# kronbichler/multigrid

Measured on AMD Instinct MI355X. Metric: DoFs/s for Laplace matvec + V-cycle, poisson_cube p=4 fp64, higher is better.
Workload: dtype f64; 1 GPU; poisson_cube FE_Q(4) 128^3 cells, 135005697 DoFs per GPU, 8 levels, step = 1 fp64 vmult + 1 V-cycle (Chebyshev degree 3, first kind); cells_per_dim=128, degree=4, n_dofs_per_gpu=135005697, global_dofs=135005697, parallelism=1 GPU

## Files before the change

### multigrid_amd/csrc/mgx_api.cpp

```cpp
#include "../../include/mgx.h"
#include "mgx_bricks.hpp"
#include "mgx_device_memory.hpp"
#include "mgx_internal.hpp"
#include "mgx_krylov.hpp"

#include <hip/hip_runtime.h>
#include <rccl/rccl.h>

#include <dlfcn.h>

#include <algorithm>
#include <chrono>
#include <cmath>
#include <cstdio>
#include <cstdlib>
#include <cstring>
#include <memory>
#include <string>
#include <type_traits>
#include <utility>
#include <vector>

using namespace mgx;

namespace
{
  thread_local std::string g_last_error;

  int fail(int code, const std::string &msg)
  {
    g_last_error = msg;
    return code;
  }

  inline size_t number_size(int number) { return number == MGX_F64 ? 8 : 4; }

  bool g_trace = false;
  bool trace_on() { return g_trace; }
#define MGX_TRACE(...)                  \
  do                                    \
    {                                   \
      if (trace_on())                   \
        {                               \
          std::fprintf(stderr, "[mgx] " __VA_ARGS__); \
          std::fputc('\n', stderr);     \
          std::fflush(stderr);          \
        }                               \
    }                                   \
  while (0)
}

int mgx::report_error(int code, const char *message) { return fail(code, message ? message : ""); }

#ifndef MGX_CELLS_FORM
#define MGX_CELLS_FORM 0
#endif
extern "C" int mgx_has_cells_form(void) { return MGX_CELLS_FORM; }
extern "C" int64_t mgx_live_device_allocations(void) { return mgx::live_device_allocations().load(); }

mgx::Tunables mgx::Tunables::from_environment()
{
  Tunables t;
  auto     num = [](const char *name, uint32_t dflt) {
    const char *e = std::getenv(name);
    return e ? (uint32_t)std::strtoul(e, nullptr, 10) : dflt;
  };
  t.trace               = std::getenv("MGX_TRACE") != nullptr;
  t.brick_min           = num("MGX_BRICK_MIN", t.brick_min);
  t.brick_min_from_env  = std::getenv("MGX_BRICK_MIN") != nullptr;
  t.overlap_min         = num("MGX_OVERLAP_MIN_BRICKS", t.overlap_min);
  t.restrict_colour_min = num("MGX_RESTRICT_COLOUR_MIN", t.restrict_colour_min);
  t.cell_colour_min     = num("MGX_CELL_COLOUR_MIN", t.cell_colour_min);
  t.free_max_bricks     = num("MGX_FREE_MAX_BRICKS", t.free_max_bricks);
  t.free_one_max        = num("MGX_FREE_ONE_MAX", t.free_one_max);
  t.graph_max_dofs      = num("MGX_GRAPH_MAX_DOFS", t.graph_max_dofs);
  return t;
}

bool mgx::Tunables::set(const std::string &name, double value)
{
  const bool     on = value != 0.;
  const uint32_t u  = value <= 0. ? 0u : (value >= 4294967295. ? 0xFFFFFFFFu : (uint32_t)value);
  struct Entry
  {
    const char *name;
    bool       *flag;
    uint32_t   *number;
  };
  const Entry table[] = {
    {"trace", &trace, nullptr},
    {"brick_min", nullptr, &brick_min},
    {"overlap_min_bricks", nullptr, &overlap_min},
    {"restrict_colour_min", nullptr, &restrict_colour_min},
    {"cell_colour_min", nullptr, &cell_colour_min},
    {"free_max_bricks", nullptr, &free_max_bricks},
    {"free_one_max", nullptr, &free_one_max},
    {"graph_max_dofs", nullptr, &graph_max_dofs},
    {"general_kernel", &general_kernel, nullptr},
    {"no_bricks", &no_bricks, nullptr},
#if MGX_CELLS_FORM
    {"cells_form", &cells_form, nullptr},
    {"brick_wide_max", nullptr, &wide_max},
#endif
    {"macro_wg_per_cu_x16", nullptr, &macro_wg_x16},
    {"no_diag_table", &no_diag_table, nullptr},
    {"no_macro_v2", &no_macro_v2, nullptr},
    {"no_general_bricks", &no_general_bricks, nullptr},
    {"general_brick_min", nullptr, &general_brick_min},
    {"fused_prolong_min_bricks", nullptr, &fused_prolong_min_bricks},
    {"roctx", &roctx, nullptr},
    {"no_fused_init", &no_fused_init, nullptr},
    {"no_fused_restrict", &no_fused_restrict, nullptr},
    {"no_fused_prolong", &no_fused_prolong, nullptr},
    {"force_fused_transfers", &force_fused_transfers, nullptr},
    {"transfer_v1", &transfer_v1, nullptr},
    {"restrict_atomic", &restrict_atomic, nullptr},
    {"exchange_unfused", &exchange_unfused, nullptr},
    {"no_graph", &no_graph, nullptr},
    {"dg_no_overlap", &dg_no_overlap, nullptr},
    {"dg_unmerged_restrict", &dg_unmerged_restrict, nullptr},
    {"no_fused_decomposed", &no_fused_decomposed, nullptr},
    {"no_fused_assembly", &no_fused_assembly, nullptr},
    {"no_fused_residual", &no_fused_residual, nullptr},
    {"no_restrict_scratch", &no_restrict_scratch, nullptr},
    {"rccl_selftest", &rccl_selftest, nullptr},
  };
  for (const Entry &e : table)
    if (name == e.name)
      {
        if (e.flag)
          *e.flag = on;
        else
          *e.number = u;
        if (name == "brick_min")
          brick_min_from_env = true;
        return true;
      }
  return false;
}

struct ExchangePlan
{
  std::vector<uint32_t> not_owned_host;
  int                    plan_id = 0, number = MGX_F64, self_pos = 0;
  std::vector<int>       rank;
  std::vector<uint32_t>  count;
  std::vector<uint32_t *> index_dev;
  std::vector<void *>    send, recv;
  uint32_t              *shared_dev = nullptr, *not_owned_dev = nullptr;
  uint32_t               n_shared = 0, n_not_owned = 0;
  void                  *own_buf = nullptr;
  std::vector<uint32_t>  start;
  uint32_t              *all_index_dev = nullptr, *csr_start_dev = nullptr, *csr_pos_dev = nullptr;
  uint8_t               *all_seg_dev = nullptr, *csr_k_dev = nullptr;
  bool                   fused = false;
};

struct RcclApi
{
  void *lib = nullptr;
  decltype(&ncclGetUniqueId)    GetUniqueId    = nullptr;
  decltype(&ncclCommInitRank)   CommInitRank   = nullptr;
  decltype(&ncclCommDestroy)    CommDestroy    = nullptr;
  decltype(&ncclGroupStart)     GroupStart     = nullptr;
  decltype(&ncclGroupEnd)       GroupEnd       = nullptr;
  decltype(&ncclSend)           Send           = nullptr;
  decltype(&ncclRecv)           Recv           = nullptr;
  decltype(&ncclAllReduce)      AllReduce      = nullptr;
  decltype(&ncclGetErrorString) GetErrorString = nullptr;
  bool load()
  {
    if (lib)
      return true;
    const char *names[] = {"librccl.so", "librccl.so.1", "/opt/rocm/lib/librccl.so.1"};
    for (const char *n : names)
      if ((lib = dlopen(n, RTLD_NOW | RTLD_NOLOAD)))
        break;
    if (!lib)
      for (const char *n : names)
        if ((lib = dlopen(n, RTLD_NOW | RTLD_GLOBAL)))
          break;
    if (!lib)
      return false;
#define MGX_RCCL_SYM(name)                                        \
  name = reinterpret_cast<decltype(name)>(dlsym(lib, "nccl" #name)); \
  if (!name)                                                      \
    {                                                             \
      lib = nullptr;                                              \
      return false;                                               \
    }
    MGX_RCCL_SYM(GetUniqueId)
    MGX_RCCL_SYM(CommInitRank)
    MGX_RCCL_SYM(CommDestroy)
    MGX_RCCL_SYM(GroupStart)
    MGX_RCCL_SYM(GroupEnd)
    MGX_RCCL_SYM(Send)
    MGX_RCCL_SYM(Recv)
    MGX_RCCL_SYM(AllReduce)
    MGX_RCCL_SYM(GetErrorString)
#undef MGX_RCCL_SYM
    return true;
  }
};
static RcclApi &rccl_api()
{
  static RcclApi api;
  return api;
}

struct mgx_context_s
{
  int         device = 0;
  Tunables    tun;
  DeviceArena mem{"mgx_context"};
  hipStream_t stream = nullptr;
  bool        borrowed_stream = false;
  hipStream_t side     = nullptr;
  hipEvent_t  ev_iface = nullptr, ev_side = nullptr;
  double     *partial_dev = nullptr;
  double     *result_dev  = nullptr;
  double     *result_host = nullptr;
  bool                                        profile = false;
  struct Bracket
  {
    hipEvent_t start, stop;
    int        form, launches;
  };
  std::vector<Bracket> ev_pool, ev_used;
  bool                                      has_comm = false;
  mgx_comm_desc                             comm{};
  ncclComm_t                                nccl = nullptr;
  bool                                      use_rccl = false;
  int                                       rccl_rank = 0, rccl_size = 1;
  double                                   *ar_dev = nullptr;
  std::vector<std::pair<size_t, struct ExchangePlan *>> plans;
};

struct mgx_operator_s
{
  mgx_context_t ctx = nullptr;
  DeviceArena   mem{"mgx_operator"};
  OperatorData  d;
  double        S[kMaxN * kMaxN], D[kMaxN * kMaxN], w[kMaxN];
  bool          has_diag = false;
  bool          profiled = false;
  uint32_t     *global_index_dev = nullptr;
  double        start_sum = 0, start_count = 0;
  std::unique_ptr<ExchangePlan> plan;
  double  *cg_partials = nullptr, *cg_result = nullptr;
  void    *cg_carrier  = nullptr;
  bool     constrained_last = false;
  bool     coef_update  = false;
  double   metric[6]    = {0, 0, 0, 0, 0, 0};
  double   det_jacobian = 0;
  void    *unit_q = nullptr, *jxw_q = nullptr;
};

struct mgx_smoother_s
{
  mgx_operator_t    op = nullptr;
  DeviceArena       mem{"mgx_smoother"};
  mgx_smoother_info info{};
  void             *x_old = nullptr, *tmp = nullptr;
  void             *x_old2 = nullptr;
  bool              fourth_kind = false;
  double            range_a     = 0;
  double            req_range  = 0;
  int               req_degree = 0, req_eig_its = 0;
  krylov::ChebyshevFactors factors() const { return krylov::ChebyshevFactors(info, fourth_kind); }
};

struct mgx_transfer_s
{
  mgx_operator_t coarse = nullptr, fine = nullptr;
  DeviceArena    mem{"mgx_transfer"};
  TransferData   d;
  void          *scratch = nullptr;
  void          *interp_1d  = nullptr;
  uint32_t      *own_coarse = nullptr;
};

struct mgx_solver_s
{
  mgx_context_t               ctx = nullptr;
  DeviceArena                 mem{"mgx_solver"};
  int                         n_levels = 0, degree = 0, n_cycles = 1, vnumber = MGX_F64;
  std::vector<mgx_operator_t> matrix, matrix_dp;
  std::vector<mgx_transfer_t> transfer, transfer_dp;
  std::vector<mgx_smoother_t> smooth;
  std::vector<double *>       solution, rhs, residual;
  std::vector<void *>         defect, t, solution_update;
  std::vector<uint32_t *>     bc_index_dev;
  std::vector<double *>       bc_value_dev, bc_zero_dev;
  std::vector<uint32_t>       bc_count;
  double                     *cg_r = nullptr, *cg_z = nullptr, *cg_d = nullptr, *cg_h = nullptr;
  bool                        timing = false;
  std::vector<double>         timings;
  int             graph_level = -1, graph_calls = 0;
  bool            graph_failed = false;
  hipGraph_t      graph = nullptr;
  hipGraphExec_t  graph_exec = nullptr;
  mgx_solver_t    agg_solver = nullptr;
  int             agg_level  = -1;
  int             agg_offset = 0;
  uint32_t       *agg_map    = nullptr;
  uint8_t        *agg_owned  = nullptr;
  hipEvent_t      agg_in = nullptr, agg_out = nullptr;
  std::vector<double> agg_host;
  std::vector<double> cg_history;
  std::vector<double *> nl_state;
};

namespace
{
  int read_result(mgx_context_t ctx, double *out)
  {
    MGX_HIP(hipMemcpyAsync(ctx->result_host, ctx->result_dev, sizeof(double), hipMemcpyDeviceToHost, ctx->stream));
    MGX_HIP(hipStreamSynchronize(ctx->stream));
    *out = ctx->result_host[0];
    return MGX_OK;
  }

  int comm_allreduce(mgx_context_t ctx, double *values, int count)
  {
    if (!ctx->has_comm)
      return MGX_OK;
    if (ctx->use_rccl)
      {
        if (count > 8)
          return fail(MGX_ERR_INVALID_ARGUMENT, "comm_allreduce: more than 8 values");
        RcclApi &R = rccl_api();
        MGX_HIP(hipMemcpyAsync(ctx->ar_dev, values, sizeof(double) * count, hipMemcpyHostToDevice, ctx->stream));
        if (R.AllReduce(ctx->ar_dev, ctx->ar_dev, (size_t)count, ncclDouble, ncclSum, ctx->nccl, ctx->stream) != ncclSuccess)
          return fail(MGX_ERR_HIP, "ncclAllReduce failed");
        MGX_HIP(hipMemcpyAsync(values, ctx->ar_dev, sizeof(double) * count, hipMemcpyDeviceToHost, ctx->stream));
        MGX_HIP(hipStreamSynchronize(ctx->stream));
        return MGX_OK;
      }
    if (!ctx->comm.allreduce_sum || ctx->comm.allreduce_sum(ctx->comm.user, values, count) != 0)
      return fail(MGX_ERR_HIP, "allreduce_sum callback failed");
    return MGX_OK;
  }

  int dot(mgx_context_t ctx, int number, const void *x, const void *y, size_t n, double *out,
          const ExchangePlan *plan = nullptr)
  {
    launch_dot(ctx->stream, number, x, y, n, ctx->partial_dev, ctx->result_dev);
    MGX_TRY(read_result(ctx, out));
    if (!ctx->has_comm)
      return MGX_OK;
    if (!plan)
      {
        for (auto &pr : ctx->plans)
          if (pr.first == n)
            {
              if (plan && (plan->n_not_owned != pr.second->n_not_owned || plan->n_shared != pr.second->n_shared))
                return fail(MGX_ERR_INVALID_ARGUMENT, "dot: two operators of this context have vectors of this length but "
                                                      "different ownership; reductions need the operator");
              plan = pr.second;
            }
        if (!plan)
          return fail(MGX_ERR_INVALID_ARGUMENT, "dot: no operator with vectors of this length is registered on this "
                                                "decomposed context (duplicated interface DoFs could not be discounted)");
      }
    if (plan->n_not_owned > 0)
      {
        double dup = 0;
        launch_dot_list(ctx->stream, number, x, y, plan->not_owned_dev, plan->n_not_owned, ctx->partial_dev,
                        ctx->result_dev);
        MGX_TRY(read_result(ctx, &dup));
        *out -= dup;
      }
    return comm_allreduce(ctx, out, 1);
  }

  int exchange_add(mgx_operator_t op, void *vec, hipStream_t on = nullptr, const BrickLaunch *post = nullptr,
                   bool *post_done = nullptr)
  {
    ExchangePlan *P = op->plan.get();
    if (!P)
      return MGX_OK;
    mgx_context_t ctx = op->ctx;
    hipStream_t   s   = on ? on : ctx->stream;
    const int     num = op->d.number;
    if (P->fused)
      launch_pack_all(s, num, P->send.data(), P->start.data(), (int)P->rank.size(), vec, P->all_index_dev,
                      P->all_seg_dev, P->start.back());
    else
      {
        for (size_t k = 0; k < P->rank.size(); ++k)
          launch_pack(s, num, P->send[k], vec, P->index_dev[k], P->count[k]);
        launch_pack(s, num, P->own_buf, vec, P->shared_dev, P->n_shared);
        launch_constrained_set(s, num, vec, 0.0, P->shared_dev, P->n_shared);
      }
    if (ctx->use_rccl)
      {
        RcclApi             &R  = rccl_api();
        const ncclDataType_t dt = num == MGX_F64 ? ncclDouble : ncclFloat;
        bool                 ok = R.GroupStart() == ncclSuccess;
        const bool to_self = ctx->tun.rccl_selftest && ctx->rccl_size == 1;
        for (size_t k = 0; ok && k < P->rank.size(); ++k)
          {
            const int peer = to_self ? 0 : P->rank[k];
            ok = ok && R.Send(P->send[k], P->count[k], dt, peer, ctx->nccl, s) == ncclSuccess;
            ok = ok && R.Recv(P->recv[k], P->count[k], dt, peer, ctx->nccl, s) == ncclSuccess;
          }
        ok = (R.GroupEnd() == ncclSuccess) && ok;
        if (!ok)
          return fail(MGX_ERR_HIP, "RCCL exchange failed");
// ... 1416 lines not shown
                                        op->cg_partials + 4 * (size_t)used);
          launch_reduce4(s, op->cg_partials, used, nullptr, op->cg_result);
          MGX_HIP(hipMemcpyAsync(sums, op->cg_result, 4 * sizeof(double), hipMemcpyDeviceToHost, s));
          MGX_HIP(hipStreamSynchronize(s));
          MGX_HIP(hipGetLastError());
          return MGX_OK;
        }
    }
  launch_cg_pre(s, num, x, p, q, alpha, beta, n);
  MGX_TRY(apply_plain(op, q, p));
  if (!ctx->has_comm)
    {
      const uint32_t used = launch_dot4(s, num, q, p, r, n, op->cg_partials);
      launch_reduce4(s, op->cg_partials, used, nullptr, op->cg_result);
      MGX_HIP(hipMemcpyAsync(sums, op->cg_result, 4 * sizeof(double), hipMemcpyDeviceToHost, s));
      MGX_HIP(hipStreamSynchronize(s));
    }
  else
    {
      MGX_TRY(dot(ctx, num, q, p, n, &sums[0], op->plan.get()));
      MGX_TRY(dot(ctx, num, r, r, n, &sums[1], op->plan.get()));
      MGX_TRY(dot(ctx, num, q, r, n, &sums[2], op->plan.get()));
      MGX_TRY(dot(ctx, num, q, q, n, &sums[3], op->plan.get()));
    }
  MGX_HIP(hipGetLastError());
  return MGX_OK;
}

static int brick_cell_lists(mgx_operator_t op, DeviceArena &mem, std::vector<uint32_t> &list_start, CellLists &out)
{
  const BrickData      &bd = op->d.bricks;
  const uint32_t        cb = op->d.n_cells / bd.n_bricks;
  std::vector<uint32_t> lists;
  list_start.assign(1, 0);
  lists.reserve(op->d.n_cells);
  for (int g = 0; g < bd.n_colours; ++g)
    for (uint32_t q = 0; q < 8; ++q)
      {
        for (uint32_t pos = bd.colour_start[g]; pos < bd.colour_start[g + 1]; ++pos)
          for (uint32_t m = q; m < cb; m += 8)
            lists.push_back(bd.order[pos] * cb + m);
        list_start.push_back((uint32_t)lists.size());
      }
  hipStream_t s         = op->ctx->stream;
  uint32_t   *lists_dev = nullptr;
  MGX_TRY(mem.alloc(&lists_dev, lists.size() + 1));
  MGX_HIP(hipMemcpyAsync(lists_dev, lists.data(), sizeof(uint32_t) * lists.size(), hipMemcpyHostToDevice, s));
  MGX_HIP(hipStreamSynchronize(s));
  out = CellLists(lists_dev, list_start.data(), (int)list_start.size() - 1);
  return MGX_OK;
}

int mgx_compute_residual(mgx_operator_t op, void *dst, const void *src, const void *rhs_q)
{
  MGX_REQUIRE(op && dst, "mgx_compute_residual: null argument");
  MGX_REQUIRE(dst != src, "mgx_compute_residual: dst and src must not alias");
  MGX_TRY(refuse_2d(op->d, "mgx_compute_residual", "right-hand sides of a two-dimensional problem are assembled on the host"));
  MGX_REQUIRE(op->d.idx27_plain, "mgx_compute_residual: the operator was created without idx27_plain");
  hipStream_t  s     = op->ctx->stream;
  const size_t bytes = number_size(op->d.number) * op->d.n_dofs;
  DeviceArena tmp("mgx_compute_residual");
  tmp.drain_before_release(s);
  if (!src)
    {
      void *zero = nullptr;
      MGX_TRY(tmp.zeros(&zero, bytes, s));
      src = zero;
    }
  MGX_HIP(hipMemsetAsync(dst, 0, bytes, s));
  std::vector<uint32_t> list_start;
  CellLists             lists;
  if (op->d.bricks.available())
    MGX_TRY(brick_cell_lists(op, tmp, list_start, lists));
  else if (op->d.cell_order && !op->d.asm_start)
    lists = CellLists(op->d);
  launch_cell_residual(s, op->d, dst, src, rhs_q, lists);
  MGX_HIP(hipGetLastError());
  return exchange_add(op, dst);
}

static int require_coef_q(mgx_operator_t op, const char *who)
{
  if (op->d.coef_q)
    return MGX_OK;
  return fail(MGX_ERR_UNSUPPORTED, std::string(who) + ": the operator has no per-point coefficient (separable or "
                                     "one-tensor-per-mesh branch); create it with mgx_operator_desc::coef_q set, e.g. to the "
                                     "unit-law tensor JxW_q J^-1 J^-T");
}

static int release_point_geometry(mgx_operator_t op)
{
  if (op->unit_q)
    {
      MGX_HIP(hipStreamSynchronize(op->ctx->stream));
      op->mem.release(op->unit_q);
      op->mem.release(op->jxw_q);
      op->unit_q = op->jxw_q = nullptr;
    }
  return MGX_OK;
}

static int set_point_geometry(mgx_operator_t op, const double *unit_q, const double *jxw_q, const char *who)
{
  const size_t nq = n_local_values(op->d.dim, op->d.p), nc = op->d.n_cells, nt = (size_t)n_tensor_entries(op->d.dim);
  const size_t nd = (size_t)op->d.dim;
  bool         ok = true;
  for (size_t c = 0; c < nc && ok; ++c)
    for (size_t q = 0; q < nq && ok; ++q)
      {
        ok = jxw_q[c * nq + q] > 0.;
        for (size_t k = 0; k < nd && ok; ++k)
          ok = unit_q[(c * nt + k) * nq + q] > 0.;
      }
  MGX_REQUIRE(ok, std::string(who) + ": JxW_q and the diagonal of JxW_q J^-1 J^-T must be positive at every quadrature point");
  void *u_dev = nullptr, *w_dev = nullptr;
  MGX_TRY(op->mem.upload_as(op->d.number, &u_dev, unit_q, nc * nt * nq));
  MGX_TRY(op->mem.upload_as(op->d.number, &w_dev, jxw_q, nc * nq));
  MGX_HIP(hipStreamSynchronize(op->ctx->stream));
  op->mem.release(op->unit_q);
  op->mem.release(op->jxw_q);
  op->unit_q      = u_dev;
  op->jxw_q       = w_dev;
  op->coef_update = true;
  return MGX_OK;
}

int mgx_operator_enable_coefficient_update_2d(mgx_operator_t op, const double metric[3], double det_jacobian)
{
  MGX_REQUIRE(op && metric, "mgx_operator_enable_coefficient_update_2d: null argument");
  if (op->d.dim != 2)
    return fail(MGX_ERR_UNSUPPORTED, "mgx_operator_enable_coefficient_update_2d: not on a three-dimensional operator (call "
                                     "mgx_operator_enable_coefficient_update)");
  MGX_TRY(require_coef_q(op, "mgx_operator_enable_coefficient_update_2d"));
  MGX_REQUIRE(det_jacobian > 0. && metric[0] > 0. && metric[0] * metric[1] - metric[2] * metric[2] > 0.,
              "mgx_operator_enable_coefficient_update_2d: the metric must be positive definite and det J > 0");
  MGX_TRY(release_point_geometry(op));
  std::fill(op->metric, op->metric + 6, 0.);
  std::copy(metric, metric + 3, op->metric);
  op->det_jacobian = det_jacobian;
  op->coef_update  = true;
  return MGX_OK;
}

int mgx_operator_enable_coefficient_update_q_2d(mgx_operator_t op, const double *unit_q, const double *jxw_q)
{
  MGX_REQUIRE(op && unit_q && jxw_q, "mgx_operator_enable_coefficient_update_q_2d: null argument");
  if (op->d.dim != 2)
    return fail(MGX_ERR_UNSUPPORTED, "mgx_operator_enable_coefficient_update_q_2d: not on a three-dimensional operator (call "
                                     "mgx_operator_enable_coefficient_update_q)");
  MGX_TRY(require_coef_q(op, "mgx_operator_enable_coefficient_update_q_2d"));
  return set_point_geometry(op, unit_q, jxw_q, "mgx_operator_enable_coefficient_update_q_2d");
}

int mgx_operator_enable_coefficient_update(mgx_operator_t op, const double metric[6], double det_jacobian)
{
  MGX_REQUIRE(op && metric, "mgx_operator_enable_coefficient_update: null argument");
  MGX_TRY(refuse_2d(op->d, "mgx_operator_enable_coefficient_update",
                    "the arrays of this call are three-dimensional: call mgx_operator_enable_coefficient_update_2d"));
  MGX_TRY(require_coef_q(op, "mgx_operator_enable_coefficient_update"));
  const double m0 = metric[0], m1 = metric[1], m2 = metric[2], m3 = metric[3], m4 = metric[4], m5 = metric[5];
  const double det_m = m0 * (m1 * m2 - m5 * m5) - m3 * (m3 * m2 - m5 * m4) + m4 * (m3 * m5 - m1 * m4);
  MGX_REQUIRE(det_jacobian > 0. && m0 > 0. && m0 * m1 - m3 * m3 > 0. && det_m > 0.,
              "mgx_operator_enable_coefficient_update: the metric must be positive definite and det J > 0");
  MGX_TRY(release_point_geometry(op));
  std::copy(metric, metric + 6, op->metric);
  op->det_jacobian = det_jacobian;
  op->coef_update  = true;
  return MGX_OK;
}

int mgx_operator_enable_coefficient_update_q(mgx_operator_t op, const double *unit_q, const double *jxw_q)
{
  MGX_REQUIRE(op && unit_q && jxw_q, "mgx_operator_enable_coefficient_update_q: null argument");
  MGX_TRY(refuse_2d(op->d, "mgx_operator_enable_coefficient_update_q",
                    "the arrays of this call are three-dimensional: call mgx_operator_enable_coefficient_update_q_2d"));
  MGX_TRY(require_coef_q(op, "mgx_operator_enable_coefficient_update_q"));
  return set_point_geometry(op, unit_q, jxw_q, "mgx_operator_enable_coefficient_update_q");
}

static int require_coefficient_update(mgx_operator_t op, int law, const char *who)
{
  const std::string w(who);
  MGX_REQUIRE(law == MGX_LAW_UNIT || law == MGX_LAW_MINIMAL_SURFACE, w + ": unknown law");
  if (op->ctx->has_comm || op->plan)
    return fail(MGX_ERR_UNSUPPORTED, w + ": not on a decomposed mesh (single rank only)");
  if (op->d.dim == 2 && !op->coef_update)
    return fail(MGX_ERR_UNSUPPORTED, w + ": not on a two-dimensional operator without a geometry: call "
                                         "mgx_operator_enable_coefficient_update_2d (affine cells) or "
                                         "mgx_operator_enable_coefficient_update_q_2d (curved cells) first");
  MGX_REQUIRE(op->coef_update, w + ": call mgx_operator_enable_coefficient_update (affine geometry of the level) or "
                                   "mgx_operator_enable_coefficient_update_q (curved cells) first");
  MGX_REQUIRE(op->d.idx27_plain, w + ": the operator was created without idx27_plain (the state is read with its boundary values)");
  return MGX_OK;
}

int mgx_evaluate_coefficient(mgx_operator_t op, int law, const void *state)
{
  MGX_REQUIRE(op && state, "mgx_evaluate_coefficient: null argument");
  MGX_TRY(require_coefficient_update(op, law, "mgx_evaluate_coefficient"));
  (op->d.dim == 2 ? launch_evaluate_coefficient_2d : launch_evaluate_coefficient)(
    op->ctx->stream, op->d, op->d.coef_q, op->d.number, law == MGX_LAW_MINIMAL_SURFACE, op->metric, op->det_jacobian, op->unit_q,
    op->jxw_q, state);
  MGX_HIP(hipGetLastError());
  op->has_diag = false;
  return MGX_OK;
}

int mgx_operator_get_coefficient(mgx_operator_t op, const void **dptr, size_t *n)
{
  MGX_REQUIRE(op && dptr && n, "mgx_operator_get_coefficient: null argument");
  if (!op->d.coef_q)
    return fail(MGX_ERR_UNSUPPORTED, "mgx_operator_get_coefficient: the operator has no per-point coefficient");
  *dptr = op->d.coef_q;
  *n    = (size_t)op->d.n_cells * n_tensor_entries(op->d.dim) * n_local_values(op->d.dim, op->d.p);
  return MGX_OK;
}

int mgx_compute_nonlinear_residual(mgx_operator_t op, int law, void *dst, const void *state)
{
  MGX_REQUIRE(op && dst && state, "mgx_compute_nonlinear_residual: null argument");
  MGX_REQUIRE(dst != state, "mgx_compute_nonlinear_residual: dst and state must not alias");
  MGX_TRY(require_coefficient_update(op, law, "mgx_compute_nonlinear_residual"));
  hipStream_t s  = op->ctx->stream;
  const bool  ms = law == MGX_LAW_MINIMAL_SURFACE;
  if (!op->d.asm_start && !op->d.cell_order)
    return fail(MGX_ERR_UNSUPPORTED, "mgx_compute_nonlinear_residual: the level has neither cell colours nor the ordered-assembly "
                                     "tables (more than 32 colours): no reproducible assembly");
  CellLists lists;
  if (!op->d.asm_start)
    {
      MGX_HIP(hipMemsetAsync(dst, 0, number_size(op->d.number) * op->d.n_dofs, s));
      lists = CellLists(op->d);
    }
  if (op->d.dim == 2)
    launch_cell_nl_residual_2d(s, op->d, ms, op->metric, op->det_jacobian, op->unit_q, op->jxw_q, dst, state);
  else
    launch_cell_nl_residual(s, op->d, ms, op->metric, op->det_jacobian, op->unit_q, op->jxw_q, dst, state, lists);
  MGX_HIP(hipGetLastError());
  return MGX_OK;
}

int mgx_compute_diagonal(mgx_operator_t op)
{
  MGX_REQUIRE(op, "mgx_compute_diagonal: null argument");
  hipStream_t s = op->ctx->stream;
  const int   n = op->d.p + 1;
  double a1d[kMaxN], m1d[kMaxN];
  double G[kMaxN * kMaxN];
  nodal_gradient(*op, G);
  for (int i = 0; i < n; ++i)
    {
      double a = 0, m = 0;
      for (int q = 0; q < n; ++q)
        {
          const double g = G[q * n + i];
          a += op->w[q] * g * g;
          m += op->w[q] * op->S[q * n + i] * op->S[q * n + i];
        }
      a1d[i] = a;
      m1d[i] = m;
    }
  MGX_HIP(hipMemsetAsync(op->d.inv_diag, 0, number_size(op->d.number) * op->d.n_dofs, s));
  DeviceArena lists_mem("mgx_compute_diagonal");
  lists_mem.drain_before_release(s);
  std::vector<uint32_t> list_start;
  CellLists             lists;
  if (op->d.bricks.available())
    MGX_TRY(brick_cell_lists(op, lists_mem, list_start, lists));
  else if (op->d.cell_order)
    lists = CellLists(op->d);
  launch_cell_diagonal(s, op->d, op->d.inv_diag, a1d, m1d, lists);
  MGX_TRY(exchange_add(op, op->d.inv_diag));
  launch_constrained_set(s, op->d.number, op->d.inv_diag, 1.0, op->d.constrained, op->d.n_constrained);
  launch_invert(s, op->d.number, op->d.inv_diag, op->d.n_dofs);
  MGX_HIP(hipGetLastError());
  op->has_diag = true;
  for (int which = 0; which < 2; ++which)
    {
      void          *&slot = which == 0 ? op->d.diag_items : op->d.diag_items2;
      const uint32_t *map  = which == 0 ? op->d.bricks.item_map : op->d.bricks.item_map2;
      op->mem.release(slot);
      slot = nullptr;
      if (!map || !op->d.separable || op->ctx->tun.no_diag_table)
        continue;
      const uint32_t nb = op->d.p <= 4 ? 4 : 2, g = nb * op->d.p + 1, npts = g * g * g;
      DeviceArena    tmp("mgx_compute_diagonal");
      void          *table = nullptr;
      uint32_t      *flag  = nullptr, mismatch = 1;
      MGX_TRY(op->mem.zeros(&table, number_size(op->d.number) * npts, s));
      MGX_TRY(tmp.zeros(&flag, 1, s));
      if (op->d.number == MGX_F64)
        macro_diag_table_f64(s, op->d, map, table, flag);
      else
        macro_diag_table_f32(s, op->d, map, table, flag);
      MGX_HIP(hipMemcpyAsync(&mismatch, flag, sizeof(uint32_t), hipMemcpyDeviceToHost, s));
      MGX_HIP(hipStreamSynchronize(s));
      if (mismatch == 0)
        slot = table;
      else
        op->mem.release(table);
      if (which == 0)
        MGX_TRACE("compute_diagonal: diagonal %s per brick item", mismatch == 0 ? "uniform" : "not uniform");
    }
  return MGX_OK;
}

int mgx_get_inverse_diagonal(mgx_operator_t op, const void **dptr)
{
  MGX_REQUIRE(op && dptr, "mgx_get_inverse_diagonal: null argument");
  MGX_REQUIRE(op->has_diag, "mgx_get_inverse_diagonal: call mgx_compute_diagonal first");
  *dptr = op->d.inv_diag;
  return MGX_OK;
}

int mgx_smoother_create(mgx_operator_t op, double smoothing_range, int degree, int eig_cg_n_iterations,
                        mgx_smoother_t *out)
{
  MGX_REQUIRE(op && out, "mgx_smoother_create: null argument");
  MGX_REQUIRE(eig_cg_n_iterations > 2, "mgx_smoother_create: eig_cg_n_iterations must be > 2");
  if (!op->has_diag)
    MGX_TRY(mgx_compute_diagonal(op));
  mgx_context_t ctx = op->ctx;
  hipStream_t   s   = ctx->stream;
  const int     num = op->d.number;
  const size_t  n   = op->d.n_dofs, bytes = number_size(num) * n;
  std::unique_ptr<mgx_smoother_s, int (*)(mgx_smoother_t)> sm(new mgx_smoother_s, mgx_smoother_destroy);
  sm->op            = op;
  sm->req_range     = smoothing_range;
  sm->req_degree    = degree;
  sm->req_eig_its   = eig_cg_n_iterations;
  MGX_TRY(sm->mem.alloc(&sm->x_old, bytes));
  MGX_TRY(sm->mem.alloc(&sm->tmp, bytes));
  void       *r = nullptr, *z = nullptr, *d = nullptr, *h = sm->tmp, *x = sm->x_old;
  DeviceArena scratch("mgx_smoother_create");
  for (void **v : {&r, &z, &d})
    MGX_TRY(scratch.alloc(v, bytes));
  {
    double sc[2] = {op->start_sum, op->start_count};
    MGX_TRY(comm_allreduce(ctx, sc, 2));
    launch_index_mod11(s, num, r, op->global_index_dev, sc[0] / sc[1], n);
  }
  MGX_HIP(hipMemsetAsync(x, 0, bytes, s));
  double res = 0;
  MGX_TRY(mgx_operator_l2_norm(op, r, &res));
  MGX_TRACE("smoother_create: n=%zu eig_its=%d res0=%g", n, eig_cg_n_iterations, res);
  const auto jacobi = [&](double *rz) {
    launch_jacobi_dot(s, num, z, op->d.inv_diag, r, n, ctx->partial_dev, ctx->result_dev);
    return fused_sum(op, r, z, rz);
  };
  CGOps<decltype(jacobi)> ops{op, x, r, z, d, h, jacobi};
  mgx_smoother_info      &info = sm->info;
  MGX_TRY(krylov::lanczos_estimate(ops, res, eig_cg_n_iterations, krylov::RitzRule{}, info));
  MGX_HIP(hipStreamSynchronize(s));
  const double a = krylov::chebyshev_interval(smoothing_range, degree, info);
  MGX_TRACE("smoother_create: its=%d lambda=[%g,%g] degree=%d", info.cg_iterations, info.lambda_min, info.lambda_max, info.degree);
  sm->range_a = a;
  *out        = sm.release();
  return MGX_OK;
}

int mgx_smoother_destroy(mgx_smoother_t sm)
{
  if (!sm)
    return MGX_OK;
  (void)hipStreamSynchronize(sm->op->ctx->stream);
  delete sm;
  return MGX_OK;
}

int mgx_smoother_get_info(mgx_smoother_t sm, mgx_smoother_info *info)
{
  MGX_REQUIRE(sm && info, "mgx_smoother_get_info: null argument");
  *info = sm->info;
  return MGX_OK;
}

int mgx_smoother_set_polynomial_type(mgx_smoother_t sm, int polynomial_type)
{
  MGX_REQUIRE(sm, "mgx_smoother_set_polynomial_type: null smoother");
  MGX_REQUIRE(polynomial_type == MGX_CHEBYSHEV_FIRST_KIND || polynomial_type == MGX_CHEBYSHEV_FOURTH_KIND,
              "mgx_smoother_set_polynomial_type: unknown polynomial type");
  sm->fourth_kind = polynomial_type == MGX_CHEBYSHEV_FOURTH_KIND;
  sm->info.delta  = sm->fourth_kind ? sm->info.lambda_max : (sm->info.lambda_max - sm->range_a) * 0.5;
  return MGX_OK;
}

static bool cheb_in_assembly(mgx_operator_t op)
{
  return op->d.asm_start && !op->plan && op->constrained_last && !op->ctx->tun.no_fused_assembly;
}

static void cheb_assembly_iteration(mgx_smoother_t sm, void *x, const void *b, double f1, double f2, bool three_term)
{
  mgx_operator_t op = sm->op;
  ProfileBracket pb(op, three_term ? kCheb : kChebFirst);
  const ChebPost post{sm->x_old, b, op->d.inv_diag, f1, f2, three_term};
  launch_cell_loop(op->ctx->stream, op->d, x, x, nullptr, op->d.n_dofs - op->d.n_constrained, &post);
}

static int cheb_loop(mgx_smoother_t sm, void *x, const void *b)
{
  const mgx_smoother_info &I = sm->info;
  mgx_operator_t           op = sm->op;
  hipStream_t              s  = op->ctx->stream;
  if (I.degree < 2 || std::fabs(I.delta) < 1e-40)
    return MGX_OK;
  krylov::ChebyshevFactors F = sm->factors();
  for (int k = 0; k < I.degree - 1; ++k)
    {
      double f1, f2;
      F.next(k, f1, f2);
      if (cheb_in_assembly(op))
        {
          cheb_assembly_iteration(sm, x, b, f1, f2, true);
          continue;
        }
      MGX_TRY(mgx_vmult(op, sm->tmp, x));
      launch_cheb_update(s, op->d.number, kUpdateThreeTerm, x, sm->x_old, b, sm->tmp, op->d.inv_diag, f1, f2, op->d.n_dofs);
    }
  MGX_HIP(hipGetLastError());
  return MGX_OK;
}

static int cheb_fused_iteration(mgx_smoother_t sm, BrickMode mode, const void *cur, const void *old, void *out,
                                const void *b, double f1, double f2, double f0 = 0., const void *coarse = nullptr,
                                const uint32_t *coarse_blocks = nullptr, const TransferData *prolong_tr = nullptr)
{
  mgx_operator_t op = sm->op;
  hipStream_t    s  = op->ctx->stream;
  BrickLaunch l;
  l.mode          = mode;
  l.src           = cur;
  l.rhs           = b;
  l.dinv          = op->d.inv_diag;
  l.old           = old;
  l.out           = out;
  l.carrier       = sm->tmp;
  l.f0            = f0;
  l.f1            = f1;
  l.f2            = f2;
  l.coarse        = const_cast<void *>(coarse);
  l.coarse_blocks = coarse_blocks;
  l.free_schedule = op->d.bricks.fr.available() && on_free_schedule(mode);
  const bool folded = l.free_schedule && !op->plan;
  bool post_done = false;
  MGX_TRY(brick_loop_with_exchange(
    op, mode, sm->tmp, [&](hipStream_t st, int g0, int g1) { launch_brick_loop(st, op->d, l.groups(g0, g1)); },
    [&](hipStream_t st) {
      if (mode == kChebFirstProlong)
        launch_interface_prolong_cheb(st, op->d.number, *prolong_tr, op->plan->shared_dev, coarse, const_cast<void *>(cur), out, b,
                                      op->d.inv_diag, f2, sm->tmp);
      else
        launch_cheb_constrained(st, op->d.number, mode, cur, out, b, op->d.inv_diag, f1, f2, op->plan->shared_dev,
                                op->plan->n_shared, sm->tmp, old, f0);
    },
    l.free_schedule,
    [&](hipStream_t st, uint32_t first, uint32_t count) {
      launch_surf_finish(st, op->d, l, first, count, folded ? op->d.constrained : nullptr, folded ? op->d.n_constrained : 0u);
    },
    (op->plan && mode != kChebFirstProlong && !op->ctx->tun.exchange_unfused) ? &l : nullptr, &post_done));
  if (!folded && !post_done)
    launch_cheb_constrained(s, op->d.number, mode, cur, out, b, op->d.inv_diag, f1, f2, op->d.constrained,
                            op->d.n_constrained, nullptr, old, f0);
  MGX_HIP(hipGetLastError());
  return MGX_OK;
}

static int smoother_apply(mgx_smoother_t sm, void *x, const void *b, bool is_step, const void *prolong_coarse = nullptr,
                          const uint32_t *prolong_blocks = nullptr, const TransferData *prolong_tr = nullptr)
{
  const mgx_smoother_info &I  = sm->info;
  mgx_operator_t           op = sm->op;
  hipStream_t              s  = op->ctx->stream;
  const int                num = op->d.number;
  const size_t             n   = op->d.n_dofs;
  if (!op->d.bricks.available())
    {
      if (is_step && cheb_in_assembly(op))
        cheb_assembly_iteration(sm, x, b, 0., sm->factors().first(), false);
      else if (is_step)
        {
          MGX_TRY(mgx_vmult(op, sm->tmp, x));
          launch_cheb_update(s, num, kUpdateFirst, x, sm->x_old, b, sm->tmp, op->d.inv_diag, 0., sm->factors().first(), n);
        }
      else
        launch_cheb_update(s, num, kUpdateStart, x, sm->x_old, b, nullptr, op->d.inv_diag, 0., sm->factors().first(), n);
      return cheb_loop(sm, x, b);
    }
  const bool three_term = I.degree >= 2 && std::fabs(I.delta) >= 1e-40;
  const int  n_loop     = three_term ? I.degree - 1 : 0;
  void      *X = x, *Y = sm->x_old;
  if (!is_step && n_loop >= 1 && op->d.separable && !op->ctx->tun.no_fused_init)
    {
      const double f0   = sm->factors().first();
      krylov::ChebyshevFactors F = sm->factors();
      void        *cur = nullptr, *old = nullptr;
      for (int k = 0; k < n_loop; ++k)
        {
          double f1, f2;
          F.next(k, f1, f2);
          void *out = ((n_loop - 1 - k) % 2 == 0) ? X : Y;
          MGX_TRY(cheb_fused_iteration(sm, k == 0 ? kChebInit : (k == 1 ? kChebOldInit : kCheb), cur, old, out, b, f1, f2, f0));
          old = cur;
          cur = out;
        }
      return MGX_OK;
    }
  if (!is_step)
    {
      void *cur = (n_loop % 2 == 0) ? X : Y, *old = nullptr;
      launch_cheb_init(s, num, cur, b, op->d.inv_diag, sm->factors().first(), n);
      krylov::ChebyshevFactors F = sm->factors();
      for (int k = 0; k < n_loop; ++k)
        {
          double f1, f2;
          F.next(k, f1, f2);
          void *out = (cur == X) ? Y : X;
          MGX_TRY(cheb_fused_iteration(sm, k == 0 ? kChebZeroOld : kCheb, cur, old, out, b, f1, f2));
          old = cur;
          cur = out;
        }
      return MGX_OK;
    }
  const int T = 1 + n_loop;
  if (T % 2 == 1 && T >= 3 && !sm->x_old2)
    MGX_TRY(sm->mem.alloc(&sm->x_old2, number_size(num) * n));
  void  *Z = sm->x_old2, *cur = X, *old = nullptr;
  krylov::ChebyshevFactors F = sm->factors();
  for (int k = 1; k <= T; ++k)
    {
      void *out;
      if (T % 2 == 0)
        out = (cur == X) ? Y : X;
      else if (T == 1)
        out = Y;
      else
        out = k == 1 ? Y : (k == 2 ? Z : (k == 3 ? X : ((cur == X) ? Y : X)));
      if (k == 1)
        MGX_TRY(cheb_fused_iteration(sm, prolong_blocks ? kChebFirstProlong : kChebFirst, cur, nullptr, out, b, 0., sm->factors().first(), 0.,
                                     prolong_coarse, prolong_blocks, prolong_tr));
      else
        {
          double f1, f2;
          F.next(k - 2, f1, f2);
          MGX_TRY(cheb_fused_iteration(sm, kCheb, cur, old, out, b, f1, f2));
        }
      old = cur;
      cur = out;
    }
  if (cur != X)
    launch_copy_cast(s, X, num, cur, num, n);
  return MGX_OK;
}

int mgx_smoother_vmult(mgx_smoother_t sm, void *x, const void *b)
{
  MGX_REQUIRE(sm && x && b && x != b, "mgx_smoother_vmult: bad argument");
  return smoother_apply(sm, x, b, false);
}

int mgx_smoother_step(mgx_smoother_t sm, void *x, const void *b)
{
  MGX_REQUIRE(sm && x && b && x != b, "mgx_smoother_step: bad argument");
  return smoother_apply(sm, x, b, true);
}

static int build_interface_transfer(mgx_transfer_s *tr, const mgx_transfer_desc *desc, const std::vector<uint32_t> &idxc)
{
  mgx_operator_t      fine = tr->fine, coarse = tr->coarse;
  const int           p = fine->d.p, n = p + 1;
  const uint32_t      npar = coarse->d.n_cells, nsh = fine->plan->n_shared;
  const ExchangePlan &pl = *fine->plan;
  std::vector<uint32_t> shared(nsh), pos(fine->d.n_dofs, kInvalid);
  if (nsh)
    MGX_HIP(hipMemcpy(shared.data(), pl.shared_dev, sizeof(uint32_t) * nsh, hipMemcpyDeviceToHost));
  for (uint32_t i = 0; i < nsh; ++i)
    pos[shared[i]] = i;
  std::vector<uint8_t> foreign(nsh, 0), done(nsh, 0);
  for (uint32_t d : pl.not_owned_host)
    if (pos[d] != kInvalid)
      foreign[pos[d]] = 1;
  std::vector<uint32_t> idxf(27 * (size_t)fine->d.n_cells);
  MGX_HIP(hipMemcpy(idxf.data(), fine->d.idx27, sizeof(uint32_t) * idxf.size(), hipMemcpyDeviceToHost));
  auto dof_of = [p](const uint32_t *ind, int ix, int iy, int iz) {
    const int      i[3] = {ix, iy, iz};
    int            code[3], off[3], len[3];
    for (int d = 0; d < 3; ++d)
      {
        code[d] = i[d] == 0 ? 0 : (i[d] == p ? 2 : 1);
        off[d]  = code[d] == 1 ? i[d] - 1 : 0;
        len[d]  = code[d] == 1 ? p - 1 : 1;
      }
    const uint32_t base = ind[(code[2] * 3 + code[1]) * 3 + code[0]];
    return base == kInvalid ? kInvalid : base + (uint32_t)((off[2] * len[1] + off[1]) * len[0] + off[0]);
  };
  struct Entry
  {
    uint32_t si, cdof;
    double   w;
  };
  std::vector<Entry> ent;
  for (uint32_t pc = 0; pc < npar; ++pc)
    for (int ch = 0; ch < 8; ++ch)
      {
        const uint32_t *indf = &idxf[27 * (size_t)desc->children[8 * (size_t)pc + ch]];
        bool            any = false;
// ... 1590 lines not shown
```

### multigrid_amd/csrc/mgx_brick_device.hpp

```cpp
#pragma once

#include "mgx_internal.hpp"

#include <hip/hip_runtime.h>

namespace mgx
{
  template <int P, bool WIDE = false>
  struct BCfg
  {
    static constexpr int  NB         = P <= 4 ? 4 : 2;
    static constexpr int  NCELLS     = NB * NB * NB;
    static constexpr int  N          = P + 1;
    static constexpr int  LN         = N | 1;
    static constexpr int  G          = NB * P + 1;
    static constexpr int  NE1        = 2 * NB + 1;
    static constexpr int  NE         = NE1 * NE1 * NE1;
    static constexpr int  TPC        = N * N;
    static constexpr bool kTwoPerWave = P <= 4;
    static constexpr int  TPW        = kTwoPerWave ? 32 : ((TPC + 63) / 64) * 64;
    static constexpr bool kWide      = WIDE && kTwoPerWave;
    static constexpr int  ROUND_CELLS = kTwoPerWave ? (kWide ? 16 : 8) : 2;
    static constexpr int  ROUNDS     = NCELLS / ROUND_CELLS;
    static constexpr int  THREADS    = kTwoPerWave ? (kWide ? 512 : 256) : 2 * TPW;
    static constexpr bool kWaveSync  = kTwoPerWave || TPW == 64;
    static constexpr int  CELL_LDS   = N * N * LN;
  };

  template <typename T>
  struct BrickPost
  {
    const T *a;
    const T *b;
    const T *old;
    T       *out;
    T       *partial;
    T        f1, f2, f0;
    T              *coarse;
    const uint32_t *coarse_blocks;
    T              *coarse_scratch;
    T              *src_w;
    T              *x_w;
    double         *sums;
    T              *priv;
    const uint32_t *surf_off;
    uint32_t        n_surf, priv_bytes;
  };

  template <typename T>
  BrickPost<T> make_post(const BrickLaunch &l)
  {
    BrickPost<T> post{};
    post.a              = (const T *)l.rhs;
    post.b              = (const T *)l.dinv;
    post.old            = (const T *)l.old;
    post.out            = (T *)l.out;
    post.partial        = (T *)l.carrier;
    post.f1             = (T)l.f1;
    post.f2             = (T)l.f2;
    post.f0             = (T)l.f0;
    post.coarse         = (T *)l.coarse;
    post.coarse_blocks  = l.coarse_blocks;
    post.coarse_scratch = (T *)l.coarse_scratch;
    return post;
  }

  __device__ __forceinline__ uint32_t ent_index(uint32_t w) { return w & 0x3FFFFFFFu; }
  __device__ __forceinline__ uint32_t ent_flags_of(uint32_t w) { return w >> 30; }

  __device__ __forceinline__ void wave_sync()
  {
    asm volatile("" ::: "memory");
    __builtin_amdgcn_wave_barrier();
    asm volatile("" ::: "memory");
  }

  __device__ __forceinline__ void lds_barrier()
  {
    asm volatile("s_waitcnt lgkmcnt(0)\n\ts_barrier" ::: "memory");
  }

#ifndef MGX_PACKED_F32
#define MGX_PACKED_F32 1
#endif
  template <int N, typename T>
  __device__ __forceinline__ void eo_split(const T (&x)[N], T (&xe)[N / 2 + 1], T (&xo)[N / 2 + 1])
  {
    constexpr int H = N / 2;
#pragma unroll
    for (int i = 0; i < H; ++i)
      {
        xe[i] = x[i] + x[N - 1 - i];
        xo[i] = x[i] - x[N - 1 - i];
      }
    xe[H] = (N % 2) ? x[H] : T(0);
    xo[H] = T(0);
  }

  template <int N, typename T>
  __device__ __forceinline__ void eo_apply(const EOMat<T> &A, const T (&xe)[N / 2 + 1], const T (&xo)[N / 2 + 1],
                                           T (&y)[N])
  {
    constexpr int H = N / 2;
    if constexpr (sizeof(T) == 4 && MGX_PACKED_F32)
      {
        typedef T T2 __attribute__((ext_vector_type(2)));
#pragma unroll
        for (int a = 0; a < H; ++a)
          {
            T2 r = T2{A.ee[a * H], A.eo[a * H]} * T2{xe[0], xo[0]};
#pragma unroll
            for (int i = 1; i < H; ++i)
              r = __builtin_elementwise_fma(T2{A.ee[a * H + i], A.eo[a * H + i]}, T2{xe[i], xo[i]}, r);
            if (N % 2)
              r[0] = fma(A.mc[a], xe[H], r[0]);
            y[a]         = r[0] + r[1];
            y[N - 1 - a] = r[0] - r[1];
          }
        if (N % 2)
          {
            T r = A.mhh * xe[H];
#pragma unroll
            for (int i = 0; i < H; ++i)
              r = fma(A.mc[i], xe[i], r);
            y[H] = r;
          }
        return;
      }
#pragma unroll
    for (int a = 0; a < H; ++a)
      {
        T r0 = A.ee[a * H] * xe[0];
        T r1 = A.eo[a * H] * xo[0];
#pragma unroll
        for (int i = 1; i < H; ++i)
          {
            r0 = fma(A.ee[a * H + i], xe[i], r0);
            r1 = fma(A.eo[a * H + i], xo[i], r1);
          }
        if (N % 2)
          r0 = fma(A.mc[a], xe[H], r0);
        y[a]         = r0 + r1;
        y[N - 1 - a] = r0 - r1;
      }
    if (N % 2)
      {
        T r = A.mhh * xe[H];
#pragma unroll
        for (int i = 0; i < H; ++i)
          r = fma(A.mc[i], xe[i], r);
        y[H] = r;
      }
  }

  template <int ROW, int TOTAL>
  __device__ __forceinline__ void scalar_operand_slice(int k)
  {
    constexpr int C = (40 / ROW) < 1 ? 1 : 40 / ROW;
    if (TOTAL > 48 && (k + 1) % C == 0)
      {
        asm volatile("" ::: "memory");
        __builtin_amdgcn_sched_barrier(0);
      }
  }

  template <int P, typename T>
  __device__ __forceinline__ void restrict_half(const T *__restrict__ pe, const T (&r)[2 * P + 1], T (&o)[P + 1])
  {
    constexpr int NH = (P + 1) / 2, TOT = (2 * P + 1) * NH + ((P % 2 == 0) ? P + 1 : 0);
#ifdef MGX_RESTRICT_DENSE
    {
      constexpr int N = P + 1, M = 2 * P + 1;
      const T *p1 = reinterpret_cast<const Basis1D<T> *>(reinterpret_cast<const char *>(pe) - offsetof(Basis1D<T>, P1eo))->P1;
#pragma unroll
      for (int j = 0; j < N; ++j)
        {
          T s = p1[j] * r[0];
#pragma unroll
          for (int a = 1; a < M; ++a)
            s = fma(p1[a * N + j], r[a], s);
          o[j] = s;
          scalar_operand_slice<M, M * N>(j);
        }
      return;
    }
#endif
    const T      *he = pe, *ho = pe + (P + 1) * NH, *pc = pe + (2 * P + 1) * NH;
    T             re[P + 1], ro[P];
#pragma unroll
    for (int a = 0; a < P; ++a)
      {
        re[a] = r[a] + r[2 * P - a];
        ro[a] = r[a] - r[2 * P - a];
      }
    re[P] = r[P];
#pragma unroll
    for (int j = 0; j < NH; ++j)
      {
        T se = he[j] * re[0], so = ho[j] * ro[0];
#pragma unroll
        for (int a = 1; a <= P; ++a)
          se = fma(he[a * NH + j], re[a], se);
#pragma unroll
        for (int a = 1; a < P; ++a)
          so = fma(ho[a * NH + j], ro[a], so);
        o[j]     = se + so;
        o[P - j] = se - so;
        scalar_operand_slice<2 * P + 1, TOT>(j);
      }
    if (P % 2 == 0)
      {
        T s = pc[0] * re[0];
#pragma unroll
        for (int a = 1; a <= P; ++a)
          s = fma(pc[a], re[a], s);
        o[P / 2] = s;
      }
  }

  template <int P, typename T, int NT, bool SCRATCH = false>
  __device__ __forceinline__ void restrict_brick(int tid, T *acc, const T *__restrict__ p1, T *__restrict__ coarse,
                                                 const uint32_t *__restrict__ ctab, T *__restrict__ scratch = nullptr)
  {
    using C           = BCfg<P>;
    constexpr int G   = C::G, PB = C::NB / 2, CN = PB * P + 1, CE1 = 2 * PB + 1, N = P + 1, M = 2 * P + 1;
    auto layer = [](int a, int &e, int &o, int &n) {
      const int q = a / P, rr = a - q * P;
      e           = 2 * q + (rr != 0);
      o           = rr ? rr - 1 : 0;
      n           = rr ? P - 1 : 1;
    };
    constexpr int NZ = (CN * CN * PB + NT - 1) / NT;
    T            *cp[SCRATCH ? 1 : NZ][N];
    T             cv[SCRATCH ? 1 : NZ][N];
    bool          ok[SCRATCH ? 1 : NZ][N];
#pragma unroll
    for (int it = 0; it < (SCRATCH ? 0 : NZ); ++it)
      {
        const int t = tid + it * NT, l = t / PB, pb = t % PB;
        const bool live = t < CN * CN * PB;
        const int  x = live ? l % CN : 0, y = live ? l / CN : 0;
        int        ex, ey, ox, oy, nx, ny;
        layer(x, ex, ox, nx);
        layer(y, ey, oy, ny);
#pragma unroll
        for (int j = 0; j < N; ++j)
          {
            int ez, oz, nz;
            layer(pb * P + j, ez, oz, nz);
            const uint32_t w = ctab[(ez * CE1 + ey) * CE1 + ex];
            ok[it][j] = live && w != kInvalid && !(PB == 2 && pb == 1 && j == 0);
            cp[it][j] = coarse + (ok[it][j] ? w + (uint32_t)((oz * ny + oy) * nx + ox) : 0u);
            cv[it][j] = *cp[it][j];
          }
      }
    auto sweep = [&](int lines, auto base, int stride, auto sink) {
#pragma unroll 1
      for (int t0 = 0; t0 < lines * PB; t0 += NT)
        {
          const int  t = t0 + tid, l = t / PB, pb = t % PB;
          const bool live = t < lines * PB;
          T          r[M], o[N];
          const int  b0 = base(live ? l : 0) + pb * 2 * P * stride;
#pragma unroll
          for (int a = 0; a < M; ++a)
            r[a] = acc[b0 + a * stride];
          restrict_half<P, T>(p1, r, o);
          if (PB == 2)
            {
              const T up = __shfl_down(o[0], 1);
              if (pb == 0)
                o[P] += up - r[2 * P];
            }
          sink(live, l, pb, o);
        }
    };
    sweep(
      G * G, [&](int l) { return l * G; }, 1,
      [&](bool live, int l, int pb, const T(&o)[N]) {
        if (live)
          {
#pragma unroll
            for (int j = (pb == 0 ? 0 : 1); j < N; ++j)
              acc[l * G + pb * P + j] = o[j];
          }
      });
    lds_barrier();
    sweep(
      CN * G, [&](int l) { return (l / CN) * G * G + l % CN; }, G,
      [&](bool live, int l, int pb, const T(&o)[N]) {
        if (live)
          {
            const int x = l % CN, z = l / CN;
#pragma unroll
            for (int j = (pb == 0 ? 0 : 1); j < N; ++j)
              acc[(z * G + pb * P + j) * G + x] = o[j];
          }
      });
    lds_barrier();
    {
      int it = 0;
      sweep(
        CN * CN, [&](int l) { return (l / CN) * G + l % CN; }, G * G,
        [&](bool live, int l, int pb, const T(&o)[N]) {
          if (SCRATCH)
            {
              if (live)
                {
#pragma unroll
                  for (int j = (pb == 0 ? 0 : 1); j < N; ++j)
                    scratch[(size_t)((pb * P + j) * CN * CN + l)] = o[j];
                }
            }
          else
            {
#pragma unroll
              for (int k = 0; k < (SCRATCH ? 0 : NZ); ++k)
                if (k == it)
                  {
#pragma unroll
                    for (int j = 0; j < N; ++j)
                      if (ok[SCRATCH ? 0 : k][j])
                        *cp[SCRATCH ? 0 : k][j] = cv[SCRATCH ? 0 : k][j] + o[j];
                  }
            }
          ++it;
        });
    }
  }

  template <int P, typename T>
  __device__ __forceinline__ void prolong_half(const T *__restrict__ pe, const T (&c)[P + 1], T (&f)[2 * P + 1])
  {
    constexpr int NH = (P + 1) / 2, TOT = (2 * P + 1) * NH + ((P % 2 == 0) ? P + 1 : 0);
    constexpr int ROW = 2 * NH + (P % 2 == 0 ? 1 : 0);
    const T      *he = pe, *ho = pe + (P + 1) * NH, *pc = pe + (2 * P + 1) * NH;
    T             ce[NH], co[NH];
#pragma unroll
    for (int i = 0; i < NH; ++i)
      {
        ce[i] = c[i] + c[P - i];
        co[i] = c[i] - c[P - i];
      }
    const T cc = c[P / 2];
#pragma unroll
    for (int a = 0; a <= P; ++a)
      {
        T se = he[a * NH] * ce[0];
#pragma unroll
// ... 166 lines not shown
```

### multigrid_amd/csrc/mgx_internal.hpp

```cpp
#pragma once

#include "../../include/mgx.h"

#include <hip/hip_runtime.h>

#include <algorithm>
#include <chrono>
#include <cstddef>
#include <cstdint>
#include <string>
#include <type_traits>
#include <vector>

struct mgx_context_s;

namespace mgx
{
  constexpr int      kMaxN    = MGX_MAX_DEGREE + 1;
  constexpr uint32_t kInvalid = 0xFFFFFFFFu;

  struct Tunables
  {
    bool     trace            = false;
    bool     general_kernel   = false;
    bool     no_bricks        = false;
    uint32_t brick_min        = 512;
    bool     brick_min_from_env = false;
    uint32_t overlap_min      = 16384;
    bool     cells_form       = false;
    uint32_t wide_max         = 1024;
    bool     dg_no_overlap    = false;
    bool     no_restrict_scratch = false;
    bool     no_fused_residual = false;
    bool     no_fused_assembly = false;
    bool     no_fused_decomposed = false;
    bool     dg_unmerged_restrict = false;
    uint32_t macro_wg_x16     = 0;
    bool     no_diag_table    = false;
    bool     roctx            = false;
    uint32_t fused_prolong_min_bricks = 8192;
    bool     no_general_bricks = false;
    uint32_t general_brick_min = 2048;
    bool     no_macro_v2      = false;
    bool     no_fused_init    = false;
    bool     no_fused_restrict = false;
    bool     no_fused_prolong = false;
    bool     force_fused_transfers = false;
    bool     transfer_v1      = false;
    bool     restrict_atomic  = false;
    uint32_t restrict_colour_min = 16384;
    bool     exchange_unfused = false;
    uint32_t cell_colour_min  = 0xFFFFFFFFu;
    uint32_t free_max_bricks  = 16384;
    uint32_t free_one_max     = 1024;
    bool     no_graph         = false;
    uint32_t graph_max_dofs   = 600000;
    bool     rccl_selftest    = false;
    static Tunables from_environment();
    bool            set(const std::string &name, double value);
  };

  template <typename T>
  struct EOMat
  {
    T ee[(kMaxN / 2) * (kMaxN / 2)];
    T eo[(kMaxN / 2) * (kMaxN / 2)];
    T mc[kMaxN / 2];
    T mhh;
  };

  template <typename T>
  struct Basis1D
  {
    T S[kMaxN * kMaxN];
    T D[kMaxN * kMaxN];
    T w[kMaxN];
    T P1[2 * kMaxN * kMaxN];
    EOMat<T> mass, lapl;
    T P1eo[2 * kMaxN * kMaxN];
  };

  struct FreeSchedule
  {
    int       n_classes = 0;
    int       n_groups = 0, n_iface_groups = 0;
    uint32_t  group_start[9] = {0};
    uint32_t *ent         = nullptr;
    uint32_t *surf_off    = nullptr;
    uint32_t  n_surf      = 0;
    void     *priv        = nullptr;
    uint32_t *surf_dof    = nullptr, *surf_start = nullptr, *surf_pos = nullptr;
    uint32_t  n_surf_dofs = 0, n_surf_shared = 0;
    bool      available() const { return ent != nullptr; }
  };

  struct BrickData
  {
    uint32_t  n_bricks  = 0;
    int       n_colours = 0;
    int       n_iface_groups = 0;
    uint32_t  colour_start[33] = {0};
    uint32_t *ent_base  = nullptr;
    uint8_t  *ent_flags = nullptr;
    uint32_t *item_map  = nullptr;
    uint32_t *item_map2 = nullptr;
    std::vector<uint32_t> order;
    uint32_t *order_dev = nullptr;
    bool      available() const { return n_bricks > 0; }
    FreeSchedule fr;
  };
  constexpr int kBrickEntities = 729;
  constexpr int kMaxColours    = 32;

  struct OperatorData
  {
    int       p        = 0;
    int       number   = 1;
    int       dim      = 3;
    uint32_t  n_cells  = 0;
    uint32_t  n_dofs   = 0;
    uint32_t  n_constrained = 0;
    uint32_t *idx27         = nullptr;
    uint32_t *idx27_plain   = nullptr;
    uint32_t *constrained   = nullptr;
    void     *basis         = nullptr;
    void     *inv_diag      = nullptr;
    double    coef[6]       = {0, 0, 0, 0, 0, 0};
    bool      full_tensor   = false;
    void     *coef_q        = nullptr;
    void     *grad_1d       = nullptr;
    uint32_t *cell_order    = nullptr;
    int       n_cell_colours = 0;
    uint32_t  cell_colour_start[33] = {0};
    uint32_t *asm_start     = nullptr;
    uint32_t *asm_pos       = nullptr;
    void     *cell_scratch  = nullptr;
    BrickData bricks;
    BrickData gbricks;
    bool      cells_form    = false;
    uint32_t  wide_max      = 1024;
    uint32_t  macro_wg_x16  = 0;
    uint32_t  n_cus         = 256;
    bool      separable     = true;
    void     *diag_items    = nullptr;
    void     *diag_items2   = nullptr;
    bool      macro_v2      = true;
  };

  struct TransferData
  {
    const OperatorData *coarse = nullptr, *fine = nullptr;
    uint32_t           *children = nullptr;
    uint8_t            *weight_shift = nullptr;
    uint32_t           *own27 = nullptr;
    uint32_t           *patch = nullptr;
    uint32_t           *coarse_blocks = nullptr;
    void               *coarse_scratch = nullptr;
    uint32_t           *cs_start = nullptr, *cs_pos = nullptr;
    uint32_t           *ifr_cdof = nullptr, *ifr_start = nullptr, *ifr_fdof = nullptr;
    void               *ifr_w = nullptr;
    uint32_t            n_ifr = 0;
    uint32_t           *ifp_start = nullptr, *ifp_cdof = nullptr;
    void               *ifp_w = nullptr;
    uint32_t            n_ifp = 0;
    mutable uint32_t    pipe_grid[4] = {0, 0, 0, 0};
    bool                owner_weights = false;
    bool                coarse_coloured = false;
    uint32_t           *parent_order = nullptr;
    int                 n_parent_colours = 0;
    uint32_t            parent_colour_start[33] = {0};
    uint32_t            n_cus = 256;
    uint32_t            colour_min = 16384;
  };

  int  exchange_buffers(struct ::mgx_context_s *ctx, int plan_id, int number, int n_neighbors, const int *ranks,
                        const uint32_t *counts, void *const *send, void *const *recv, hipStream_t stream = nullptr);
  hipStream_t side_stream_begin(struct ::mgx_context_s *ctx);
  int         side_stream_end(struct ::mgx_context_s *ctx);
  int  allreduce_sum(struct ::mgx_context_s *ctx, double *values, int count);
  int  dot_owned_prefix(struct ::mgx_context_s *ctx, int number, const void *x, const void *y, size_t n, double *out);
  bool context_has_comm(struct ::mgx_context_s *ctx);
  int  operator_dim(struct ::mgx_operator_s *op);
  const Tunables &context_tunables(struct ::mgx_context_s *ctx);
  struct LevelTimer
  {
    struct ::mgx_context_s               *ctx;
    double                               *slot;
    bool                                  ranges;
    std::chrono::steady_clock::time_point t0;
    LevelTimer(struct ::mgx_context_s *ctx, bool timed, double *times, int level, int part, bool with_ranges = false);
    ~LevelTimer();
    LevelTimer(const LevelTimer &) = delete;
  };
  int residual_update_finish(hipStream_t s, int number, const void *cycle_result, double *residual, double *update, double factor,
                             size_t n_free, size_t n, double *partials, double *sums_dev, double out[2]);

  int report_error(int code, const char *message);
  inline int report_error(int code, const std::string &message) { return report_error(code, message.c_str()); }

#define MGX_HIP(call)                                                                                                \
  do                                                                                                                 \
    {                                                                                                                \
      hipError_t e_ = (call);                                                                                        \
      if (e_ != hipSuccess)                                                                                          \
        return mgx::report_error(MGX_ERR_HIP, std::string(#call) + ": " + hipGetErrorString(e_) + " (" + __FILE__ + ":" + \
                                                std::to_string(__LINE__) + ")");                                     \
    }                                                                                                                \
  while (0)

#define MGX_TRY(call)     \
  do                      \
    {                     \
      int s_ = (call);    \
      if (s_ != MGX_OK)   \
        return s_;        \
    }                     \
  while (0)

#define MGX_REQUIRE(cond, msg)                                      \
  do                                                                \
    {                                                               \
      if (!(cond))                                                  \
        return mgx::report_error(MGX_ERR_INVALID_ARGUMENT, (msg));  \
    }                                                               \
  while (0)

  void launch_prolongate_pipe(hipStream_t s, const TransferData &t, void *fine, const void *coarse, bool add,
                              bool with_constraints);
  void launch_restrict_add_pipe(hipStream_t s, const TransferData &t, void *coarse, const void *fine,
                                bool with_constraints);

  struct CellLists
  {
    const uint32_t *cells = nullptr;
    const uint32_t *start = nullptr;
    int             n     = 0;
    CellLists() = default;
    CellLists(const uint32_t *cells_, const uint32_t *start_, int n_) : cells(cells_), start(start_), n(n_) {}
    explicit CellLists(const OperatorData &op) : cells(op.cell_order), start(op.cell_colour_start), n(op.n_cell_colours) {}
  };
  struct CellTensor
  {
    const void *per_point = nullptr;
    double      c[6]      = {0, 0, 0, 0, 0, 0};
    static CellTensor at_points(const void *q)
    {
      CellTensor t;
      t.per_point = q;
      return t;
    }
    static CellTensor per_mesh(const double *m)
    {
      CellTensor t;
      std::copy(m, m + 6, t.c);
      return t;
    }
    static CellTensor of(const OperatorData &op) { return op.coef_q ? at_points(op.coef_q) : per_mesh(op.coef); }
  };
  struct ChebPost
  {
    void       *x_old;
    const void *b, *dinv;
    double      f1, f2;
    bool        three_term;
  };
  void launch_cell_loop(hipStream_t s, const OperatorData &op, void *dst, const void *src, const void *tail_src = nullptr,
                        uint32_t n_head = 0,
                        const ChebPost *post = nullptr);
  void launch_general_bricks(hipStream_t s, const OperatorData &op, void *dst, const void *src);
  void launch_assemble(hipStream_t s, const OperatorData &op, int mode, void *dst, const void *tail_src, uint32_t n_head);
  void launch_assemble_cheb(hipStream_t s, const OperatorData &op, void *x, uint32_t n_head, const ChebPost &post);
  enum BrickMode
  {
    kPlain    = 0,
    kResidual = 1,
    kCheb     = 2,
    kChebFirst = 3,
    kChebZeroOld = 4,
    kChebInit    = 5,
    kChebOldInit = 6,
    kResidualRestrict = 7,
    kCgUpdate = 8,
    kChebFirstProlong = 9
  };
  __host__ __device__ constexpr bool is_cheb_mode(int mode)
  {
    return (mode >= kCheb && mode <= kChebOldInit) || mode == kChebFirstProlong;
  }
  constexpr bool on_free_schedule(int mode) { return mode >= kPlain && mode <= kChebOldInit; }

  struct BrickLaunch
  {
    BrickMode       mode    = kPlain;
    const void     *src     = nullptr;
    const void     *rhs     = nullptr;
    const void     *dinv    = nullptr;
    const void     *old     = nullptr;
    void           *out     = nullptr;
    void           *carrier = nullptr;
    double          f0 = 0., f1 = 0., f2 = 0.;
    void           *coarse         = nullptr;
    const uint32_t *coarse_blocks  = nullptr;
    void           *coarse_scratch = nullptr;
    int             group_begin = 0, group_end = -1;
    bool            free_schedule = false;

    BrickLaunch groups(int g0, int g1) const
    {
      BrickLaunch l = *this;
      l.group_begin = g0;
      l.group_end   = g1;
      return l;
    }
    BrickLaunch resolved(int n_groups = 0) const
    {
      BrickLaunch l = *this;
      if (l.group_end < 0)
        l.group_end = n_groups;
      if (!l.old)
        l.old = l.out;
      if (!l.src)
        l.src = l.rhs;
      return l;
    }
  };
  void launch_brick_loop(hipStream_t s, const OperatorData &op, const BrickLaunch &launch);

  template <typename F>
  static bool dispatch_degree(int p, F &&f)
  {
    switch (p)
      {
#define MGX_DEGREE_CASE(P) \
  case P: f(std::integral_constant<int, P>()); return true;
#ifdef MGX_MACRO_ONLY_P
        MGX_DEGREE_CASE(MGX_MACRO_ONLY_P)
#else
        MGX_DEGREE_CASE(1)
        MGX_DEGREE_CASE(2)
        MGX_DEGREE_CASE(3)
        MGX_DEGREE_CASE(4)
        MGX_DEGREE_CASE(5)
        MGX_DEGREE_CASE(6)
        MGX_DEGREE_CASE(7)
        MGX_DEGREE_CASE(8)
        MGX_DEGREE_CASE(9)
#endif
#undef MGX_DEGREE_CASE
        default: return false;
      }
  }
  template <int... MODES, typename F>
  static bool dispatch_mode(int mode, F &&f)
  {
    return ((mode == MODES ? (f(std::integral_constant<int, MODES>()), true) : false) || ...);
  }
  template <typename F>
  static void dispatch_number(int number, F &&f)
  {
    if (number == MGX_F64)
      f(double());
    else
      f(float());
  }
  template <typename F>
  static bool dispatch_number_degree(int number, int p, F &&f)
  {
    bool found = false;
    dispatch_number(number, [&](auto t) { found = dispatch_degree(p, [&](auto P) { f(t, P); }); });
    return found;
  }
  inline uint32_t persistent_grid(const OperatorData &op, int wgs_per_cu, uint32_t count)
  {
    const uint32_t resident = op.macro_wg_x16 ? std::max<uint32_t>(1u, op.n_cus * op.macro_wg_x16 / 16u) : (uint32_t)wgs_per_cu * op.n_cus;
    return std::min(count, resident);
  }
  void launch_cell_residual(hipStream_t s, const OperatorData &op, void *dst, const void *src, const void *rhs_q,
                            const CellLists &lists);
  void launch_cell_nl_residual(hipStream_t s, const OperatorData &op, bool minimal_surface, const double *metric, double det,
                               const void *unit_q, const void *jxw_q, void *dst, const void *src, const CellLists &lists);
  void launch_evaluate_coefficient(hipStream_t s, const OperatorData &op, void *coef_q, int coef_number, bool minimal_surface,
                                   const double *metric, double det, const void *unit_q, const void *jxw_q, const void *state);
  void launch_interpolate_to_coarse(hipStream_t s, const TransferData &t, const void *r1d, const uint32_t *own_c, void *coarse,
                                    const void *fine);
  void launch_surf_finish(hipStream_t s, const OperatorData &op, const BrickLaunch &launch, uint32_t first, uint32_t count,
                          const uint32_t *constrained = nullptr, uint32_t n_constrained = 0,
                          const FreeSchedule *schedule = nullptr);
  bool launch_macro_loop_f64(hipStream_t s, const OperatorData &op, const BrickLaunch &launch);
  bool launch_macro_loop_f32(hipStream_t s, const OperatorData &op, const BrickLaunch &launch);
  bool launch_macro_cg_update_f64(hipStream_t s, const OperatorData &op, double alpha, double beta, const void *r, void *q,
                                  void *p, void *x, void *carrier, double *partials, uint32_t capacity,
                                  uint32_t *n_partials);
  bool launch_macro_cg_update_f32(hipStream_t s, const OperatorData &op, double alpha, double beta, const void *r, void *q,
                                  void *p, void *x, void *carrier, double *partials, uint32_t capacity,
                                  uint32_t *n_partials);
  void launch_reduce4(hipStream_t s, const double *partials, uint32_t n, const double *extra, double *sums);
  void macro_diag_table_f64(hipStream_t s, const OperatorData &op, const uint32_t *item_map, void *table, uint32_t *flag_dev);
  void macro_diag_table_f32(hipStream_t s, const OperatorData &op, const uint32_t *item_map, void *table, uint32_t *flag_dev);
  bool launch_macro2_loop_f64(hipStream_t s, const OperatorData &op, const BrickLaunch &launch);
  bool launch_macro2_loop_f32(hipStream_t s, const OperatorData &op, const BrickLaunch &launch);
  void launch_cell_diagonal(hipStream_t s, const OperatorData &op, void *diag, const double *a1d, const double *m1d,
                            const CellLists &lists);
  void launch_prolongate(hipStream_t s, const TransferData &t, void *fine, const void *coarse, bool add,
                         bool with_constraints);
  void launch_restrict_add(hipStream_t s, const TransferData &t, void *coarse, const void *fine,
                           bool with_constraints);
  void launch_cell_loop_2d(hipStream_t s, const OperatorData &op, void *dst, const void *src, const void *tail_src,
                           uint32_t n_head, const ChebPost *post);
  void launch_cell_diagonal_2d(hipStream_t s, const OperatorData &op, void *diag, const double *a1d, const double *m1d);
  void launch_prolongate_2d(hipStream_t s, const TransferData &t, void *fine, const void *coarse, bool add,
                            bool with_constraints);
  void launch_restrict_add_2d(hipStream_t s, const TransferData &t, void *coarse, const void *fine, bool with_constraints);
  void launch_evaluate_coefficient_2d(hipStream_t s, const OperatorData &op, void *coef_q, int coef_number, bool minimal_surface,
                                      const double *metric, double det, const void *unit_q, const void *jxw_q, const void *state);
  void launch_cell_nl_residual_2d(hipStream_t s, const OperatorData &op, bool minimal_surface, const double *metric, double det,
                                  const void *unit_q, const void *jxw_q, void *dst, const void *state);
  void launch_interpolate_to_coarse_2d(hipStream_t s, const TransferData &t, const void *r1d, const uint32_t *own_c, void *coarse,
                                       const void *fine);

  void launch_copy_cast(hipStream_t s, void *dst, int dn, const void *src, int sn, size_t n);
  void launch_add_cast(hipStream_t s, void *dst, int dn, const void *src, int sn, size_t n);
  void launch_sadd(hipStream_t s, int number, void *x, double sx, double a, const void *v, size_t n);
  void launch_rhs_minus(hipStream_t s, int number, void *res, const void *rhs, size_t n);
  void launch_constrained_copy(hipStream_t s, int number, void *dst, const void *src, const uint32_t *list,
                               uint32_t count);
  void launch_constrained_residual(hipStream_t s, int number, void *res, const void *rhs, const void *lhs,
                                   const uint32_t *list, uint32_t count);
  void launch_constrained_set(hipStream_t s, int number, void *v, double value, const uint32_t *list,
                              uint32_t count);
  void launch_invert(hipStream_t s, int number, void *v, size_t n);
  void launch_scatter_values(hipStream_t s, int number, void *v, const uint32_t *idx_dev, const double *val_dev,
                             uint32_t count);
  enum ChebUpdate
  {
    kUpdateStart     = 0,
    kUpdateFirst     = 1,
    kUpdateThreeTerm = 2
  };
  void launch_cheb_update(hipStream_t s, int number, ChebUpdate mode, void *x, void *x_old, const void *b,
                          const void *t, const void *dinv, double f1, double f2, size_t n);
  void launch_cheb_init(hipStream_t s, int number, void *x, const void *b, const void *dinv, double f2, size_t n);
  void launch_cheb_constrained(hipStream_t s, int number, BrickMode mode, const void *x, void *out, const void *b,
                               const void *dinv, double f1, double f2, const uint32_t *list, uint32_t count,
                               const void *ax = nullptr, const void *old = nullptr, double f0 = 0.);
  void launch_pack(hipStream_t s, int number, void *buf, const void *v, const uint32_t *list, uint32_t count);
  void launch_dg_cg_transfer(hipStream_t s, int number, int p, bool to_dg, void *dst, const void *src,
                             const uint32_t *idx27, uint32_t n_cells, const void *P1, bool eight_colours = false);
  bool launch_dg_transfer(hipStream_t s, int number, int fine_degree, int coarse_degree, bool prolong, void *dst, const void *src,
                          uint32_t n_groups, const void *m1d, int dim, const uint32_t *children, bool identity);
  namespace dg
  {
    struct Host1D;
    struct Geometry;

    enum Action
    {
      kVmult     = 0,
      kRestrict  = 1,
      kCgSums    = 2,
      kChebyshev = 3,
      kResidual  = 4,
      kJacobi    = 5,
      kPcgSums   = 6
    };

    struct CellOperands
    {
      int            number = 0, degree = 0, basis = 0;
      const int32_t *neigh    = nullptr;
      const void    *consts   = nullptr;
      const void    *inv_diag = nullptr;
      uint32_t       n_owned  = 0;
      bool           has_ghosts = false;
      int            dim        = 3;
      bool           has_neumann = false;
    };

    struct DGLaunch
    {
      DGLaunch(int action_, void *dst_, const void *rhs_, const void *src_) : action(action_), dst(dst_), rhs(rhs_), src(src_) {}
      int             action;
      void           *dst;
      const void     *rhs, *src;
      double          f1 = 0, f2 = 0;
      int             iteration_index = 0;
      const uint32_t *cell_list       = nullptr;
      uint32_t        cell_first = 0, cell_stride = 1, n_cells = 0;
      double         *partials = nullptr;
      void           *cg       = nullptr;
      const uint32_t *idx27    = nullptr;
      const void     *P1       = nullptr;
      int             plain    = 0;
      const void     *lumped   = nullptr;
    };
    int      launch_dg_cells(hipStream_t s, const CellOperands &op, const DGLaunch &launch);
    uint32_t cell_grid(int number, int p, uint32_t n_cells, int dim);
    std::vector<char> const_block(int number, const Host1D &h, const Geometry &g);
    void launch_pack_cells(hipStream_t s, int number, void *buf, const void *vec, const uint32_t *cells, uint32_t count,
                           uint32_t n3);
    void launch_pack_faces(hipStream_t s, int number, void *buf, const void *vec, const uint32_t *cells, const uint8_t *faces,
                           uint32_t count, int N, double hderiv);
    void launch_start_vector(hipStream_t s, int number, void *v, const uint32_t *cell_id, uint32_t n_cells, uint32_t n3,
                             double mean);

    struct DGFunctionArgs
    {
      int           kind = 0;
      double        amplitude = 0, wave[3] = {0, 0, 0}, phase[3] = {0, 0, 0};
      const double *cell_values = nullptr, *face_values = nullptr;
    };
    struct DGRhsGeometry
    {
      double jac[9], origin[3], xq[kMaxN], wq[kMaxN], det, sigma[3], fw[3], cn[3][3];
      double normal[3][3];
    };
    struct DGRhsOperands
    {
      int            number = 0, degree = 0, dim = 3;
      const int32_t *neigh    = nullptr;
      const void    *consts   = nullptr;
      const int32_t *cell_pos = nullptr;
      uint32_t       n_cells  = 0;
      bool           has_neumann = false;
      DGRhsGeometry  geo;
    };
    bool launch_dg_rhs(hipStream_t s, const DGRhsOperands &op, const DGFunctionArgs &f, const DGFunctionArgs &g,
                       const DGFunctionArgs &h, void *dst);
    bool     launch_dg_l2_error(hipStream_t s, const DGRhsOperands &op, const DGFunctionArgs &u, const void *vec, double *partials);
    uint32_t rhs_grid(int p, uint32_t n_cells, int dim);
  }
  void launch_zero_head_copy_tail(hipStream_t s, int number, void *dst, const void *src, uint32_t n_head, uint32_t n);
  void launch_scatter_map(hipStream_t s, int number, void *dst, const void *src, const uint32_t *map,
                          const uint8_t *mask, uint32_t n);
  void launch_pack_all(hipStream_t s, int number, void *const *send, const uint32_t *start, int n_neighbors,
                       const void *v, const uint32_t *index, const uint8_t *seg, uint32_t total);
  void launch_unpack_ordered(hipStream_t s, int number, void *const *recv, int n_neighbors, void *v,
                             const uint32_t *shared, const uint32_t *csr_start, const uint8_t *csr_k,
                             const uint32_t *csr_pos, uint32_t n_shared);
  void launch_unpack_ordered_cheb(hipStream_t s, int number, void *const *recv, int n_neighbors, void *v,
                                  const uint32_t *shared, const uint32_t *csr_start, const uint8_t *csr_k,
                                  const uint32_t *csr_pos, uint32_t n_shared, const BrickLaunch &post,
                                  const uint32_t *constrained, uint32_t n_constrained);
  void launch_unpack_add(hipStream_t s, int number, void *v, const void *buf, const uint32_t *list, uint32_t count);
  void launch_list_residual(hipStream_t s, int number, void *res, const void *rhs, const uint32_t *list,
                            uint32_t count);
  void launch_dot_list(hipStream_t s, int number, const void *x, const void *y, const uint32_t *list,
                       uint32_t count, double *partial_dev, double *result_dev);
  void launch_index_mod11(hipStream_t s, int number, void *v, const uint32_t *global_index_dev, double mean,
                          size_t n);
  void launch_dot(hipStream_t s, int number, const void *x, const void *y, size_t n, double *partial_dev,
                  double *result_dev);
  constexpr int kDotBlocks = 1024;
  void launch_cg_update(hipStream_t s, int number, void *x, void *r, const void *d, const void *h, double alpha,
                        size_t n, double *partial_dev, double *result_dev);
  void launch_xpby(hipStream_t s, int number, void *d, const void *z, double beta, size_t n);
  void launch_cg_update_f32copy(hipStream_t s, double *x, double *r, const double *d, const double *h, double alpha, size_t n,
                                float *r32, double *partial_dev, double *result_dev);
  void launch_dot_f64_f32(hipStream_t s, const double *x, const float *y, size_t n, double *partial_dev, double *result_dev);
  void launch_xpby_f64_f32(hipStream_t s, double *d, const float *z, double beta, size_t n);
  void launch_jacobi_dot(hipStream_t s, int number, void *z, const void *dinv, const void *r, size_t n,
                         double *partial_dev, double *result_dev);
  uint32_t launch_cg_list_update(hipStream_t s, int number, const uint32_t *list, uint32_t count, double alpha,
                                 double beta, const void *r, void *q, void *p, void *x, double *partials);
  void launch_coarse_assemble(hipStream_t s, int number, const TransferData &tr, void *coarse);
  void launch_interface_restrict(hipStream_t s, int number, const TransferData &tr, void *coarse, const void *b, const void *ax);
  void launch_interface_prolong_cheb(hipStream_t s, int number, const TransferData &tr, const uint32_t *shared, const void *e,
                                     void *x, void *out, const void *b, const void *dinv, double f2, const void *ax);
  uint32_t launch_axpy_norm(hipStream_t s, int number, void *r, const void *q, double factor, size_t n, double *partials);
  void     launch_cg_pre(hipStream_t s, int number, void *x, void *p, void *q, double alpha, double beta, size_t n);
  uint32_t launch_dot4(hipStream_t s, int number, const void *q, const void *p, const void *r, size_t n, double *partials);
  constexpr uint32_t kPcgTableMax = 1000;
  void launch_pcg_start(hipStream_t s, int number, void *x, void *r, void *p, const void *b, const void *table, uint32_t n3,
                        size_t n);
  constexpr uint32_t kPcgPresumFrom = 4096, kPcgPresums = 256;
  void launch_pcg_scalars(hipStream_t s, const double *partials, uint32_t n_partials, uint32_t k, double *scalars, double *rho_hist,
                          double *presums);
  void launch_pcg_update(hipStream_t s, int number, void *x, void *r, void *p, const void *q, const void *table, uint32_t n3,
                         const double *scalars, size_t n);
  void launch_tile_table(hipStream_t s, int number, void *v, const void *table, uint32_t n3, size_t n);
  void     launch_residual_pre(hipStream_t s, int defect_number, void *defect, const double *residual, const double *update,
                               double factor, size_t n);
  uint32_t launch_residual_post(hipStream_t s, int z_number, const void *z, double *residual, double *update, double factor,
                                size_t n_free, size_t n, double *partials);
}
```

### multigrid_amd/csrc/mgx_macro.hip

```cpp
#include "mgx_macro_device.hpp"

#include <hip/hip_runtime.h>

#include <algorithm>
#include <cstdlib>

#ifndef MGX_MACRO_CHUNK
#define MGX_MACRO_CHUNK (MGX_MACRO_PAIRS ? 3 : 4)
#endif
#ifndef MGX_MACRO_CHUNK_CHEB
#define MGX_MACRO_CHUNK_CHEB (MGX_MACRO_PAIRS ? 2 : 3)
#endif
#ifndef MGX_MACRO_T
#define MGX_MACRO_T double
#endif

#ifdef MGX_MACRO_STAMPS
#ifndef MGX_MACRO_STAMP_MODE
#define MGX_MACRO_STAMP_MODE -1
#endif
__device__ unsigned long long g_mgx_stamps[8192 * 16];
#define MGX_STAMP(k)                                                                    \
  do                                                                                    \
    {                                                                                   \
      if (threadIdx.x == 0 && blockIdx.x < 8192 && (MGX_MACRO_STAMP_MODE < 0 || MODE == MGX_MACRO_STAMP_MODE)) \
        g_mgx_stamps[blockIdx.x * 16 + (k)] = ((k) == 15 || (k) == 13) ? __builtin_amdgcn_s_memrealtime() \
                                                        : __builtin_amdgcn_s_memtime();  \
    }                                                                                   \
  while (0)
extern "C" int mgx_debug_read_stamps(unsigned long long *host, int n_blocks)
{
  return (int)hipMemcpyFromSymbol(host, HIP_SYMBOL(g_mgx_stamps), sizeof(unsigned long long) * 16 * n_blocks);
}
#define MGX_STAMP_IT(k)      \
  do                         \
    {                        \
      if (mgx_iter == 3)     \
        MGX_STAMP(k);        \
    }                        \
  while (0)
#define MGX_STAMP_NEXT() ++mgx_iter
#define mgx_iter_is(k) (mgx_iter == (k))
#else
#define MGX_STAMP(k) ((void)0)
#define MGX_STAMP_IT(k) ((void)0)
#define MGX_STAMP_NEXT() ((void)0)
#define mgx_iter_is(k) false
#endif

namespace mgx
{
  template <int P, typename T, int MODE, bool DTAB, bool FREE = false>
  __global__ void __launch_bounds__((MCfg<P, T>::THREADS), (MCfg<P, T>::MINW))
    brick_macro_kernel(const T *__restrict__ src, uint32_t brick_first, uint32_t brick_count,
                       const uint32_t *__restrict__ ent_base, const uint32_t *__restrict__ item_map,
                       const Basis1D<T> *__restrict__ B, T c0, T c1, T c2, BrickPost<T> post, uint32_t vec_bytes)
  {
    using C              = MCfg<P, T>;
    constexpr int G      = C::G;
    constexpr int NT     = C::THREADS;
    constexpr int IT     = C::IT;
    constexpr int LINES  = C::LINES;
    constexpr int NEW    = (C::NE + NT - 1) / NT;
    constexpr int N = P + 1, NB = C::NB;
    constexpr int REM    = LINES - NT;
    constexpr bool kKeepX = is_cheb_mode(MODE) || MODE == kCgUpdate;
    constexpr int  NG     = ((MODE == kChebInit && !DTAB) || MODE == kCgUpdate) ? 2 : 1;
    __shared__ T U[C::ASZ];
    __shared__ T W[C::ASZ];

    const int tid = threadIdx.x;
    uint32_t  b   = blockIdx.x;
    if (b >= brick_count)
      return;
    MGX_STAMP(0);
    MGX_STAMP(15);
#ifdef MGX_MACRO_STAGGER
    if (__builtin_amdgcn_s_getreg(6 | (0 << 6) | ((8 - 1) << 11)) != 0)
      for (int i = 0; i < MGX_MACRO_STAGGER; ++i)
        __builtin_amdgcn_s_sleep(64);
#endif
    constexpr int NP = C::NPAIR, NS = C::NSINGLE, JP = C::JP, JS = C::JS, NU = JP + JS;
    auto live_p = [&](int j) { return (j + 1) * NT <= NP || tid + j * NT < NP; };
    auto live_s = [&](int j) { return (j + 1) * NT <= NS || tid + j * NT < NS; };
    auto live   = [&](int v) { return v < 2 * JP ? live_p(v / 2) : live_s(v - 2 * JP); };
    uint32_t mw[IT];
#pragma unroll
    for (int j = 0; j < JP; ++j)
      {
        const int     q = tid + j * NT;
        const u32x2_t m = reinterpret_cast<const u32x2_t *>(item_map)[q < NP ? q : 0];
        mw[2 * j]       = m.x;
        mw[2 * j + 1]   = m.y;
      }
#pragma unroll
    for (int j = 0; j < JS; ++j)
      {
        const int q    = tid + j * NT;
        mw[2 * JP + j] = item_map[2 * NP + (q < NS ? q : 0)];
      }
    T dv[DTAB ? IT : 1];
    if (DTAB)
      {
#pragma unroll
        for (int j = 0; j < JP; ++j)
          {
            const int q                = tid + j * NT;
            dv[DTAB ? 2 * j : 0]       = post.b[2 * (q < NP ? q : 0)];
            dv[DTAB ? 2 * j + 1 : 0]   = post.b[2 * (q < NP ? q : 0) + 1];
          }
#pragma unroll
        for (int j = 0; j < JS; ++j)
          {
            const int q               = tid + j * NT;
            dv[DTAB ? 2 * JP + j : 0] = post.b[2 * NP + (q < NS ? q : 0)];
          }
      }
    const rsrc_t      rsrc = make_rsrc(src, vec_bytes);
    const PostRsrc<T> R{make_rsrc(post.a, vec_bytes),   make_rsrc(post.b, vec_bytes),       make_rsrc(post.old, vec_bytes),
                        make_rsrc(post.out, vec_bytes), make_rsrc(post.partial, vec_bytes), rsrc,
                        make_rsrc((MODE == kCgUpdate || MODE == kChebFirstProlong) ? post.src_w : post.out, vec_bytes),
                        make_rsrc(MODE == kCgUpdate ? post.x_w : post.out, vec_bytes),
                        make_rsrc(FREE ? (const void *)post.priv : (const void *)post.out, FREE ? post.priv_bytes : vec_bytes)};
    double cg[4] = {0., 0., 0., 0.};
    const EOMat<T>   &M = B->mass, &K = B->lapl;

    uint32_t ec[NEW], en[NEW];
    uint32_t sc[FREE ? NEW : 1];
    if (FREE)
      {
#pragma unroll
        for (int j = 0; j < NEW; ++j)
          {
            const int i      = tid + j * NT;
            sc[FREE ? j : 0] = post.surf_off[i < C::NE ? i : 0];
          }
      }
    auto table_load = [&](uint32_t brick, uint32_t(&e)[NEW]) {
#pragma unroll
      for (int j = 0; j < NEW; ++j)
        {
          const int i = tid + j * NT;
          e[j]        = ent_base[(size_t)(brick_first + brick) * C::NE + (i < C::NE ? i : 0)];
        }
    };
    auto table_store = [&](uint32_t *E, const uint32_t(&e)[NEW]) {
#pragma unroll
      for (int j = 0; j < NEW; ++j)
        if (tid + j * NT < C::NE)
          E[tid + j * NT] = e[j];
    };
    auto unit_offset = [&](uint32_t w, uint32_t m, int it = 0, uint32_t brick = 0) {
#ifdef MGX_MACRO_CONTIG
      return w != kInvalid ? ((brick_first + brick) * (uint32_t)(C::NB * C::NB * C::NB * P * P * P) + (uint32_t)(tid + it * NT)) * (uint32_t)sizeof(T) : kOob;
#else
      return w != kInvalid ? (ent_index(w) + item_offset(m)) * (uint32_t)sizeof(T) : kOob;
#endif
    };
    constexpr bool kProlong = MODE == kChebFirstProlong;
    constexpr int  CNP = (C::NB / 2) * P + 1, NCV = CNP * CNP * CNP / NT + 1, CE3 = (C::NB + 1) * (C::NB + 1) * (C::NB + 1);
    T              cvv[NCV];
    T    g[NG][IT];
    uint32_t cw[NCV];
    auto coarse_words = [&](uint32_t brick) {
      if (kProlong)
        {
          const uint32_t *ctab = post.coarse_blocks + (size_t)(brick_first + brick) * CE3;
#pragma unroll
          for (int k = 0; k < NCV; ++k)
            {
              const int l = tid + k * NT;
              int       slot = 0, pnt;
              uint32_t  off;
              if (l < CNP * CNP * CNP)
                coarse_point<P>(l, slot, off, pnt);
              cw[k] = ctab[slot];
            }
        }
    };
    auto coarse_values = [&]() {
      if (kProlong)
        {
#pragma unroll
          for (int k = 0; k < NCV; ++k)
            {
              const int l = tid + k * NT;
              cvv[k]      = T(0);
              if (l < CNP * CNP * CNP)
                {
                  int      slot, pnt;
                  uint32_t off;
                  coarse_point<P>(l, slot, off, pnt);
                  const uint32_t w = cw[k];
                  const T        v = post.coarse[w != kInvalid ? w + off : 0u];
                  cvv[k]           = w != kInvalid ? v : T(0);
                }
            }
        }
    };
    auto gather_issue = [&](const uint32_t *E, uint32_t brick) {
      const rsrc_t r0 = MODE == kChebInit ? (DTAB ? R.a : R.b) : rsrc;
      const rsrc_t r1 = MODE == kCgUpdate ? R.b : R.a;
#pragma unroll
      for (int j = 0; j < JP; ++j)
        {
#pragma unroll
          for (int e = 0; e < 2; ++e)
            g[0][2 * j + e] = g[NG - 1][2 * j + e] = T(0);
          if (live_p(j))
            {
              const uint32_t off = unit_offset(E[item_slot(mw[2 * j])], mw[2 * j], 2 * j, brick);
              buf_ld2(r0, off, g[0][2 * j], g[0][2 * j + 1]);
              if (NG == 2)
                buf_ld2(r1, off, g[NG - 1][2 * j], g[NG - 1][2 * j + 1]);
            }
        }
#pragma unroll
      for (int j = 0; j < JS; ++j)
        {
          const int v = 2 * JP + j;
          g[0][v] = g[NG - 1][v] = T(0);
          if (live_s(j))
            {
              const uint32_t off = unit_offset(E[item_slot(mw[v])], mw[v], v, brick);
              g[0][v]            = buf_ld(r0, off, T());
              if (NG == 2)
                g[NG - 1][v] = buf_ld(r1, off, T());
            }
        }
    };
    constexpr bool kKeepRhs = keeps_rhs(MODE);
    T              xs[kKeepX ? IT : 1];
    auto           gather_land = [&]() {
#pragma unroll
      for (int it = 0; it < IT; ++it)
        {
          T       v  = g[0][it];
          const T bi = g[DTAB ? 0 : NG - 1][it];
          if (MODE == kChebInit)
            v = cheb_first_iterate(post.f0, DTAB ? dv[DTAB ? it : 0] : g[0][it], bi);
          if (MODE == kCgUpdate)
            v = post.f1 == T(0) ? g[NG - 1][it] : post.f2 * g[0][it] + g[NG - 1][it];
          if (live(it))
            U[item_point(mw[it])] = v;
          if (kKeepX)
            xs[it] = kKeepRhs ? bi : v;
        }
    };

    auto interpolate = [&]() {
      if (kProlong)
        {
          lds_barrier();
          prolong_brick<P, T, NT>(tid, W, B->P1eo, cvv);
        }
    };
    auto add_correction = [&]() {
      if (kProlong)
        {
#pragma unroll
          for (int it = 0; it < IT; ++it)
            if (live(it))
              {
                const uint32_t pnt = item_point(mw[it]);
                xs[kKeepX ? it : 0] += W[pnt];
                U[pnt] = xs[kKeepX ? it : 0];
              }
        }
    };

    table_load(b, ec);
    table_store(reinterpret_cast<uint32_t *>(W), ec);
    __syncthreads();
    MGX_STAMP(1);
    gather_issue(reinterpret_cast<const uint32_t *>(W), b);
    coarse_words(b);
    coarse_values();
    interpolate();
    gather_land();
    add_correction();
    MGX_STAMP(2);
    __syncthreads();

#ifdef MGX_MACRO_STAMPS
    int mgx_iter = 0;
#endif
    for (;;)
      {
        if (mgx_iter_is(4))
          MGX_STAMP(11);
        const uint32_t bn       = b + gridDim.x;
        const bool     has_next = bn < brick_count;
        MGX_STAMP_IT(3);
        if (has_next)
          {
            table_load(bn, en);
            coarse_words(bn);
          }
#pragma unroll
        for (int it = 0; it < IT; ++it)
          asm volatile("" : "+v"(mw[it]));
        if (DTAB && (MODE == kChebInit || MODE == kChebOldInit))
          {
#pragma unroll
            for (int it = 0; it < IT; ++it)
              asm volatile("" : "+v"(dv[DTAB ? it : 0]));
          }
#ifndef MGX_MACRO_NOSWEEP
        if (kSlicedSweeps<P, MODE>)
          brick_sweeps_sliced<P, T>(
            tid, U, W, B, c0, c1, c2, [&](int i) { MGX_STAMP_IT(4 + i); }, [&]() { __syncthreads(); });
        else
          {
        if (tid < LINES)
          {
            const int l = tid;
            T         in[G], t1[G], k1[G];
#pragma unroll
            for (int j = 0; j < G; ++j)
              in[j] = U[l * G + j];
            macro_apply2<P, T>(M, K, in, t1, k1);
#pragma unroll
            for (int j = 0; j < G; ++j)
              {
                W[l * G + j] = t1[j];
                U[l * G + j] = k1[j];
              }
          }
        if (REM > 0 && tid < REM * NB)
          {
            const int l = NT + tid / NB, c = tid % NB, base = l * G + c * P;
            T         seg[N], y[N], z[N];
#pragma unroll
            for (int i = 0; i < N; ++i)
              seg[i] = U[base + i];
            cell_apply2<P, T>(M, K, seg, y, z);
            const T yn = next_lane(y[0]), zn = next_lane(z[0]);
            if (c + 1 < NB)
              {
                y[P] += yn;
                z[P] += zn;
              }
#pragma unroll
            for (int i = 1; i < N; ++i)
              {
                W[base + i] = y[i];
                U[base + i] = z[i];
              }
            if (c == 0)
              {
                W[base] = y[0];
                U[base] = z[0];
              }
          }
        __syncthreads();
        MGX_STAMP_IT(4);
        if (REM > 0 && tid < REM * NB)
          {
            const int l = NT + tid / NB, c = tid % NB, base = (l / G) * (G * G) + l % G + c * P * G;
            T         seg[N], y[N], z[N], r[N];
#pragma unroll
            for (int i = 0; i < N; ++i)
              seg[i] = W[base + i * G];
            cell_apply2<P, T>(M, K, seg, y, z);
#pragma unroll
            for (int i = 0; i < N; ++i)
              seg[i] = U[base + i * G];
            cell_apply<P, T>(M, seg, r);
#pragma unroll
            for (int i = 0; i < N; ++i)
              z[i] = fma(c0, r[i], c1 * z[i]);
            const T yn = next_lane(y[0]), zn = next_lane(z[0]);
            if (c + 1 < NB)
              {
                y[P] += yn;
                z[P] += zn;
              }
#pragma unroll
            for (int i = 1; i < N; ++i)
              {
                W[base + i * G] = y[i];
                U[base + i * G] = z[i];
              }
            if (c == 0)
              {
                W[base] = y[0];
                U[base] = z[0];
              }
          }
        if (tid < LINES)
          {
            const int l    = tid;
            const int base = (l / G) * (G * G) + l % G;
            T         a[G], t2[G], s2[G];
#pragma unroll
            for (int j = 0; j < G; ++j)
              a[j] = W[base + j * G];
            macro_apply2<P, T>(M, K, a, t2, s2);
#pragma unroll
            for (int j = 0; j < G; ++j)
              W[base + j * G] = t2[j];
#pragma unroll
            for (int j = 0; j < G; ++j)
              a[j] = U[base + j * G];
            macro_apply<P, T>(M, a, t2);
#pragma unroll
            for (int j = 0; j < G; ++j)
              U[base + j * G] = fma(c0, t2[j], c1 * s2[j]);
          }
        __syncthreads();
        MGX_STAMP_IT(5);
        if (REM > 0 && tid < REM * NB)
          {
            const int l = NT + tid / NB, c = tid % NB, base = l + c * P * (G * G);
            T         seg[N], y[N], r[N];
#pragma unroll
            for (int i = 0; i < N; ++i)
              seg[i] = W[base + i * (G * G)];
            cell_apply<P, T>(K, seg, r);
#pragma unroll
            for (int i = 0; i < N; ++i)
              seg[i] = U[base + i * (G * G)];
            cell_apply<P, T>(M, seg, y);
#pragma unroll
            for (int i = 0; i < N; ++i)
              y[i] = fma(c2, r[i], y[i]);
            const T yn = next_lane(y[0]);
            if (c + 1 < NB)
              y[P] += yn;
#pragma unroll
            for (int i = 1; i < N; ++i)
              W[base + i * (G * G)] = y[i];
            if (c == 0)
              W[base] = y[0];
          }
        if (tid < LINES)
          {
            const int l = tid;
            T         a[G], r[G], o[G];
#pragma unroll
            for (int j = 0; j < G; ++j)
              a[j] = W[l + j * (G * G)];
            macro_apply<P, T>(K, a, r);
#pragma unroll
            for (int j = 0; j < G; ++j)
              a[j] = U[l + j * (G * G)];
            macro_apply<P, T>(M, a, o);
#pragma unroll
            for (int j = 0; j < G; ++j)
              W[l + j * (G * G)] = fma(c2, r[j], o[j]);
          }
          }
#endif
        __syncthreads();
        MGX_STAMP_IT(6);
        uint32_t *ebase = reinterpret_cast<uint32_t *>(U), *E2 = ebase + C::NE;
        table_store(ebase, ec);
        if (has_next)
          table_store(E2, en);
        const uint32_t *sbase = ebase + 2 * C::NE;
        if (FREE)
          {
#pragma unroll
            for (int j = 0; j < NEW; ++j)
              if (tid + j * NT < C::NE)
                ebase[2 * C::NE + tid + j * NT] = sc[FREE ? j : 0];
          }
        __syncthreads();
        constexpr bool kPipeGather = (MODE != kChebInit || DTAB) && MODE != kCgUpdate && MODE != kChebFirstProlong;
        if (has_next && kPipeGather)
          gather_issue(E2, bn);
        if (has_next)
          coarse_values();
        MGX_STAMP_IT(7);

        {
          constexpr int kChunk = MODE == kPlain ? NU : (MODE == kResidual ? (NU + 1) / 2 : (kKeepX ? MGX_MACRO_CHUNK_CHEB : MGX_MACRO_CHUNK)),
                        NCH    = (NU + kChunk - 1) / kChunk;
          PostOps<T>    ops[2][kChunk];
          uint32_t      iw[2][kChunk];
          uint32_t      pw[2][FREE ? kChunk : 1];
          const uint32_t priv0 = FREE ? (brick_first + b) * post.n_surf : 0u;
          auto slot0 = [&](int u) { return u < JP ? 2 * u : JP + u; };
          auto ulive = [&](int u) { return u < JP ? live_p(u) : live_s(u - JP); };
          auto issue = [&](int c, PostOps<T>(&o)[kChunk], uint32_t(&w)[kChunk], uint32_t(&pv)[FREE ? kChunk : 1]) {
#pragma unroll
            for (int j = 0; j < kChunk; ++j)
              {
                const int u = c * kChunk + j;
                w[j]        = kInvalid;
                if (u < NU && ulive(u))
                  w[j] = ebase[item_slot(mw[slot0(u)])];
                if (FREE)
                  {
                    const uint32_t so = (u < NU && ulive(u)) ? sbase[item_slot(mw[slot0(u < NU ? u : 0)])] : kInvalid;
                    const bool     vd = w[j] != kInvalid;
                    if (vd && so != kInvalid)
                      w[j] = ent_index(w[j]) | 0x40000000u;
                    pv[FREE ? j : 0] = (vd && so != kInvalid)
                                         ? (priv0 + so + item_offset(mw[slot0(u < NU ? u : 0)])) * (uint32_t)sizeof(T)
                                         : kOob;
                  }
              }
#pragma unroll
            for (int j = 0; j < kChunk; ++j)
              {
                const int u = c * kChunk + j;
                if (u < JP)
                  post_issue<T, MODE, DTAB, true>(R, w[j], unit_offset(w[j], mw[slot0(u < NU ? u : 0)], slot0(u < NU ? u : 0), b), o[j]);
                else if (u < NU)
                  post_issue<T, MODE, DTAB, false>(R, w[j], unit_offset(w[j], mw[slot0(u < NU ? u : 0)], slot0(u < NU ? u : 0), b), o[j]);
              }
          };
          issue(0, ops[0], iw[0], pw[0]);
#pragma unroll
          for (int c = 0; c < NCH; ++c)
            {
              if (c + 1 < NCH)
                issue(c + 1, ops[(c + 1) & 1], iw[(c + 1) & 1], pw[(c + 1) & 1]);
              __builtin_amdgcn_sched_barrier(0);
              T val[kChunk][2];
#pragma unroll
              for (int j = 0; j < kChunk; ++j)
                {
                  const int u = c * kChunk + j;
                  val[j][0] = val[j][1] = T(0);
                  if (u < NU && ulive(u))
                    {
                      val[j][0] = W[item_point(mw[slot0(u)])];
                      if (u < JP)
                        val[j][1] = W[item_point(mw[slot0(u) + 1])];
                    }
                }
#pragma unroll
              for (int j = 0; j < kChunk; ++j)
                {
                  const int u = c * kChunk + j;
                  if (u < NU)
                    {
                      const int         v0   = slot0(u);
                      const bool        pair = u < JP;
                      const uint32_t    w    = iw[c & 1][j];
                      const bool        vld  = w != kInvalid, last = vld && (w >> 31);
                      const uint32_t    off  = unit_offset(w, mw[v0], v0, b);
                      const PostOps<T> &o    = ops[c & 1][j];
                      T                 res[2];
#pragma unroll
                      for (int e = 0; e < 2; ++e)
                        {
                          const int v    = (e == 0 || pair) ? v0 + e : v0;
                          const T   dinv = DTAB ? dv[DTAB ? v : 0] : o.bv[e];
                          const T   kept = xs[kKeepX ? v : 0];
                          const T   xi   = kKeepRhs ? cheb_first_iterate(post.f0, dinv, kept) : kept;
                          res[e]         = (e == 0 || pair) ? post_finish<T, MODE>(post, o.pv[e], kKeepRhs ? kept : o.av[e], o.ov[e], dinv,
                                                                                   last, val[j][e], xi)
                                                            : T(0);
                        }
                      constexpr int kStAux = (MODE == kPlain || MODE == kResidual) ? kAuxNt : 0;
                      auto          st     = [&](rsrc_t r, uint32_t f) {
                        if (pair)
                          buf_st2(r, f, res[0], res[1]);
                        else
                          buf_st<kStAux>(r, f, res[0]);
                      };
                      if (MODE == kResidualRestrict)
                        {
                          if (ulive(u))
                            {
                              W[item_point(mw[v0])] = vld ? res[0] : T(0);
                              if (pair)
                                W[item_point(mw[v0 + 1])] = vld ? res[1] : T(0);
                            }
                        }
                      else if (MODE == kCgUpdate)
                        {
                          st(R.out, last ? off : kOob);
                          if (__builtin_amdgcn_ballot_w64(vld && !last) != 0)
                            st(R.partial, last ? kOob : off);
                          const T xn = o.ov[0] + post.f1 * o.bv[0];
                          buf_st(R.srcw, last ? off : kOob, xs[kKeepX ? v0 : 0]);
                          if (post.f1 != T(0))
                            buf_st(R.xw, last ? off : kOob, xn);
                          if (last)
                            {
                              const double qv = (double)res[0], pn = (double)xs[kKeepX ? v0 : 0], rv = (double)o.av[0];
                              cg[0] += qv * pn;
                              cg[1] += rv * rv;
                              cg[2] += qv * rv;
                              cg[3] += qv * qv;
                            }
                        }
                      else
                        {
                          st(R.out, last ? off : kOob);
                          if (FREE)
                            {
                              const uint32_t po = pw[c & 1][FREE ? j : 0];
                              if (__builtin_amdgcn_ballot_w64(po != kOob) != 0)
                                st(R.priv, po);
                              if (__builtin_amdgcn_ballot_w64(vld && !last && po == kOob) != 0)
                                st(R.partial, (last || po != kOob) ? kOob : off);
                            }
#ifndef MGX_MACRO_NOCARRIER
                          else if (__builtin_amdgcn_ballot_w64(vld && !last) != 0)
                            st(R.partial, last ? kOob : off);
#endif
                          if (MODE == kChebFirstProlong)
                            buf_st(R.srcw, last ? off : kOob, xs[kKeepX ? v0 : 0]);
                        }
                    }
                }
              __builtin_amdgcn_sched_barrier(0);
            }
        }
        MGX_STAMP_IT(8);
        if (MODE == kResidualRestrict)
          {
            constexpr int CE1 = C::NB + 1;
            __syncthreads();
            const uint32_t *ctab = post.coarse_blocks + (size_t)(brick_first + b) * (CE1 * CE1 * CE1);
            if (post.coarse_scratch)
              restrict_brick<P, T, NT, true>(tid, W, B->P1eo, nullptr, ctab,
                                             post.coarse_scratch + (size_t)(brick_first + b) * (CNP * CNP * CNP));
            else
              restrict_brick<P, T, NT, false>(tid, W, B->P1eo, post.coarse, ctab);
          }
        if (!has_next)
          break;
        if (!kPipeGather)
          gather_issue(E2, bn);
        __syncthreads();
#pragma unroll
        for (int j = 0; j < NEW; ++j)
          ec[j] = en[j];
        interpolate();
        gather_land();
        add_correction();
        MGX_STAMP_IT(9);
        __syncthreads();
        MGX_STAMP_IT(10);
        b = bn;
        MGX_STAMP_NEXT();
      }
    if (MODE == kCgUpdate)
      {
        static_assert(MODE != kCgUpdate || !MGX_MACRO_PAIRS, "kCgUpdate is written for single items");
        __syncthreads();
        double *red = reinterpret_cast<double *>(U);
#pragma unroll
        for (int k = 0; k < 4; ++k)
          red[k * NT + tid] = cg[k];
        __syncthreads();
        constexpr int P2 = NT <= 64 ? 64 : (NT <= 128 ? 128 : (NT <= 256 ? 256 : 512));
        for (int stride = P2 / 2; stride > 0; stride >>= 1)
          {
            if (tid < stride && tid + stride < NT)
              {
#pragma unroll
                for (int k = 0; k < 4; ++k)
                  red[k * NT + tid] += red[k * NT + tid + stride];
              }
            __syncthreads();
          }
        if (tid < 4)
          post.sums[blockIdx.x * 4 + tid] = red[tid * NT];
      }
#ifdef MGX_MACRO_STAMPS
    asm volatile("s_waitcnt vmcnt(0)" ::: "memory");
    MGX_STAMP(14);
    MGX_STAMP(13);
#endif
  }

  template <int P, typename T, int MODE, bool FREE>
  static void macro_launch(hipStream_t s, const OperatorData &op, const T *src, BrickPost<T> post, int g0, int g1)
  {
    using C                     = MCfg<P, T>;
    const BrickData &bd         = op.bricks;
    const uint32_t  *ent        = FREE ? bd.fr.ent : bd.ent_base;
    const uint32_t  *group_start = FREE ? bd.fr.group_start : bd.colour_start;
    if (FREE)
      {
        post.priv       = (T *)bd.fr.priv;
        post.surf_off   = bd.fr.surf_off;
        post.n_surf     = bd.fr.n_surf;
        post.priv_bytes = (uint32_t)((size_t)bd.n_bricks * bd.fr.n_surf * sizeof(T));
      }
    constexpr bool kUsesDiag = is_cheb_mode(MODE);
    const bool     dtab      = kUsesDiag && op.diag_items;
    if (dtab)
      post.b = (const T *)op.diag_items;
    const bool one_launch = MODE == kResidualRestrict && post.coarse_scratch != nullptr;
    for (int c = g0; c < g1; ++c)
      {
        uint32_t first = group_start[c], count = group_start[c + 1] - first;
        if (one_launch)
          {
            if (c != g0)
              break;
            count = group_start[g1] - first;
          }
        if (count == 0)
          continue;
        const uint32_t grid = persistent_grid(op, C::WGS, count);
        if (dtab)
          hipLaunchKernelGGL((brick_macro_kernel<P, T, MODE, kUsesDiag, FREE>), dim3(grid), dim3(C::THREADS), 0, s, src, first,
                             count, ent, bd.item_map, (const Basis1D<T> *)op.basis, (T)op.coef[0], (T)op.coef[1],
                             (T)op.coef[2], post, (uint32_t)(op.n_dofs * sizeof(T)));
        else
          hipLaunchKernelGGL((brick_macro_kernel<P, T, MODE, false, FREE>), dim3(grid), dim3(C::THREADS), 0, s, src, first,
                             count, ent, bd.item_map, (const Basis1D<T> *)op.basis, (T)op.coef[0], (T)op.coef[1],
                             (T)op.coef[2], post, (uint32_t)(op.n_dofs * sizeof(T)));
      }
  }

#if MGX_MACRO_IS_F64
  __global__ void reduce4_kernel(const double *__restrict__ partials, uint32_t n, const double *__restrict__ extra,
                                 double *__restrict__ sums)
  {
    __shared__ double red[4 * 256];
    const int         tid = threadIdx.x;
    double            acc[4] = {0., 0., 0., 0.};
    for (uint32_t i = tid; i < n; i += 256)
      for (int k = 0; k < 4; ++k)
        acc[k] += partials[4 * (size_t)i + k];
    for (int k = 0; k < 4; ++k)
      red[k * 256 + tid] = acc[k];
    __syncthreads();
    for (int stride = 128; stride > 0; stride >>= 1)
      {
        if (tid < stride)
          for (int k = 0; k < 4; ++k)
            red[k * 256 + tid] += red[k * 256 + tid + stride];
        __syncthreads();
      }
    if (tid < 4)
      sums[tid] = red[tid * 256] + (extra ? extra[tid] : 0.);
  }
#endif

  template <typename T, bool VERIFY>
  __global__ void diag_table_kernel(const T *__restrict__ inv_diag, const uint32_t *__restrict__ ent_base,
                                    const uint32_t *__restrict__ item_map, uint32_t ne, uint32_t npts, uint32_t n_bricks,
                                    T *table, uint32_t *flag)
  {
    if (!VERIFY)
      {
        const uint32_t i = blockIdx.x * blockDim.x + threadIdx.x;
        if (i >= npts)
          return;
        const uint32_t m = item_map[i];
        for (uint32_t brick = n_bricks; brick-- > 0;)
          {
            const uint32_t w = ent_base[(size_t)brick * ne + item_slot(m)];
            if (w != kInvalid)
              {
                table[i] = inv_diag[ent_index(w) + item_offset(m)];
                break;
              }
          }
        return;
      }
    const uint32_t brick = blockIdx.x;
    for (uint32_t i = threadIdx.x; i < npts; i += blockDim.x)
      {
        const uint32_t m = item_map[i], w = ent_base[(size_t)brick * ne + item_slot(m)];
        if (w == kInvalid)
          continue;
        const T v = inv_diag[ent_index(w) + item_offset(m)];
        const T    t   = table[i];
        const T    tol = (sizeof(T) == 8 ? T(1e-14) : T(2e-6)) * (t < 0 ? -t : t);
        const T    dvt = v - t;
        const bool same = (dvt < 0 ? -dvt : dvt) <= tol;
        if (!same)
          atomicOr(flag, 1u);
      }
  }

#define MGX_CAT2(a, b) a##b
#define MGX_CAT(a, b) MGX_CAT2(a, b)
  void MGX_CAT(macro_diag_table_, MGX_MACRO_SUFFIX)(hipStream_t s, const OperatorData &op, const uint32_t *item_map, void *table,
                                                    uint32_t *flag_dev)
  {
    using T             = MGX_MACRO_T;
    const BrickData &bd = op.bricks;
    const uint32_t   nb = op.p <= 4 ? 4 : 2, g = nb * op.p + 1, npts = g * g * g, e1 = 2 * nb + 1, ne = e1 * e1 * e1;
    hipLaunchKernelGGL((diag_table_kernel<T, false>), dim3((npts + 255) / 256), dim3(256), 0, s, (const T *)op.inv_diag,
                       bd.ent_base, item_map, ne, npts, (uint32_t)bd.n_bricks, (T *)table, flag_dev);
    hipLaunchKernelGGL((diag_table_kernel<T, true>), dim3(bd.n_bricks), dim3(256), 0, s, (const T *)op.inv_diag,
                       bd.ent_base, item_map, ne, npts, (uint32_t)bd.n_bricks, (T *)table, flag_dev);
  }

  bool MGX_CAT(launch_macro_cg_update_, MGX_MACRO_SUFFIX)(hipStream_t s, const OperatorData &op, double alpha, double beta,
                                                           const void *r, void *q, void *p, void *x, void *carrier,
                                                           double *partials, uint32_t capacity, uint32_t *n_partials)
  {
    using T = MGX_MACRO_T;
    if (MGX_MACRO_PAIRS || (uint64_t)op.n_dofs * sizeof(T) >= 0xFFFFFFF0ull)
      return false;
    BrickPost<T> post{};
    post.a       = (const T *)r;
    post.b       = (const T *)q;
    post.old     = (const T *)x;
    post.out     = (T *)q;
    post.partial = (T *)carrier;
    post.f1      = (T)alpha;
    post.f2      = (T)beta;
    post.src_w   = (T *)p;
    post.x_w     = (T *)x;
    const BrickData &bd   = op.bricks;
    uint32_t         used = 0;
    auto             run  = [&](auto cfg) {
      using C = decltype(cfg);
      uint64_t total = 0;
      for (int c = 0; c < bd.n_colours; ++c)
        total += persistent_grid(op, C::WGS, bd.colour_start[c + 1] - bd.colour_start[c]);
      if (total > capacity)
        return false;
      for (int c = 0; c < bd.n_colours; ++c)
        {
          const uint32_t first = bd.colour_start[c], count = bd.colour_start[c + 1] - first;
          if (count == 0)
            continue;
          const uint32_t grid = persistent_grid(op, C::WGS, count);
          post.sums = partials + 4 * (size_t)used;
          used += grid;
          hipLaunchKernelGGL((brick_macro_kernel<C::N - 1, T, kCgUpdate, false>), dim3(grid), dim3(C::THREADS), 0, s,
                             (const T *)p, first, count, bd.ent_base, bd.item_map, (const Basis1D<T> *)op.basis,
                             (T)op.coef[0], (T)op.coef[1], (T)op.coef[2], post, (uint32_t)(op.n_dofs * sizeof(T)));
        }
      return true;
    };
    bool ok = false;
    dispatch_degree(op.p, [&](auto degree) {
      if constexpr (!MGX_MACRO_PAIRS)
        ok = run(MCfg<decltype(degree)::value, T>());
    });
    *n_partials = used;
    return ok;
  }

#if MGX_MACRO_IS_F64
  void launch_reduce4(hipStream_t s, const double *partials, uint32_t n, const double *extra, double *sums)
  {
    hipLaunchKernelGGL(reduce4_kernel, dim3(1), dim3(256), 0, s, partials, n, extra, sums);
  }
#endif

  bool MGX_CAT(launch_macro_loop_, MGX_MACRO_SUFFIX)(hipStream_t s, const OperatorData &op, const BrickLaunch &l)
  {
    using T = MGX_MACRO_T;
    const bool fr = l.free_schedule && op.bricks.fr.available() && on_free_schedule(l.mode) && !MGX_MACRO_PAIRS;
    if (l.free_schedule && !fr)
      return false;
    if (!l.free_schedule && op.macro_v2 && !MGX_MACRO_PAIRS && MGX_CAT(launch_macro2_loop_, MGX_MACRO_SUFFIX)(s, op, l))
      return true;
    if (MGX_MACRO_PAIRS * (l.mode == kChebFirstProlong) || (uint64_t)op.n_dofs * sizeof(T) >= 0xFFFFFFF0ull)
      return false;
    BrickPost<T> post = make_post<T>(l);
    post.src_w        = (T *)const_cast<void *>(l.src);
    const T  *src     = (const T *)l.src;
    const int g0 = l.group_begin, g1 = l.group_end;
    bool      launched = false;
    dispatch_degree(op.p, [&](auto degree) {
      constexpr int P = decltype(degree)::value;
      launched        = dispatch_mode<kPlain, kResidual, kCheb, kChebFirst, kChebZeroOld, kChebInit, kChebOldInit, kResidualRestrict,
                               kChebFirstProlong>(l.mode, [&](auto form) {
        constexpr int MODE = decltype(form)::value;
        if constexpr (on_free_schedule(MODE))
          if (fr)
            return macro_launch<P, T, MODE, true>(s, op, src, post, g0, g1);
        macro_launch<P, T, MODE, false>(s, op, src, post, g0, g1);
      });
    });
    return launched;
  }
}
```

### multigrid_amd/csrc/mgx_macro2.hip

```cpp
#include "mgx_macro_device.hpp"

#include <hip/hip_runtime.h>

#include <algorithm>
#include <cstdlib>

#ifndef MGX_MACRO_T
#define MGX_MACRO_T double
#endif
#ifndef MGX_MACRO2_CHUNK
#define MGX_MACRO2_CHUNK 3
#endif

#ifdef MGX_MACRO_STAMPS
#ifndef MGX_MACRO_STAMP_MODE
#define MGX_MACRO_STAMP_MODE -1
#endif
__device__ unsigned long long g_mgx_stamps2[8192 * 16];
#define MGX_STAMP(k)                                                                                              \
  do                                                                                                              \
    {                                                                                                             \
      if (threadIdx.x == 0 && blockIdx.x < 8192 && (MGX_MACRO_STAMP_MODE < 0 || MODE == MGX_MACRO_STAMP_MODE))      \
        g_mgx_stamps2[blockIdx.x * 16 + (k)] = ((k) == 15 || (k) == 13) ? __builtin_amdgcn_s_memrealtime()         \
                                                                         : __builtin_amdgcn_s_memtime();           \
    }                                                                                                             \
  while (0)
#if MGX_MACRO_IS_F64
extern "C" int mgx_debug_read_stamps2(unsigned long long *host, int n_blocks)
{
  return (int)hipMemcpyFromSymbol(host, HIP_SYMBOL(g_mgx_stamps2), sizeof(unsigned long long) * 16 * n_blocks);
}
#endif
#define MGX_STAMP_IT(k)  \
  do                     \
    {                    \
      if (mgx_iter == 3) \
        MGX_STAMP(k);    \
    }                    \
  while (0)
#else
#define MGX_STAMP(k) ((void)0)
#define MGX_STAMP_IT(k) ((void)0)
#endif

namespace mgx
{
  template <int P, typename T>
  struct M2Cfg
  {
    using C = MCfg<P, T>;
    static constexpr int G = C::G, NE = C::NE, NB = C::NB, NPTS = C::NPTS, LINES = C::LINES, THREADS = C::THREADS;
    static constexpr int IT    = (NPTS + THREADS - 1) / THREADS;
    static constexpr int NINT  = (G - 2) * (G - 2) * (G - 2);
    static constexpr int JINT  = NINT / THREADS;
    static constexpr int JSURF = IT - JINT;
    static constexpr int TW    = (NE * 4 + (int)sizeof(T) - 1) / (int)sizeof(T);
    static constexpr int ASZ   = NPTS > TW ? NPTS : TW;
    static constexpr int LDS   = 2 * ASZ * (int)sizeof(T) + NE * 4;
    static constexpr int WG_LDS  = 163840 / LDS;
    static constexpr int WG_WAVE = 32 / (THREADS / 64);
    static constexpr int WGS     = WG_LDS < WG_WAVE ? (WG_LDS < 8 ? WG_LDS : 8) : (WG_WAVE < 8 ? WG_WAVE : 8);
    static constexpr int WAVES   = WGS * (THREADS / 64);
    static constexpr int REGS = (3 * G + JSURF + IT + ((P == 7 || P == 8) ? 4 * (P + 1) : 0)) * ((int)sizeof(T) / 4) + IT + 40;
#ifdef MGX_M2_RMAX
    static constexpr int RMAX = MGX_M2_RMAX;
#else
    static constexpr int RMAX = REGS > 168 ? 2 : (REGS > 128 ? 3 : 4);
#endif
    static constexpr int MINW = (WAVES + 3) / 4 < RMAX ? (WAVES + 3) / 4 : RMAX;
  };

  template <int P, typename T, typename Mark>
  __device__ __forceinline__ void brick_sweeps(int tid, T *__restrict__ U, T *__restrict__ W, const EOMat<T> &M, const EOMat<T> &K,
                                               T c0, T c1, T c2, Mark mark)
  {
    using C             = MCfg<P, T>;
    constexpr int G     = C::G, NT = C::THREADS, LINES = C::LINES, N = P + 1, NB = C::NB;
    constexpr int REM   = LINES - NT;
    if (tid < LINES)
      {
        const int l = tid;
        T         in[G], t1[G], k1[G];
#pragma unroll
        for (int j = 0; j < G; ++j)
          in[j] = U[l * G + j];
        macro_apply2<P, T>(M, K, in, t1, k1);
#pragma unroll
        for (int j = 0; j < G; ++j)
          {
            W[l * G + j] = t1[j];
            U[l * G + j] = k1[j];
          }
      }
    if (REM > 0 && tid < REM * NB)
      {
        const int l = NT + tid / NB, c = tid % NB, base = l * G + c * P;
        T         seg[N], y[N], z[N];
#pragma unroll
        for (int i = 0; i < N; ++i)
          seg[i] = U[base + i];
        cell_apply2<P, T>(M, K, seg, y, z);
        const T yn = next_lane(y[0]), zn = next_lane(z[0]);
        if (c + 1 < NB)
          {
            y[P] += yn;
            z[P] += zn;
          }
#pragma unroll
        for (int i = 1; i < N; ++i)
          {
            W[base + i] = y[i];
            U[base + i] = z[i];
          }
        if (c == 0)
          {
            W[base] = y[0];
            U[base] = z[0];
          }
      }
    lds_barrier();
    mark(0);
    if (REM > 0 && tid < REM * NB)
      {
        const int l = NT + tid / NB, c = tid % NB, base = (l / G) * (G * G) + l % G + c * P * G;
        T         seg[N], y[N], z[N], r[N];
#pragma unroll
        for (int i = 0; i < N; ++i)
          seg[i] = W[base + i * G];
        cell_apply2<P, T>(M, K, seg, y, z);
#pragma unroll
        for (int i = 0; i < N; ++i)
          seg[i] = U[base + i * G];
        cell_apply<P, T>(M, seg, r);
#pragma unroll
        for (int i = 0; i < N; ++i)
          z[i] = fma(c0, r[i], c1 * z[i]);
        const T yn = next_lane(y[0]), zn = next_lane(z[0]);
        if (c + 1 < NB)
          {
            y[P] += yn;
            z[P] += zn;
          }
#pragma unroll
        for (int i = 1; i < N; ++i)
          {
            W[base + i * G] = y[i];
            U[base + i * G] = z[i];
          }
        if (c == 0)
          {
            W[base] = y[0];
            U[base] = z[0];
          }
      }
    if (tid < LINES)
      {
        const int l    = tid;
        const int base = (l / G) * (G * G) + l % G;
        T         a[G], t2[G], s2[G];
#pragma unroll
        for (int j = 0; j < G; ++j)
          a[j] = W[base + j * G];
        macro_apply2<P, T>(M, K, a, t2, s2);
#pragma unroll
        for (int j = 0; j < G; ++j)
          W[base + j * G] = t2[j];
#pragma unroll
        for (int j = 0; j < G; ++j)
          a[j] = U[base + j * G];
        macro_apply<P, T>(M, a, t2);
#pragma unroll
        for (int j = 0; j < G; ++j)
          U[base + j * G] = fma(c0, t2[j], c1 * s2[j]);
      }
    lds_barrier();
    mark(1);
    if (REM > 0 && tid < REM * NB)
      {
        const int l = NT + tid / NB, c = tid % NB, base = l + c * P * (G * G);
        T         seg[N], y[N], r[N];
#pragma unroll
        for (int i = 0; i < N; ++i)
          seg[i] = W[base + i * (G * G)];
        cell_apply<P, T>(K, seg, r);
#pragma unroll
        for (int i = 0; i < N; ++i)
          seg[i] = U[base + i * (G * G)];
        cell_apply<P, T>(M, seg, y);
#pragma unroll
        for (int i = 0; i < N; ++i)
          y[i] = fma(c2, r[i], y[i]);
        const T yn = next_lane(y[0]);
        if (c + 1 < NB)
          y[P] += yn;
#pragma unroll
        for (int i = 1; i < N; ++i)
          W[base + i * (G * G)] = y[i];
        if (c == 0)
          W[base] = y[0];
      }
    if (tid < LINES)
      {
        const int l = tid;
        T         a[G], r[G], o[G];
#pragma unroll
        for (int j = 0; j < G; ++j)
          a[j] = W[l + j * (G * G)];
        macro_apply<P, T>(K, a, r);
#pragma unroll
        for (int j = 0; j < G; ++j)
          a[j] = U[l + j * (G * G)];
        macro_apply<P, T>(M, a, o);
#pragma unroll
        for (int j = 0; j < G; ++j)
          W[l + j * (G * G)] = fma(c2, r[j], o[j]);
      }
  }

  __host__ __device__ constexpr bool macro2_covers(int mode, int p)
  {
    return mode == kPlain || mode == kResidual || ((mode == kResidualRestrict || mode == kChebInit) && p <= 4) || mode == kChebOldInit;
  }

  template <int P, typename T, int MODE>
  __global__ void __launch_bounds__((M2Cfg<P, T>::THREADS), (M2Cfg<P, T>::MINW))
    brick_macro2_kernel(const T *__restrict__ src, uint32_t brick_first, uint32_t brick_count,
                        const uint32_t *__restrict__ ent_base, const uint32_t *__restrict__ item_map,
                        const Basis1D<T> *__restrict__ B, T c0, T c1, T c2, BrickPost<T> post, uint32_t vec_bytes)
  {
    static_assert(macro2_covers(MODE, P), "form not covered by this pipeline");
    using C            = M2Cfg<P, T>;
    constexpr int NT   = C::THREADS, IT = C::IT, JINT = C::JINT, JSURF = C::JSURF, NE = C::NE;
    constexpr int NEW  = (NE + NT - 1) / NT;
    __shared__ T        U[C::ASZ];
    __shared__ T        W[C::ASZ];
    __shared__ uint32_t E[NE];

    const int tid = threadIdx.x;
    uint32_t  b   = blockIdx.x;
    if (b >= brick_count)
      return;
    MGX_STAMP(0);
    MGX_STAMP(15);
#ifdef MGX_MACRO_STAMPS
    int mgx_iter = 0;
#endif
    auto live = [&](int j) { return (j + 1) * NT <= C::NPTS || tid + j * NT < C::NPTS; };
    uint32_t mw[IT];
#pragma unroll
    for (int j = 0; j < IT; ++j)
      mw[j] = item_map[live(j) ? tid + j * NT : 0];
    const rsrc_t rsrc = make_rsrc(src, vec_bytes), r_a = make_rsrc(post.a, vec_bytes), r_out = make_rsrc(post.out, vec_bytes),
                 r_partial = make_rsrc(post.partial, vec_bytes), r_old = make_rsrc(post.old, vec_bytes);
    const EOMat<T> &M = B->mass, &K = B->lapl;
    constexpr bool kKeepX = is_cheb_mode(MODE);
    T              dv[kKeepX ? IT : 1];
    if (kKeepX)
      {
#pragma unroll
        for (int j = 0; j < IT; ++j)
          dv[kKeepX ? j : 0] = post.b[live(j) ? tid + j * NT : 0];
      }

    uint32_t en[NEW] = {};
    auto     table_load = [&](uint32_t brick, uint32_t(&e)[NEW]) {
#pragma unroll
      for (int j = 0; j < NEW; ++j)
        {
          const int i = tid + j * NT;
          e[j]        = ent_base[(size_t)(brick_first + brick) * NE + (i < NE ? i : 0)];
        }
    };
    auto table_store = [&](uint32_t *dst, const uint32_t(&e)[NEW]) {
#pragma unroll
      for (int j = 0; j < NEW; ++j)
        if (tid + j * NT < NE)
          dst[tid + j * NT] = e[j];
    };
    auto unit_offset = [&](uint32_t w, uint32_t m) {
      return w != kInvalid ? (ent_index(w) + item_offset(m)) * (uint32_t)sizeof(T) : kOob;
    };
    T    g[IT];
    auto gather_issue = [&](const uint32_t *tab) {
#pragma unroll
      for (int j = 0; j < IT; ++j)
        {
          g[j] = T(0);
          if (live(j))
            g[j] = buf_ld(MODE == kChebInit ? r_a : rsrc, unit_offset(tab[item_slot(mw[j])], mw[j]), T());
        }
    };
    constexpr bool kKeepRhs = keeps_rhs(MODE);
    T              xs[kKeepX ? IT : 1];
    auto           gather_land = [&]() {
#pragma unroll
      for (int j = 0; j < IT; ++j)
        {
          T v = g[j];
          if (MODE == kChebInit)
            v = cheb_first_iterate(post.f0, dv[kKeepX ? j : 0], g[j]);
          if (live(j))
            U[item_point(mw[j])] = v;
          if (kKeepX)
            xs[kKeepX ? j : 0] = kKeepRhs ? g[j] : v;
        }
    };
    constexpr bool kCarrier = MODE != kResidualRestrict;
    T              pp[JSURF];
    auto           partial_issue = [&]() {
#pragma unroll
      for (int j = JINT; j < IT; ++j)
        {
          pp[j - JINT] = T(0);
          if (!kCarrier)
            continue;
#ifndef MGX_MACRO_NOCARRIER
          const uint32_t w    = live(j) ? E[item_slot(mw[j])] : kInvalid;
          const bool     need = w != kInvalid && !(w & 0x40000000u);
          if (__builtin_amdgcn_ballot_w64(need) != 0)
            pp[j - JINT] = buf_ld(r_partial, need ? unit_offset(w, mw[j]) : kOob, T());
#endif
        }
    };

    constexpr bool kRhs = MODE == kResidual || MODE == kResidualRestrict;
    T              av[kRhs ? IT : 1];
    auto           rhs_issue = [&]() {
      if (kRhs)
        {
#pragma unroll
          for (int j = 0; j < IT; ++j)
            {
              const uint32_t w    = live(j) ? E[item_slot(mw[j])] : kInvalid;
              const bool     last = w != kInvalid && (j < JINT || (w >> 31));
              av[kRhs ? j : 0]    = buf_ld(r_a, last ? unit_offset(w, mw[j]) : kOob, T());
            }
        }
    };

    {
      uint32_t e0[NEW];
      table_load(b, e0);
      if (b + gridDim.x < brick_count)
        table_load(b + gridDim.x, en);
      table_store(E, e0);
      lds_barrier();
      MGX_STAMP(1);
      gather_issue(E);
      gather_land();
      MGX_STAMP(2);
      lds_barrier();
    }

    for (;;)
      {
        const uint32_t bn = b + gridDim.x;
        const bool     has_next = bn < brick_count;
        MGX_STAMP_IT(3);
#ifdef MGX_MACRO_STAMPS
        if (mgx_iter == 4)
          MGX_STAMP(11);
#endif
        partial_issue();
        rhs_issue();
#pragma unroll
        for (int j = 0; j < IT; ++j)
          asm volatile("" : "+v"(mw[j]));
        if (MODE == kChebInit || MODE == kChebOldInit)
          {
#pragma unroll
            for (int j = 0; j < IT; ++j)
              asm volatile("" : "+v"(dv[kKeepX ? j : 0]));
          }
        MGX_STAMP_IT(4);
#ifndef MGX_MACRO_NOSWEEP
        if (kSlicedSweeps<P, MODE> && P >= 9)
          brick_sweeps_sliced<P, T>(
            tid, U, W, B, c0, c1, c2, [&](int k) { MGX_STAMP_IT(5 + k); }, [&]() { lds_barrier(); });
        else
          brick_sweeps<P, T>(tid, U, W, M, K, c0, c1, c2, [&](int k) { MGX_STAMP_IT(5 + k); });
#endif
        lds_barrier();
        MGX_STAMP_IT(7);
        if (has_next)
          {
            table_store(reinterpret_cast<uint32_t *>(U), en);
            lds_barrier();
            gather_issue(reinterpret_cast<const uint32_t *>(U));
          }
        MGX_STAMP_IT(8);

        if constexpr (kKeepX)
          {
            constexpr int kChunk = MGX_MACRO2_CHUNK < IT ? MGX_MACRO2_CHUNK : IT, NCH = (IT + kChunk - 1) / kChunk;
            struct Ops
            {
              T        av, ov;
              uint32_t w, off;
            };
            Ops  ops[2][kChunk];
            auto issue = [&](int c, Ops(&o)[kChunk]) {
#pragma unroll
              for (int k = 0; k < kChunk; ++k)
                {
                  const int j = c * kChunk + k;
                  if (j < IT)
                    o[k].w = live(j) ? E[item_slot(mw[j])] : kInvalid;
                }
#pragma unroll
              for (int k = 0; k < kChunk; ++k)
                {
                  const int j = c * kChunk + k;
                  if (j >= IT)
                    continue;
                  if (j < JINT && o[k].w != kInvalid)
                    o[k].w |= 0xC0000000u;
                  const bool last  = o[k].w != kInvalid && (o[k].w >> 31);
                  o[k].off         = unit_offset(o[k].w, mw[j]);
                  const uint32_t ol = last ? o[k].off : kOob;
                  o[k].av          = kKeepRhs ? T(0) : buf_ld(r_a, ol, T());
                  o[k].ov          = MODE == kCheb ? buf_ld(r_old, ol, T()) : T(0);
                }
            };
            issue(0, ops[0]);
#pragma unroll
            for (int c = 0; c < NCH; ++c)
              {
                if (c + 1 < NCH)
                  issue(c + 1, ops[(c + 1) & 1]);
                __builtin_amdgcn_sched_barrier(0);
                T val[kChunk];
#pragma unroll
                for (int k = 0; k < kChunk; ++k)
                  {
                    const int j = c * kChunk + k;
                    val[k]      = (j < IT && live(j)) ? W[item_point(mw[j])] : T(0);
                  }
#pragma unroll
                for (int k = 0; k < kChunk; ++k)
                  {
                    const int j = c * kChunk + k;
                    if (j >= IT)
                      continue;
                    const Ops &o   = ops[c & 1][k];
                    const bool vld = o.w != kInvalid, last = vld && (o.w >> 31);
                    const T    kept = xs[kKeepX ? j : 0];
                    const T    xi   = kKeepRhs ? cheb_first_iterate(post.f0, dv[kKeepX ? j : 0], kept) : kept;
                    const T    res  = post_finish<T, MODE>(post, j >= JINT ? pp[j >= JINT ? j - JINT : 0] : T(0),
                                                           kKeepRhs ? kept : o.av, o.ov, dv[kKeepX ? j : 0], last, val[k], xi);
                    if (j < JINT)
                      buf_st(r_out, o.off, res);
                    else
                      {
                        buf_st(r_out, last ? o.off : kOob, res);
#ifndef MGX_MACRO_NOCARRIER
                        if (__builtin_amdgcn_ballot_w64(vld && !last) != 0)
                          buf_st(r_partial, last ? kOob : o.off, res);
#endif
                      }
                  }
                __builtin_amdgcn_sched_barrier(0);
              }
          }
        else
          {
          {
            uint32_t w[IT];
  #pragma unroll
            for (int j = 0; j < IT; ++j)
              w[j] = live(j) ? E[item_slot(mw[j])] : kInvalid;
  #pragma unroll
            for (int j = 0; j < IT; ++j)
              {
                if (j < JINT && w[j] != kInvalid)
                  w[j] |= 0xC0000000u;
                const bool     vld = w[j] != kInvalid, last = vld && (w[j] >> 31);
                const uint32_t off = unit_offset(w[j], mw[j]);
                T              val = live(j) ? W[item_point(mw[j])] : T(0);
                if (j >= JINT && kCarrier)
                  val += pp[j >= JINT ? j - JINT : 0];
                if (MODE == kResidualRestrict)
                  {
                    if (live(j))
                      W[item_point(mw[j])] = vld ? (last ? av[kRhs ? j : 0] : T(0)) - val : T(0);
                    continue;
                  }
                if (MODE == kResidual && last)
                  val = av[kRhs ? j : 0] - val;
                if (j < JINT)
                  buf_st<kAuxNt>(r_out, off, val);
                else
                  {
                    buf_st<kAuxNt>(r_out, last ? off : kOob, val);
  #ifndef MGX_MACRO_NOCARRIER
                    if (__builtin_amdgcn_ballot_w64(vld && !last) != 0)
                      buf_st(r_partial, last ? kOob : off, val);
  #endif
                  }
              }
          }
          }
        if (MODE == kResidualRestrict)
          {
            constexpr int CE1 = C::NB + 1, CNP = (C::NB / 2) * P + 1;
            lds_barrier();
            const uint32_t *ctab = post.coarse_blocks + (size_t)(brick_first + b) * (CE1 * CE1 * CE1);
            if (post.coarse_scratch)
              restrict_brick<P, T, NT, true>(tid, W, B->P1eo, nullptr, ctab,
                                             post.coarse_scratch + (size_t)(brick_first + b) * (CNP * CNP * CNP));
            else
              restrict_brick<P, T, NT, false>(tid, W, B->P1eo, post.coarse, ctab);
          }
        MGX_STAMP_IT(9);
        if (!has_next)
          break;
        lds_barrier();
        gather_land();
        table_store(E, en);
        if (bn + gridDim.x < brick_count)
          table_load(bn + gridDim.x, en);
        MGX_STAMP_IT(10);
        lds_barrier();
        b = bn;
#ifdef MGX_MACRO_STAMPS
        ++mgx_iter;
#endif
      }
#ifdef MGX_MACRO_STAMPS
    asm volatile("s_waitcnt vmcnt(0)" ::: "memory");
    MGX_STAMP(14);
    MGX_STAMP(13);
#endif
  }

  template <int P, typename T, int MODE>
  static void macro2_launch(hipStream_t s, const OperatorData &op, const T *src, const BrickPost<T> &post, int g0, int g1)
  {
    using C             = M2Cfg<P, T>;
    const BrickData &bd = op.bricks;
    const bool one_launch = MODE == kResidualRestrict && post.coarse_scratch != nullptr;
    for (int c = g0; c < g1; ++c)
      {
        uint32_t first = bd.colour_start[c], count = bd.colour_start[c + 1] - first;
        if (one_launch)
          {
            if (c != g0)
              break;
            count = bd.colour_start[g1] - first;
          }
        if (count == 0)
          continue;
        const uint32_t grid = persistent_grid(op, C::WGS, count);
        hipLaunchKernelGGL((brick_macro2_kernel<P, T, MODE>), dim3(grid), dim3(C::THREADS), 0, s, src, first, count, bd.ent_base,
                           bd.item_map2, (const Basis1D<T> *)op.basis, (T)op.coef[0], (T)op.coef[1], (T)op.coef[2], post,
                           (uint32_t)(op.n_dofs * sizeof(T)));
      }
  }

#define MGX_CAT2(a, b) a##b
#define MGX_CAT(a, b) MGX_CAT2(a, b)
  bool MGX_CAT(launch_macro2_loop_, MGX_MACRO_SUFFIX)(hipStream_t s, const OperatorData &op, const BrickLaunch &l)
  {
    using T = MGX_MACRO_T;
    if (!macro2_covers(l.mode, op.p) || !op.bricks.item_map2 || (uint64_t)op.n_dofs * sizeof(T) >= 0xFFFFFFF0ull)
      return false;
    if (is_cheb_mode(l.mode) && !op.diag_items2)
      return false;
    BrickPost<T> post = make_post<T>(l);
    post.b            = (const T *)op.diag_items2;
    bool launched     = false;
    dispatch_degree(op.p, [&](auto degree) {
      constexpr int P = decltype(degree)::value;
      dispatch_mode<kPlain, kResidual, kChebInit, kChebOldInit, kResidualRestrict>(l.mode, [&](auto form) {
        constexpr int MODE = decltype(form)::value;
        if constexpr (macro2_covers(MODE, P))
          {
            macro2_launch<P, T, MODE>(s, op, (const T *)l.src, post, l.group_begin, l.group_end);
            launched = true;
          }
      });
    });
    return launched;
  }
}
```

### multigrid_amd/csrc/mgx_macro_device.hpp

```cpp
#pragma once

#include "mgx_brick_device.hpp"
#include "mgx_bricks.hpp"

#include <hip/hip_runtime.h>

namespace mgx
{
  template <int P, typename T>
  struct MCfg
  {
    using C = BCfg<P>;
    static constexpr int NB = C::NB, G = C::G, NE = C::NE, N = P + 1;
    static constexpr int LINES   = G * G;
    static constexpr int THREADS = (LINES > 128 && LINES % 64 <= 40) ? (LINES / 64) * 64 : ((LINES + 63) / 64) * 64;
    static constexpr int NPTS    = G * G * G;
    static constexpr int ent_count(int t) { return (t == 0 || t == 3 ? 1 : 3) * ipow(NB, t) * ipow(NB + 1, 3 - t); }
    static constexpr int ipow(int b, int e) { return e == 0 ? 1 : b * ipow(b, e - 1); }
    static constexpr int ent_size(int t) { return ipow(P - 1, t); }
    static constexpr int NPAIR   = MGX_MACRO_PAIRS ? ent_count(0) * (ent_size(0) / 2) + ent_count(1) * (ent_size(1) / 2) +
                                                     ent_count(2) * (ent_size(2) / 2) + ent_count(3) * (ent_size(3) / 2)
                                                 : 0;
    static constexpr int NSINGLE = NPTS - 2 * NPAIR;
    static constexpr int JP      = (NPAIR + THREADS - 1) / THREADS;
    static constexpr int JS      = (NSINGLE + THREADS - 1) / THREADS;
    static constexpr int IT      = 2 * JP + JS;
    static constexpr int TSZ     = (3 * NE * 4 + (int)sizeof(T) - 1) / (int)sizeof(T);
    static constexpr int ASZ     = NPTS > TSZ ? NPTS : TSZ;
    static constexpr int LDS     = 2 * ASZ * (int)sizeof(T);
    static constexpr int WG_LDS  = 163840 / LDS;
    static constexpr int WG_WAVE = 32 / (THREADS / 64);
    static constexpr int WGS     = WG_LDS < WG_WAVE ? (WG_LDS < 8 ? WG_LDS : 8) : (WG_WAVE < 8 ? WG_WAVE : 8);
    static constexpr int WAVES   = WGS * (THREADS / 64);
    static constexpr int REGS = (3 * G + 2 * IT) * ((int)sizeof(T) / 4) + 2 * IT + 40;
    static constexpr int RMAX = REGS > 168 ? 2 : (REGS > 128 ? 3 : 4);
    static constexpr int MINW = (WAVES + 3) / 4 < RMAX ? (WAVES + 3) / 4 : RMAX;
  };

  template <int P, typename T>
  __device__ __forceinline__ void macro_apply(const EOMat<T> &A, const T (&in)[BCfg<P>::G], T (&out)[BCfg<P>::G])
  {
    constexpr int N = P + 1, NB = BCfg<P>::NB, H1 = N / 2 + 1;
#pragma unroll
    for (int c = 0; c < NB; ++c)
      {
        T seg[N], xe[H1], xo[H1], y[N];
#pragma unroll
        for (int i = 0; i < N; ++i)
          seg[i] = in[c * P + i];
        eo_split<N, T>(seg, xe, xo);
        eo_apply<N, T>(A, xe, xo, y);
        if (c == 0)
          out[0] = y[0];
        else
          out[c * P] += y[0];
#pragma unroll
        for (int i = 1; i < N; ++i)
          out[c * P + i] = y[i];
      }
  }

  template <int P, typename T>
  __device__ __forceinline__ void macro_apply2(const EOMat<T> &A, const EOMat<T> &Bm, const T (&in)[BCfg<P>::G],
                                               T (&oa)[BCfg<P>::G], T (&ob)[BCfg<P>::G])
  {
    constexpr int N = P + 1, NB = BCfg<P>::NB, H1 = N / 2 + 1;
#pragma unroll
    for (int c = 0; c < NB; ++c)
      {
        T seg[N], xe[H1], xo[H1], y[N], z[N];
#pragma unroll
        for (int i = 0; i < N; ++i)
          seg[i] = in[c * P + i];
        eo_split<N, T>(seg, xe, xo);
        eo_apply<N, T>(A, xe, xo, y);
        eo_apply<N, T>(Bm, xe, xo, z);
        if (c == 0)
          {
            oa[0] = y[0];
            ob[0] = z[0];
          }
        else
          {
            oa[c * P] += y[0];
            ob[c * P] += z[0];
          }
#pragma unroll
        for (int i = 1; i < N; ++i)
          {
            oa[c * P + i] = y[i];
            ob[c * P + i] = z[i];
          }
      }
  }

  template <int P, typename T>
  __device__ __forceinline__ void cell_apply(const EOMat<T> &A, const T (&seg)[P + 1], T (&y)[P + 1])
  {
    constexpr int N = P + 1, H1 = N / 2 + 1;
    T             xe[H1], xo[H1];
    eo_split<N, T>(seg, xe, xo);
    eo_apply<N, T>(A, xe, xo, y);
  }
  template <int P, typename T>
  __device__ __forceinline__ void cell_apply2(const EOMat<T> &A, const EOMat<T> &Bm, const T (&seg)[P + 1],
                                              T (&y)[P + 1], T (&z)[P + 1])
  {
    constexpr int N = P + 1, H1 = N / 2 + 1;
    T             xe[H1], xo[H1];
    eo_split<N, T>(seg, xe, xo);
    eo_apply<N, T>(A, xe, xo, y);
    eo_apply<N, T>(Bm, xe, xo, z);
  }
  __device__ __forceinline__ double next_lane(double v) { return __shfl_down(v, 1); }
  __device__ __forceinline__ float  next_lane(float v) { return __shfl_down(v, 1); }

#ifndef MGX_MACRO_SLICED_FROM
#define MGX_MACRO_SLICED_FROM 7
#endif
  template <int P, int MODE>
  constexpr bool kSlicedSweeps = P >= MGX_MACRO_SLICED_FROM && MODE != kResidualRestrict && MODE != kChebFirstProlong;

  template <typename T>
  __device__ __forceinline__ const EOMat<T> &coef_reload(const EOMat<T> *m)
  {
    typedef const EOMat<T> __attribute__((address_space(4))) *ConstPtr;
    ConstPtr q = (ConstPtr)(uintptr_t)m;
    asm volatile("" : "+s"(q));
    return *(const EOMat<T> *)q;
  }

  template <int P, typename T, typename Mark, typename Barrier>
  __device__ __forceinline__ void brick_sweeps_sliced(int tid, T *__restrict__ U, T *__restrict__ W, const Basis1D<T> *__restrict__ B,
                                                      T c0, T c1, T c2, Mark mark, Barrier barrier)
  {
    using C           = MCfg<P, T>;
    constexpr int G   = C::G, NT = C::THREADS, LINES = C::LINES, N = P + 1, NB = C::NB;
    constexpr int REM = LINES - NT;
    const bool    ln  = tid < LINES, rm = REM > 0 && tid < REM * NB;
    const int     rl  = NT + tid / NB, rc = tid % NB;
    auto seam = [&](T(&y)[N]) {
      const T yn = next_lane(y[0]);
      if (rc + 1 < NB)
        y[P] += yn;
    };
    if (ln)
      {
        T in[G], o[G];
#pragma unroll
        for (int j = 0; j < G; ++j)
          in[j] = U[tid * G + j];
#pragma unroll
        for (int ph = 0; ph < 2; ++ph)
          {
            const EOMat<T> &A   = coef_reload(ph == 0 ? &B->mass : &B->lapl);
            T              *dst = ph == 0 ? W : U;
            macro_apply<P, T>(A, in, o);
#pragma unroll
            for (int j = 0; j < G; ++j)
              dst[tid * G + j] = o[j];
          }
      }
    if (rm)
      {
        T         seg[N], y[N];
        const int base = rl * G + rc * P;
#pragma unroll
        for (int i = 0; i < N; ++i)
          seg[i] = U[base + i];
#pragma unroll
        for (int ph = 0; ph < 2; ++ph)
          {
            const EOMat<T> &A   = coef_reload(ph == 0 ? &B->mass : &B->lapl);
            T              *dst = ph == 0 ? W : U;
            cell_apply<P, T>(A, seg, y);
            seam(y);
#pragma unroll
            for (int i = 1; i < N; ++i)
              dst[base + i] = y[i];
            if (rc == 0)
              dst[base] = y[0];
          }
      }
    barrier();
    mark(0);
    if (ln)
      {
        T         a[G], s2[G], t2[G];
        const int lb = (tid / G) * (G * G) + tid % G;
#pragma unroll
        for (int j = 0; j < G; ++j)
          a[j] = W[lb + j * G];
        macro_apply<P, T>(coef_reload(&B->lapl), a, s2);
        const EOMat<T> &M = coef_reload(&B->mass);
        macro_apply<P, T>(M, a, t2);
#pragma unroll
        for (int j = 0; j < G; ++j)
          W[lb + j * G] = t2[j];
#pragma unroll
        for (int j = 0; j < G; ++j)
          a[j] = U[lb + j * G];
        macro_apply<P, T>(M, a, t2);
#pragma unroll
        for (int j = 0; j < G; ++j)
          U[lb + j * G] = fma(c0, t2[j], c1 * s2[j]);
      }
    if (rm)
      {
        T         seg[N], y[N], z[N], r[N];
        const int base = (rl / G) * (G * G) + rl % G + rc * P * G;
#pragma unroll
        for (int i = 0; i < N; ++i)
          seg[i] = W[base + i * G];
        cell_apply<P, T>(coef_reload(&B->lapl), seg, z);
        const EOMat<T> &M = coef_reload(&B->mass);
        cell_apply<P, T>(M, seg, y);
#pragma unroll
        for (int i = 0; i < N; ++i)
          seg[i] = U[base + i * G];
        cell_apply<P, T>(M, seg, r);
#pragma unroll
        for (int i = 0; i < N; ++i)
          z[i] = fma(c0, r[i], c1 * z[i]);
        seam(y);
        seam(z);
#pragma unroll
        for (int i = 1; i < N; ++i)
          {
            W[base + i * G] = y[i];
            U[base + i * G] = z[i];
          }
        if (rc == 0)
          {
            W[base] = y[0];
            U[base] = z[0];
          }
      }
    barrier();
    mark(1);
    if (ln)
      {
        T a[G], r[G], o[G];
#pragma unroll
        for (int j = 0; j < G; ++j)
          a[j] = W[tid + j * (G * G)];
        macro_apply<P, T>(coef_reload(&B->lapl), a, r);
#pragma unroll
        for (int j = 0; j < G; ++j)
          a[j] = U[tid + j * (G * G)];
        macro_apply<P, T>(coef_reload(&B->mass), a, o);
#pragma unroll
        for (int j = 0; j < G; ++j)
          W[tid + j * (G * G)] = fma(c2, r[j], o[j]);
      }
    if (rm)
      {
        T         seg[N], y[N], q[N];
        const int base = rl + rc * P * (G * G);
#pragma unroll
        for (int i = 0; i < N; ++i)
          seg[i] = W[base + i * (G * G)];
        cell_apply<P, T>(coef_reload(&B->lapl), seg, q);
#pragma unroll
        for (int i = 0; i < N; ++i)
          seg[i] = U[base + i * (G * G)];
        cell_apply<P, T>(coef_reload(&B->mass), seg, y);
#pragma unroll
        for (int i = 0; i < N; ++i)
          y[i] = fma(c2, q[i], y[i]);
        seam(y);
#pragma unroll
        for (int i = 1; i < N; ++i)
          W[base + i * (G * G)] = y[i];
        if (rc == 0)
          W[base] = y[0];
      }
  }

  __device__ __forceinline__ uint32_t item_slot(uint32_t m) { return m & 1023u; }
  __device__ __forceinline__ uint32_t item_point(uint32_t m) { return (m >> 10) & 8191u; }
  __device__ __forceinline__ uint32_t item_offset(uint32_t m) { return m >> 23; }

  using rsrc_t = __amdgpu_buffer_rsrc_t;
  typedef unsigned int u32x2_t __attribute__((ext_vector_type(2)));
  constexpr uint32_t kOob = 0xFFFFFFF0u;
  constexpr int kAuxNt = 2;
  __device__ __forceinline__ rsrc_t make_rsrc(const void *p, uint32_t bytes)
  {
    return __builtin_amdgcn_make_buffer_rsrc(const_cast<void *>(p), 0, bytes, 0x00020000);
  }
  __device__ __forceinline__ double buf_ld(rsrc_t r, uint32_t off, double)
  {
    return __builtin_bit_cast(double, __builtin_amdgcn_raw_buffer_load_b64(r, off, 0, 0));
  }
  __device__ __forceinline__ float buf_ld(rsrc_t r, uint32_t off, float)
  {
    return __builtin_bit_cast(float, __builtin_amdgcn_raw_buffer_load_b32(r, off, 0, 0));
  }
  template <int AUX = 0>
  __device__ __forceinline__ void buf_st(rsrc_t r, uint32_t off, double v)
  {
    __builtin_amdgcn_raw_buffer_store_b64(__builtin_bit_cast(u32x2_t, v), r, off, 0, AUX);
  }
  template <int AUX = 0>
  __device__ __forceinline__ void buf_st(rsrc_t r, uint32_t off, float v)
  {
    __builtin_amdgcn_raw_buffer_store_b32(__builtin_bit_cast(unsigned int, v), r, off, 0, AUX);
  }

  typedef unsigned int u32x4_t __attribute__((ext_vector_type(4)));
  __device__ __forceinline__ void buf_ld2(rsrc_t r, uint32_t off, double &a, double &b)
  {
    const u32x4_t v = __builtin_bit_cast(u32x4_t, __builtin_amdgcn_raw_buffer_load_b128(r, off, 0, 0));
    a               = __builtin_bit_cast(double, u32x2_t{v.x, v.y});
    b               = __builtin_bit_cast(double, u32x2_t{v.z, v.w});
  }
  __device__ __forceinline__ void buf_ld2(rsrc_t r, uint32_t off, float &a, float &b)
  {
    const unsigned long long u = __builtin_bit_cast(unsigned long long, __builtin_amdgcn_raw_buffer_load_b64(r, off, 0, 0));
    a                          = __builtin_bit_cast(float, (unsigned int)u);
    b                          = __builtin_bit_cast(float, (unsigned int)(u >> 32));
  }
  __device__ __forceinline__ void buf_st2(rsrc_t r, uint32_t off, double a, double b)
  {
    const u32x2_t lo = __builtin_bit_cast(u32x2_t, a), hi = __builtin_bit_cast(u32x2_t, b);
    __builtin_amdgcn_raw_buffer_store_b128(u32x4_t{lo.x, lo.y, hi.x, hi.y}, r, off, 0, 0);
  }
  __device__ __forceinline__ void buf_st2(rsrc_t r, uint32_t off, float a, float b)
  {
    __builtin_amdgcn_raw_buffer_store_b64(u32x2_t{__builtin_bit_cast(unsigned int, a), __builtin_bit_cast(unsigned int, b)}, r,
                                          off, 0, 0);
  }

#ifndef MGX_CHEB_INIT_REREAD
#define MGX_CHEB_INIT_REREAD 0
#endif
  __host__ __device__ constexpr bool keeps_rhs(int mode) { return mode == kChebInit && !MGX_CHEB_INIT_REREAD; }

  template <typename T>
  __device__ __forceinline__ T cheb_first_iterate(T f0, T d, T b)
  {
    T x = f0 * d * b;
    asm("" : "+v"(x));
    return x;
  }

  template <typename T>
  struct PostRsrc
  {
    rsrc_t a, b, old, out, partial, src, srcw, xw, priv;
  };

  template <typename T>
  struct PostOps
  {
    T pv[2], av[2], bv[2], ov[2];
  };

  template <typename T, int MODE, bool DTAB, bool PAIR>
  __device__ __forceinline__ void post_issue(const PostRsrc<T> &R, uint32_t w, uint32_t off, PostOps<T> &o)
  {
    const bool valid        = w != kInvalid;
    const bool need_partial = valid && !(w & 0x40000000u) && MODE != kResidualRestrict;
    const bool last         = valid && (w >> 31);
    o.pv[0] = o.pv[1] = o.av[0] = o.av[1] = o.bv[0] = o.bv[1] = o.ov[0] = o.ov[1] = T(0);
    const uint32_t ol = last ? off : kOob, op = need_partial ? off : kOob;
    auto           ld = [&](rsrc_t r, uint32_t f, T(&v)[2]) {
      if (PAIR)
        buf_ld2(r, f, v[0], v[1]);
      else
        v[0] = buf_ld(r, f, T());
    };
#ifndef MGX_MACRO_NOCARRIER
    if (__builtin_amdgcn_ballot_w64(need_partial) != 0)
      ld(R.partial, op, o.pv);
#endif
    if (MODE != kPlain && !keeps_rhs(MODE))
      ld(R.a, ol, o.av);
    if (is_cheb_mode(MODE) && !DTAB)
      ld(R.b, ol, o.bv);
    if (MODE == kCheb || MODE == kCgUpdate)
      ld(R.old, ol, o.ov);
    if (MODE == kCgUpdate)
      ld(R.src, ol, o.bv);
  }

  template <typename T, int MODE>
  __device__ __forceinline__ T post_finish(const BrickPost<T> &post, T pv, T av, T ov, T bv, bool last, T val, T xi)
  {
    val += pv;
    if (MODE == kPlain || MODE == kCgUpdate)
      return val;
    else if (MODE == kResidualRestrict)
      return (last ? av : T(0)) - val;
    else if (MODE == kResidual)
      return last ? av - val : val;
    else
      {
        if (MODE == kChebOldInit)
          ov = post.f0 * bv * av;
        T xn = xi + post.f2 * bv * (av - val);
        if (MODE == kCheb || MODE == kChebOldInit)
          xn += post.f1 * (xi - ov);
        else if (MODE == kChebZeroOld || MODE == kChebInit)
          xn += post.f1 * xi;
        return last ? xn : val;
      }
  }
}
```

Baseline: 14.82 billion DoFs/s.

## Look up inverse diagonal from a small per-class LDS table in brick kernels

Adds an optional path where the inverse diagonal, if it is bitwise uniform across bricks by position class, is stored as a tiny table (p^3 or merged (p/2+1)^3 entries) in LDS. Per-item diagonal registers are replaced by packed 6-bit class indices. For some Chebyshev modes the right-hand side is loaded early alongside the gather, and barriers become LDS-only. This is meant to cut register pressure and diagonal traffic, at the cost of LDS lookups, extra setup kernels and a check at diagonal computation time.

```diff
diff --git a/multigrid_amd/csrc/mgx_api.cpp b/multigrid_amd/csrc/mgx_api.cpp
--- a/multigrid_amd/csrc/mgx_api.cpp
+++ b/multigrid_amd/csrc/mgx_api.cpp
@@ -105,6 +105,7 @@
     {"macro_wg_per_cu_x16", nullptr, &macro_wg_x16},
     {"no_diag_table", &no_diag_table, nullptr},
     {"no_macro_v2", &no_macro_v2, nullptr},
+    {"no_diag_classes", &no_diag_classes, nullptr},
     {"no_general_bricks", &no_general_bricks, nullptr},
     {"general_brick_min", nullptr, &general_brick_min},
     {"fused_prolong_min_bricks", nullptr, &fused_prolong_min_bricks},
@@ -2127,6 +2128,39 @@
       if (which == 0)
         MGX_TRACE("compute_diagonal: diagonal %s per brick item", mismatch == 0 ? "uniform" : "not uniform");
     }
+  for (int which = 0; which < 2; ++which)
+    {
+      void          *&slot  = which == 0 ? op->d.diag_classes : op->d.diag_classes2;
+      const void     *items = which == 0 ? op->d.diag_items : op->d.diag_items2;
+      const uint32_t *map   = which == 0 ? op->d.bricks.item_map : op->d.bricks.item_map2;
+      const char     *name  = which == 0 ? "class" : "merged class (second pipeline)";
+      op->mem.release(slot);
+      slot = nullptr;
+      if (!items || op->d.p > 4 || op->ctx->tun.no_diag_classes)
+        {
+          MGX_TRACE("compute_diagonal: diagonal by %s not used (%s)", name,
+                    !items ? "no per-item table" : (op->d.p > 4 ? "p > 4" : "option no_diag_classes"));
+          continue;
+        }
+      const uint32_t n1 = which == 0 ? (uint32_t)op->d.p : (uint32_t)op->d.p / 2 + 1;
+      DeviceArena    tmp("mgx_compute_diagonal");
+      void          *table = nullptr;
+      uint32_t      *flag  = nullptr, mismatch = 1;
+      MGX_TRY(op->mem.zeros(&table, number_size(op->d.number) * n1 * n1 * n1, s));
+      MGX_TRY(tmp.zeros(&flag, 1, s));
+      if (op->d.number == MGX_F64)
+        macro_diag_classes_f64(s, op->d, map, items, which == 1, table, flag);
+      else
+        macro_diag_classes_f32(s, op->d, map, items, which == 1, table, flag);
+      MGX_HIP(hipMemcpyAsync(&mismatch, flag, sizeof(uint32_t), hipMemcpyDeviceToHost, s));
+      MGX_HIP(hipStreamSynchronize(s));
+      if (mismatch == 0)
+        slot = table;
+      else
+        op->mem.release(table);
+      MGX_TRACE("compute_diagonal: diagonal by %s %s", name,
+                mismatch == 0 ? "bitwise uniform, class table in use" : "not bitwise uniform, per-item registers kept");
+    }
   return MGX_OK;
 }
 
diff --git a/multigrid_amd/csrc/mgx_brick_device.hpp b/multigrid_amd/csrc/mgx_brick_device.hpp
--- a/multigrid_amd/csrc/mgx_brick_device.hpp
+++ b/multigrid_amd/csrc/mgx_brick_device.hpp
@@ -45,6 +45,7 @@
     T              *priv;
     const uint32_t *surf_off;
     uint32_t        n_surf, priv_bytes;
+    const T        *dcls;
   };
 
   template <typename T>
diff --git a/multigrid_amd/csrc/mgx_internal.hpp b/multigrid_amd/csrc/mgx_internal.hpp
--- a/multigrid_amd/csrc/mgx_internal.hpp
+++ b/multigrid_amd/csrc/mgx_internal.hpp
@@ -41,6 +41,7 @@
     uint32_t fused_prolong_min_bricks = 8192;
     bool     no_general_bricks = false;
     uint32_t general_brick_min = 2048;
+    bool     no_diag_classes  = false;
     bool     no_macro_v2      = false;
     bool     no_fused_init    = false;
     bool     no_fused_restrict = false;
@@ -144,6 +145,8 @@
     bool      separable     = true;
     void     *diag_items    = nullptr;
     void     *diag_items2   = nullptr;
+    void     *diag_classes  = nullptr;
+    void     *diag_classes2 = nullptr;
     bool      macro_v2      = true;
   };
 
@@ -397,6 +400,10 @@
   void launch_reduce4(hipStream_t s, const double *partials, uint32_t n, const double *extra, double *sums);
   void macro_diag_table_f64(hipStream_t s, const OperatorData &op, const uint32_t *item_map, void *table, uint32_t *flag_dev);
   void macro_diag_table_f32(hipStream_t s, const OperatorData &op, const uint32_t *item_map, void *table, uint32_t *flag_dev);
+  void macro_diag_classes_f64(hipStream_t s, const OperatorData &op, const uint32_t *item_map, const void *table, bool merged,
+                              void *classes, uint32_t *flag_dev);
+  void macro_diag_classes_f32(hipStream_t s, const OperatorData &op, const uint32_t *item_map, const void *table, bool merged,
+                              void *classes, uint32_t *flag_dev);
   bool launch_macro2_loop_f64(hipStream_t s, const OperatorData &op, const BrickLaunch &launch);
   bool launch_macro2_loop_f32(hipStream_t s, const OperatorData &op, const BrickLaunch &launch);
   void launch_cell_diagonal(hipStream_t s, const OperatorData &op, void *diag, const double *a1d, const double *m1d,
diff --git a/multigrid_amd/csrc/mgx_macro.hip b/multigrid_amd/csrc/mgx_macro.hip
--- a/multigrid_amd/csrc/mgx_macro.hip
+++ b/multigrid_amd/csrc/mgx_macro.hip
@@ -4,6 +4,7 @@
 
 #include <algorithm>
 #include <cstdlib>
+#include <type_traits>
 
 #ifndef MGX_MACRO_CHUNK
 #define MGX_MACRO_CHUNK (MGX_MACRO_PAIRS ? 3 : 4)
@@ -50,7 +51,9 @@
 
 namespace mgx
 {
-  template <int P, typename T, int MODE, bool DTAB, bool FREE = false>
+  template <int P, typename T, int MODE, int DTAB, bool FREE>
+  constexpr bool kEarlyRhs = DTAB == kDiagClasses && !FREE && (diag_classes_use(MODE, P, sizeof(T) == 8) & kUseEarlyRhs) != 0;
+  template <int P, typename T, int MODE, int DTAB, bool FREE = false>
   __global__ void __launch_bounds__((MCfg<P, T>::THREADS), (MCfg<P, T>::MINW))
     brick_macro_kernel(const T *__restrict__ src, uint32_t brick_first, uint32_t brick_count,
                        const uint32_t *__restrict__ ent_base, const uint32_t *__restrict__ item_map,
@@ -68,6 +71,16 @@
     constexpr int  NG     = ((MODE == kChebInit && !DTAB) || MODE == kCgUpdate) ? 2 : 1;
     __shared__ T U[C::ASZ];
     __shared__ T W[C::ASZ];
+    constexpr bool kRegs = DTAB == kDiagItems, kCls = DTAB == kDiagClasses;
+    constexpr bool kEarlyB = kEarlyRhs<P, T, MODE, DTAB, FREE>;
+    static_assert(!kCls || (C::DCLS > 0 && C::DCLS <= 64 && C::DCLS <= NT), "class table: p <= 4");
+    __shared__ T DC[kCls ? C::DCLS : 1];
+    auto sync = [&]() {
+      if (kEarlyB)
+        lds_barrier();
+      else
+        __syncthreads();
+    };
 
     const int tid = threadIdx.x;
     uint32_t  b   = blockIdx.x;
@@ -99,23 +112,39 @@
         const int q    = tid + j * NT;
         mw[2 * JP + j] = item_map[2 * NP + (q < NS ? q : 0)];
       }
-    T dv[DTAB ? IT : 1];
-    if (DTAB)
+    T dv[kRegs ? IT : 1];
+    if (kRegs)
       {
 #pragma unroll
         for (int j = 0; j < JP; ++j)
           {
             const int q                = tid + j * NT;
-            dv[DTAB ? 2 * j : 0]       = post.b[2 * (q < NP ? q : 0)];
-            dv[DTAB ? 2 * j + 1 : 0]   = post.b[2 * (q < NP ? q : 0) + 1];
+            dv[kRegs ? 2 * j : 0]      = post.b[2 * (q < NP ? q : 0)];
+            dv[kRegs ? 2 * j + 1 : 0]  = post.b[2 * (q < NP ? q : 0) + 1];
           }
 #pragma unroll
         for (int j = 0; j < JS; ++j)
           {
             const int q               = tid + j * NT;
-            dv[DTAB ? 2 * JP + j : 0] = post.b[2 * NP + (q < NS ? q : 0)];
-          }
-      }
+            dv[kRegs ? 2 * JP + j : 0] = post.b[2 * NP + (q < NS ? q : 0)];
+          }
+      }
+    if (kCls && tid < C::DCLS)
+      DC[tid] = post.dcls[tid];
+    constexpr int NDW = (IT + 4) / 5;
+    uint32_t      dcw[kCls ? NDW : 1];
+    if (kCls)
+      {
+#pragma unroll
+        for (int k = 0; k < NDW; ++k)
+          dcw[kCls ? k : 0] = 0u;
+#pragma unroll
+        for (int it = 0; it < IT; ++it)
+          dcw[kCls ? it / 5 : 0] |= diag_class_of(item_point(mw[it]), (uint32_t)G, (uint32_t)P) << (6 * (it % 5));
+      }
+    auto dinv_of = [&](int it) -> T {
+      return kCls ? DC[(dcw[kCls ? it / 5 : 0] >> (6 * (it % 5))) & 63u] : dv[kRegs ? it : 0];
+    };
     const rsrc_t      rsrc = make_rsrc(src, vec_bytes);
     const PostRsrc<T> R{make_rsrc(post.a, vec_bytes),   make_rsrc(post.b, vec_bytes),       make_rsrc(post.old, vec_bytes),
                         make_rsrc(post.out, vec_bytes), make_rsrc(post.partial, vec_bytes), rsrc,
@@ -229,6 +258,34 @@
             }
         }
     };
+    T    bq[kEarlyB ? IT : 1];
+    auto rhs_issue = [&](const uint32_t *E, uint32_t brick) {
+      if (kEarlyB)
+        {
+#pragma unroll
+          for (int j = 0; j < JP; ++j)
+            {
+              bq[kEarlyB ? 2 * j : 0] = bq[kEarlyB ? 2 * j + 1 : 0] = T(0);
+              if (live_p(j))
+                {
+                  const uint32_t w = E[item_slot(mw[2 * j])];
+                  buf_ld2(R.a, (w != kInvalid && (w >> 31)) ? unit_offset(w, mw[2 * j], 2 * j, brick) : kOob, bq[kEarlyB ? 2 * j : 0],
+                          bq[kEarlyB ? 2 * j + 1 : 0]);
+                }
+            }
+#pragma unroll
+          for (int j = 0; j < JS; ++j)
+            {
+              const int v         = 2 * JP + j;
+              bq[kEarlyB ? v : 0] = T(0);
+              if (live_s(j))
+                {
+                  const uint32_t w    = E[item_slot(mw[v])];
+                  bq[kEarlyB ? v : 0] = buf_ld(R.a, (w != kInvalid && (w >> 31)) ? unit_offset(w, mw[v], v, brick) : kOob, T());
+                }
+            }
+        }
+    };
     constexpr bool kKeepRhs = keeps_rhs(MODE);
     T              xs[kKeepX ? IT : 1];
     auto           gather_land = [&]() {
@@ -238,7 +295,7 @@
           T       v  = g[0][it];
           const T bi = g[DTAB ? 0 : NG - 1][it];
           if (MODE == kChebInit)
-            v = cheb_first_iterate(post.f0, DTAB ? dv[DTAB ? it : 0] : g[0][it], bi);
+            v = cheb_first_iterate(post.f0, DTAB ? dinv_of(it) : g[0][it], bi);
           if (MODE == kCgUpdate)
             v = post.f1 == T(0) ? g[NG - 1][it] : post.f2 * g[0][it] + g[NG - 1][it];
           if (live(it))
@@ -274,13 +331,14 @@
     __syncthreads();
     MGX_STAMP(1);
     gather_issue(reinterpret_cast<const uint32_t *>(W), b);
+    rhs_issue(reinterpret_cast<const uint32_t *>(W), b);
     coarse_words(b);
     coarse_values();
     interpolate();
     gather_land();
     add_correction();
     MGX_STAMP(2);
-    __syncthreads();
+    sync();
 
 #ifdef MGX_MACRO_STAMPS
     int mgx_iter = 0;
@@ -300,16 +358,22 @@
 #pragma unroll
         for (int it = 0; it < IT; ++it)
           asm volatile("" : "+v"(mw[it]));
-        if (DTAB && (MODE == kChebInit || MODE == kChebOldInit))
+        if (kCls)
+          {
+#pragma unroll
+            for (int k = 0; k < NDW; ++k)
+              asm volatile("" : "+v"(dcw[kCls ? k : 0]));
+          }
+        if (kRegs && (MODE == kChebInit || MODE == kChebOldInit))
           {
 #pragma unroll
             for (int it = 0; it < IT; ++it)
-              asm volatile("" : "+v"(dv[DTAB ? it : 0]));
+              asm volatile("" : "+v"(dv[kRegs ? it : 0]));
           }
 #ifndef MGX_MACRO_NOSWEEP
         if (kSlicedSweeps<P, MODE>)
           brick_sweeps_sliced<P, T>(
-            tid, U, W, B, c0, c1, c2, [&](int i) { MGX_STAMP_IT(4 + i); }, [&]() { __syncthreads(); });
+            tid, U, W, B, c0, c1, c2, [&](int i) { MGX_STAMP_IT(4 + i); }, [&]() { sync(); });
         else
           {
         if (tid < LINES)
@@ -353,7 +417,7 @@
                 U[base] = z[0];
               }
           }
-        __syncthreads();
+        sync();
         MGX_STAMP_IT(4);
         if (REM > 0 && tid < REM * NB)
           {
@@ -408,7 +472,7 @@
             for (int j = 0; j < G; ++j)
               U[base + j * G] = fma(c0, t2[j], c1 * s2[j]);
           }
-        __syncthreads();
+        sync();
         MGX_STAMP_IT(5);
         if (REM > 0 && tid < REM * NB)
           {
@@ -452,7 +516,7 @@
           }
           }
 #endif
-        __syncthreads();
+        sync();
         MGX_STAMP_IT(6);
         uint32_t *ebase = reinterpret_cast<uint32_t *>(U), *E2 = ebase + C::NE;
         table_store(ebase, ec);
@@ -466,7 +530,7 @@
               if (tid + j * NT < C::NE)
                 ebase[2 * C::NE + tid + j * NT] = sc[FREE ? j : 0];
           }
-        __syncthreads();
+        sync();
         constexpr bool kPipeGather = (MODE != kChebInit || DTAB) && MODE != kCgUpdate && MODE != kChebFirstProlong;
         if (has_next && kPipeGather)
           gather_issue(E2, bn);
@@ -507,9 +571,9 @@
               {
                 const int u = c * kChunk + j;
                 if (u < JP)
-                  post_issue<T, MODE, DTAB, true>(R, w[j], unit_offset(w[j], mw[slot0(u < NU ? u : 0)], slot0(u < NU ? u : 0), b), o[j]);
+                  post_issue<T, MODE, DTAB != 0, true, kEarlyB>(R, w[j], unit_offset(w[j], mw[slot0(u < NU ? u : 0)], slot0(u < NU ? u : 0), b), o[j]);
                 else if (u < NU)
-                  post_issue<T, MODE, DTAB, false>(R, w[j], unit_offset(w[j], mw[slot0(u < NU ? u : 0)], slot0(u < NU ? u : 0), b), o[j]);
+                  post_issue<T, MODE, DTAB != 0, false, kEarlyB>(R, w[j], unit_offset(w[j], mw[slot0(u < NU ? u : 0)], slot0(u < NU ? u : 0), b), o[j]);
               }
           };
           issue(0, ops[0], iw[0], pw[0]);
@@ -549,10 +613,11 @@
                       for (int e = 0; e < 2; ++e)
                         {
                           const int v    = (e == 0 || pair) ? v0 + e : v0;
-                          const T   dinv = DTAB ? dv[DTAB ? v : 0] : o.bv[e];
+                          const T   dinv = DTAB ? dinv_of(v) : o.bv[e];
+                          const T   rhs  = kEarlyB ? bq[kEarlyB ? v : 0] : o.av[e];
                           const T   kept = xs[kKeepX ? v : 0];
                           const T   xi   = kKeepRhs ? cheb_first_iterate(post.f0, dinv, kept) : kept;
-                          res[e]         = (e == 0 || pair) ? post_finish<T, MODE>(post, o.pv[e], kKeepRhs ? kept : o.av[e], o.ov[e], dinv,
+                          res[e]         = (e == 0 || pair) ? post_finish<T, MODE>(post, o.pv[e], kKeepRhs ? kept : rhs, o.ov[e], dinv,
                                                                                    last, val[j][e], xi)
                                                             : T(0);
                         }
@@ -629,7 +694,8 @@
           break;
         if (!kPipeGather)
           gather_issue(E2, bn);
-        __syncthreads();
+        rhs_issue(E2, bn);
+        sync();
 #pragma unroll
         for (int j = 0; j < NEW; ++j)
           ec[j] = en[j];
@@ -637,7 +703,7 @@
         gather_land();
         add_correction();
         MGX_STAMP_IT(9);
-        __syncthreads();
+        sync();
         MGX_STAMP_IT(10);
         b = bn;
         MGX_STAMP_NEXT();
@@ -690,6 +756,9 @@
     const bool     dtab      = kUsesDiag && op.diag_items;
     if (dtab)
       post.b = (const T *)op.diag_items;
+    constexpr bool kClasses = (diag_classes_use(MODE, P, sizeof(T) == 8) & kUseClasses) != 0;
+    const bool     dcls     = dtab && kClasses && op.diag_classes;
+    post.dcls               = dcls ? (const T *)op.diag_classes : nullptr;
     const bool one_launch = MODE == kResidualRestrict && post.coarse_scratch != nullptr;
     for (int c = g0; c < g1; ++c)
       {
@@ -703,12 +772,20 @@
         if (count == 0)
           continue;
         const uint32_t grid = persistent_grid(op, C::WGS, count);
+        if constexpr (kClasses)
+          if (dcls)
+            {
+              hipLaunchKernelGGL((brick_macro_kernel<P, T, MODE, kDiagClasses, FREE>), dim3(grid), dim3(C::THREADS), 0, s, src,
+                                 first, count, ent, bd.item_map, (const Basis1D<T> *)op.basis, (T)op.coef[0], (T)op.coef[1],
+                                 (T)op.coef[2], post, (uint32_t)(op.n_dofs * sizeof(T)));
+              continue;
+            }
         if (dtab)
-          hipLaunchKernelGGL((brick_macro_kernel<P, T, MODE, kUsesDiag, FREE>), dim3(grid), dim3(C::THREADS), 0, s, src, first,
+          hipLaunchKernelGGL((brick_macro_kernel<P, T, MODE, kUsesDiag ? kDiagItems : kDiagStreamed, FREE>), dim3(grid), dim3(C::THREADS), 0, s, src, first,
                              count, ent, bd.item_map, (const Basis1D<T> *)op.basis, (T)op.coef[0], (T)op.coef[1],
                              (T)op.coef[2], post, (uint32_t)(op.n_dofs * sizeof(T)));
         else
-          hipLaunchKernelGGL((brick_macro_kernel<P, T, MODE, false, FREE>), dim3(grid), dim3(C::THREADS), 0, s, src, first,
+          hipLaunchKernelGGL((brick_macro_kernel<P, T, MODE, kDiagStreamed, FREE>), dim3(grid), dim3(C::THREADS), 0, s, src, first,
                              count, ent, bd.item_map, (const Basis1D<T> *)op.basis, (T)op.coef[0], (T)op.coef[1],
                              (T)op.coef[2], post, (uint32_t)(op.n_dofs * sizeof(T)));
       }
@@ -789,6 +866,43 @@
                        bd.ent_base, item_map, ne, npts, (uint32_t)bd.n_bricks, (T *)table, flag_dev);
     hipLaunchKernelGGL((diag_table_kernel<T, true>), dim3(bd.n_bricks), dim3(256), 0, s, (const T *)op.inv_diag,
                        bd.ent_base, item_map, ne, npts, (uint32_t)bd.n_bricks, (T *)table, flag_dev);
+  }
+
+  template <typename T, bool VERIFY>
+  __global__ void diag_class_kernel(const T *__restrict__ table, const uint32_t *__restrict__ item_map, uint32_t npts, uint32_t g,
+                                    uint32_t p, bool merged, T *classes, uint32_t *flag)
+  {
+    using Bits       = typename std::conditional<sizeof(T) == 8, unsigned long long, unsigned int>::type;
+    const uint32_t i = blockIdx.x * blockDim.x + threadIdx.x;
+    if (i >= npts)
+      return;
+    const uint32_t pnt = item_point(item_map[i]), c = merged ? diag_class_merged_of(pnt, g, p) : diag_class_of(pnt, g, p);
+    const Bits     t   = __builtin_bit_cast(Bits, table[i]);
+    if (!VERIFY)
+      {
+        const uint32_t x = pnt % g, y = (pnt / g) % g, z = pnt / (g * g);
+        auto           is_entry = [&](uint32_t a) { return a >= 1 && a <= p && (!merged || a == p || 2 * a <= p); };
+        if (is_entry(x) && is_entry(y) && is_entry(z))
+          {
+            classes[c] = table[i];
+            if (t == 0)
+              atomicOr(flag, 1u);
+          }
+        return;
+      }
+    if (t != 0 && t != __builtin_bit_cast(Bits, classes[c]))
+      atomicOr(flag, 1u);
+  }
+
+  void MGX_CAT(macro_diag_classes_, MGX_MACRO_SUFFIX)(hipStream_t s, const OperatorData &op, const uint32_t *item_map,
+                                                      const void *table, bool merged, void *classes, uint32_t *flag_dev)
+  {
+    using T           = MGX_MACRO_T;
+    const uint32_t nb = op.p <= 4 ? 4 : 2, g = nb * op.p + 1, npts = g * g * g;
+    hipLaunchKernelGGL((diag_class_kernel<T, false>), dim3((npts + 255) / 256), dim3(256), 0, s, (const T *)table, item_map, npts, g,
+                       (uint32_t)op.p, merged, (T *)classes, flag_dev);
+    hipLaunchKernelGGL((diag_class_kernel<T, true>), dim3((npts + 255) / 256), dim3(256), 0, s, (const T *)table, item_map, npts, g,
+                       (uint32_t)op.p, merged, (T *)classes, flag_dev);
   }
 
   bool MGX_CAT(launch_macro_cg_update_, MGX_MACRO_SUFFIX)(hipStream_t s, const OperatorData &op, double alpha, double beta,
@@ -825,7 +939,7 @@
           const uint32_t grid = persistent_grid(op, C::WGS, count);
           post.sums = partials + 4 * (size_t)used;
           used += grid;
-          hipLaunchKernelGGL((brick_macro_kernel<C::N - 1, T, kCgUpdate, false>), dim3(grid), dim3(C::THREADS), 0, s,
+          hipLaunchKernelGGL((brick_macro_kernel<C::N - 1, T, kCgUpdate, kDiagStreamed>), dim3(grid), dim3(C::THREADS), 0, s,
                              (const T *)p, first, count, bd.ent_base, bd.item_map, (const Basis1D<T> *)op.basis,
                              (T)op.coef[0], (T)op.coef[1], (T)op.coef[2], post, (uint32_t)(op.n_dofs * sizeof(T)));
         }
diff --git a/multigrid_amd/csrc/mgx_macro2.hip b/multigrid_amd/csrc/mgx_macro2.hip
--- a/multigrid_amd/csrc/mgx_macro2.hip
+++ b/multigrid_amd/csrc/mgx_macro2.hip
@@ -222,7 +222,7 @@
     return mode == kPlain || mode == kResidual || ((mode == kResidualRestrict || mode == kChebInit) && p <= 4) || mode == kChebOldInit;
   }
 
-  template <int P, typename T, int MODE>
+  template <int P, typename T, int MODE, bool DCLS = false>
   __global__ void __launch_bounds__((M2Cfg<P, T>::THREADS), (M2Cfg<P, T>::MINW))
     brick_macro2_kernel(const T *__restrict__ src, uint32_t brick_first, uint32_t brick_count,
                         const uint32_t *__restrict__ ent_base, const uint32_t *__restrict__ item_map,
@@ -235,6 +235,9 @@
     __shared__ T        U[C::ASZ];
     __shared__ T        W[C::ASZ];
     __shared__ uint32_t E[NE];
+    constexpr int       NM = P / 2 + 1;
+    static_assert(!DCLS || (P <= 4 && C::WGS * (C::LDS + NM * NM * NM * (int)sizeof(T)) <= 163840), "class table: p <= 4");
+    __shared__ T DC[DCLS ? NM * NM * NM : 1];
 
     const int tid = threadIdx.x;
     uint32_t  b   = blockIdx.x;
@@ -254,13 +257,28 @@
                  r_partial = make_rsrc(post.partial, vec_bytes), r_old = make_rsrc(post.old, vec_bytes);
     const EOMat<T> &M = B->mass, &K = B->lapl;
     constexpr bool kKeepX = is_cheb_mode(MODE);
-    T              dv[kKeepX ? IT : 1];
-    if (kKeepX)
+    constexpr bool kRegs  = kKeepX && !DCLS;
+    T              dv[kRegs ? IT : 1];
+    if (kRegs)
       {
 #pragma unroll
         for (int j = 0; j < IT; ++j)
-          dv[kKeepX ? j : 0] = post.b[live(j) ? tid + j * NT : 0];
-      }
+          dv[kRegs ? j : 0] = post.b[live(j) ? tid + j * NT : 0];
+      }
+    if (DCLS && tid < NM * NM * NM)
+      DC[tid] = post.dcls[tid];
+    constexpr int NDW = (IT + 4) / 5;
+    uint32_t      dcw[DCLS ? NDW : 1];
+    if (DCLS)
+      {
+#pragma unroll
+        for (int k = 0; k < NDW; ++k)
+          dcw[DCLS ? k : 0] = 0u;
+#pragma unroll
+        for (int j = 0; j < IT; ++j)
+          dcw[DCLS ? j / 5 : 0] |= diag_class_merged_of(item_point(mw[j]), (uint32_t)C::G, (uint32_t)P) << (6 * (j % 5));
+      }
+    auto dinv_of = [&](int j) -> T { return DCLS ? DC[(dcw[DCLS ? j / 5 : 0] >> (6 * (j % 5))) & 63u] : dv[kRegs ? j : 0]; };
 
     uint32_t en[NEW] = {};
     auto     table_load = [&](uint32_t brick, uint32_t(&e)[NEW]) {
@@ -298,7 +316,7 @@
         {
           T v = g[j];
           if (MODE == kChebInit)
-            v = cheb_first_iterate(post.f0, dv[kKeepX ? j : 0], g[j]);
+            v = cheb_first_iterate(post.f0, dinv_of(j), g[j]);
           if (live(j))
             U[item_point(mw[j])] = v;
           if (kKeepX)
@@ -323,7 +341,8 @@
         }
     };
 
-    constexpr bool kRhs = MODE == kResidual || MODE == kResidualRestrict;
+    constexpr bool kRhs = MODE == kResidual || MODE == kResidualRestrict ||
+                          (DCLS && (diag_classes_use(MODE, P, sizeof(T) == 8, 2) & kUseEarlyRhs) != 0);
     T              av[kRhs ? IT : 1];
     auto           rhs_issue = [&]() {
       if (kRhs)
@@ -366,11 +385,17 @@
 #pragma unroll
         for (int j = 0; j < IT; ++j)
           asm volatile("" : "+v"(mw[j]));
-        if (MODE == kChebInit || MODE == kChebOldInit)
+        if (DCLS)
+          {
+#pragma unroll
+            for (int k = 0; k < NDW; ++k)
+              asm volatile("" : "+v"(dcw[DCLS ? k : 0]));
+          }
+        if (kRegs && (MODE == kChebInit || MODE == kChebOldInit))
           {
 #pragma unroll
             for (int j = 0; j < IT; ++j)
-              asm volatile("" : "+v"(dv[kKeepX ? j : 0]));
+              asm volatile("" : "+v"(dv[kRegs ? j : 0]));
           }
         MGX_STAMP_IT(4);
 #ifndef MGX_MACRO_NOSWEEP
@@ -418,7 +443,7 @@
                   const bool last  = o[k].w != kInvalid && (o[k].w >> 31);
                   o[k].off         = unit_offset(o[k].w, mw[j]);
                   const uint32_t ol = last ? o[k].off : kOob;
-                  o[k].av          = kKeepRhs ? T(0) : buf_ld(r_a, ol, T());
+                  o[k].av          = (kKeepRhs || kRhs) ? T(0) : buf_ld(r_a, ol, T());
                   o[k].ov          = MODE == kCheb ? buf_ld(r_old, ol, T()) : T(0);
                 }
             };
@@ -445,9 +470,10 @@
                     const Ops &o   = ops[c & 1][k];
                     const bool vld = o.w != kInvalid, last = vld && (o.w >> 31);
                     const T    kept = xs[kKeepX ? j : 0];
-                    const T    xi   = kKeepRhs ? cheb_first_iterate(post.f0, dv[kKeepX ? j : 0], kept) : kept;
+                    const T    dinv = dinv_of(j);
+                    const T    xi   = kKeepRhs ? cheb_first_iterate(post.f0, dinv, kept) : kept;
                     const T    res  = post_finish<T, MODE>(post, j >= JINT ? pp[j >= JINT ? j - JINT : 0] : T(0),
-                                                           kKeepRhs ? kept : o.av, o.ov, dv[kKeepX ? j : 0], last, val[k], xi);
+                                                           kKeepRhs ? kept : (kRhs ? av[kRhs ? j : 0] : o.av), o.ov, dinv, last, val[k], xi);
                     if (j < JINT)
                       buf_st(r_out, o.off, res);
                     else
@@ -534,8 +560,11 @@
   }
 
   template <int P, typename T, int MODE>
-  static void macro2_launch(hipStream_t s, const OperatorData &op, const T *src, const BrickPost<T> &post, int g0, int g1)
+  static void macro2_launch(hipStream_t s, const OperatorData &op, const T *src, BrickPost<T> post, int g0, int g1)
   {
+    constexpr bool kClasses = macro2_covers(MODE, P) && (diag_classes_use(MODE, P, sizeof(T) == 8, 2) & kUseClasses) != 0;
+    const bool     dcls     = kClasses && op.diag_classes2;
+    post.dcls               = dcls ? (const T *)op.diag_classes2 : nullptr;
     using C             = M2Cfg<P, T>;
     const BrickData &bd = op.bricks;
     const bool one_launch = MODE == kResidualRestrict && post.coarse_scratch != nullptr;
@@ -551,6 +580,14 @@
         if (count == 0)
           continue;
         const uint32_t grid = persistent_grid(op, C::WGS, count);
+        if constexpr (kClasses)
+          if (dcls)
+            {
+              hipLaunchKernelGGL((brick_macro2_kernel<P, T, MODE, true>), dim3(grid), dim3(C::THREADS), 0, s, src, first, count,
+                                 bd.ent_base, bd.item_map2, (const Basis1D<T> *)op.basis, (T)op.coef[0], (T)op.coef[1],
+                                 (T)op.coef[2], post, (uint32_t)(op.n_dofs * sizeof(T)));
+              continue;
+            }
         hipLaunchKernelGGL((brick_macro2_kernel<P, T, MODE>), dim3(grid), dim3(C::THREADS), 0, s, src, first, count, bd.ent_base,
                            bd.item_map2, (const Basis1D<T> *)op.basis, (T)op.coef[0], (T)op.coef[1], (T)op.coef[2], post,
                            (uint32_t)(op.n_dofs * sizeof(T)));
diff --git a/multigrid_amd/csrc/mgx_macro_device.hpp b/multigrid_amd/csrc/mgx_macro_device.hpp
--- a/multigrid_amd/csrc/mgx_macro_device.hpp
+++ b/multigrid_amd/csrc/mgx_macro_device.hpp
@@ -35,7 +35,42 @@
     static constexpr int REGS = (3 * G + 2 * IT) * ((int)sizeof(T) / 4) + 2 * IT + 40;
     static constexpr int RMAX = REGS > 168 ? 2 : (REGS > 128 ? 3 : 4);
     static constexpr int MINW = (WAVES + 3) / 4 < RMAX ? (WAVES + 3) / 4 : RMAX;
+    static constexpr int DCLS = P <= 4 ? P * P * P : 0;
+    static_assert(WGS * (LDS + DCLS * (int)sizeof(T)) <= 163840, "the class table does not fit next to the brick arrays");
   };
+
+  enum DiagSource
+  {
+    kDiagStreamed = 0,
+    kDiagItems    = 1,
+    kDiagClasses  = 2
+  };
+  __host__ __device__ constexpr uint32_t diag_class_of(uint32_t point, uint32_t g, uint32_t p)
+  {
+    return (((point / (g * g)) % p) * p + ((point / g) % g) % p) * p + (point % g) % p;
+  }
+  __host__ __device__ constexpr uint32_t diag_merged(uint32_t r, uint32_t p) { return r < p - r ? r : p - r; }
+  __host__ __device__ constexpr uint32_t diag_class_merged_of(uint32_t point, uint32_t g, uint32_t p)
+  {
+    const uint32_t nm = p / 2 + 1;
+    return (diag_merged((point / (g * g)) % p, p) * nm + diag_merged(((point / g) % g) % p, p)) * nm + diag_merged((point % g) % p, p);
+  }
+#ifndef MGX_DIAG_CLASSES_ALL
+#define MGX_DIAG_CLASSES_ALL 0
+#endif
+  constexpr int kUseClasses = 1, kUseEarlyRhs = 2;
+  __host__ __device__ constexpr int diag_classes_use(int mode, int p, bool f64, int pipeline = 1)
+  {
+    if (!is_cheb_mode(mode) || p > 4)
+      return 0;
+    if (MGX_DIAG_CLASSES_ALL)
+      return (mode == kChebInit || (pipeline == 2 && !f64)) ? kUseClasses : (kUseClasses | kUseEarlyRhs);
+    if (pipeline != 2 || p != 4)
+      return 0;
+    if (f64)
+      return mode == kChebOldInit ? (kUseClasses | kUseEarlyRhs) : 0;
+    return (mode == kChebInit || mode == kChebOldInit) ? kUseClasses : 0;
+  }
 
   template <int P, typename T>
   __device__ __forceinline__ void macro_apply(const EOMat<T> &A, const T (&in)[BCfg<P>::G], T (&out)[BCfg<P>::G])
@@ -357,7 +392,7 @@
     T pv[2], av[2], bv[2], ov[2];
   };
 
-  template <typename T, int MODE, bool DTAB, bool PAIR>
+  template <typename T, int MODE, bool DTAB, bool PAIR, bool EARLYB = false>
   __device__ __forceinline__ void post_issue(const PostRsrc<T> &R, uint32_t w, uint32_t off, PostOps<T> &o)
   {
     const bool valid        = w != kInvalid;
@@ -375,7 +410,7 @@
     if (__builtin_amdgcn_ballot_w64(need_partial) != 0)
       ld(R.partial, op, o.pv);
 #endif
-    if (MODE != kPlain && !keeps_rhs(MODE))
+    if (MODE != kPlain && !keeps_rhs(MODE) && !EARLYB)
       ld(R.a, ol, o.av);
     if (is_cheb_mode(MODE) && !DTAB)
       ld(R.b, ol, o.bv);
```

Result: no change. 14.87 billion DoFs/s, median of 4 (+0.4%).
